# JuliaMolSim/DFTK.jl

Measured on AMD Instinct MI355X. Metric: SCF iterations/sec (Hψ applies/sec) at fixed Ecut·atoms, higher is better.
Workload: dtype f64

## Files before the change

### dftk.jl_amd/_lib.py

```python
from __future__ import annotations

import ctypes as C
import os

from . import _build

c_cplx_p = C.c_void_p
_i64 = C.c_int64


class dftk_mi_cplx(C.Structure):
    _fields_ = [("re", C.c_double), ("im", C.c_double)]


class dftk_mi_batch_op(C.Structure):
    _fields_ = ([(name, C.c_int32) for name in ("type", "fiber", "trans", "m", "k", "i0", "mode", "flags", "join_next",
                                                 "sync_after", "status", "reserved")] +
                [(name, _i64) for name in ("n", "gm", "gn", "gk", "lda", "ldb", "ldc")] +
                [("alpha", dftk_mi_cplx), ("beta", dftk_mi_cplx), ("s0", C.c_double)] +
                [(name, C.c_void_p) for name in ("A", "B", "W", "W2", "W3", "C", "D", "E", "F", "kb", "host")] +
                [("bytes", C.c_uint64)])


class DftkMiError(RuntimeError):
    def __init__(self, status, msg):
        super().__init__(f"dftk_mi355x status {status}: {msg}")
        self.status = status


_SIGNATURES = {
    "dftk_mi_last_error": (C.c_char_p, []),
    "dftk_mi_version": (C.c_char_p, []),
    "dftk_mi_basis_create": (C.c_int, [C.c_int, C.c_int, C.c_int, C.c_double, C.c_int, C.POINTER(C.c_void_p)]),
    "dftk_mi_basis_destroy": (C.c_int, [C.c_void_p]),
    "dftk_mi_basis_sync": (C.c_int, [C.c_void_p]),
    "dftk_mi_basis_set_fft_batch": (C.c_int, [C.c_void_p, C.c_int]),
    "dftk_mi_basis_stream": (C.c_void_p, [C.c_void_p]),
    "dftk_mi_kblock_create": (C.c_int, [C.c_void_p, _i64, C.c_void_p, C.c_void_p, C.POINTER(C.c_void_p)]),
    "dftk_mi_kblock_destroy": (C.c_int, [C.c_void_p]),
    "dftk_mi_kblock_set_projectors": (C.c_int, [C.c_void_p, C.c_int, C.c_void_p, _i64, C.c_void_p]),
    "dftk_mi_kblock_set_potential": (C.c_int, [C.c_void_p, C.c_void_p]),
    "dftk_mi_apply_H": (C.c_int, [C.c_void_p, C.c_int, C.c_void_p, _i64, C.c_void_p, _i64]),
    "dftk_mi_apply_H_parts": (C.c_int, [C.c_void_p, C.c_int, C.c_int, C.c_void_p, _i64, C.c_void_p, _i64]),
    "dftk_mi_local_potential": (C.c_int, [C.c_void_p, C.c_void_p, C.c_void_p, C.c_void_p, C.c_int, C.c_void_p,
                                          C.c_void_p]),
    "dftk_mi_local_potential_collinear": (C.c_int, [C.c_void_p, C.c_void_p, C.c_void_p, C.c_void_p, C.c_int, C.c_void_p,
                                                    C.c_void_p]),
    "dftk_mi_density_accumulate_spin": (C.c_int, [C.c_void_p, C.c_int, C.c_void_p, _i64, C.c_void_p, C.c_void_p, C.c_int,
                                                  C.c_int]),
    "dftk_mi_kpoint_sphere_host": (C.c_int, [C.c_int, C.c_int, C.c_int, C.c_void_p, C.c_void_p, C.c_double, _i64,
                                             C.POINTER(_i64), C.c_void_p, C.c_void_p, C.c_void_p]),
    "dftk_mi_build_projectors_hgh": (C.c_int, [C.c_void_p, _i64, C.c_void_p, C.c_void_p, C.c_void_p, C.c_double, C.c_int,
                                               C.c_void_p, C.c_void_p, C.c_int, C.c_void_p, C.c_void_p, C.c_void_p, _i64,
                                               C.POINTER(C.c_int)]),
    "dftk_mi_atomic_superposition": (C.c_int, [C.c_void_p, C.c_int, C.c_void_p, C.c_int, C.c_void_p, C.c_int, C.c_void_p,
                                               C.c_void_p, C.c_void_p]),
    "dftk_mi_forces_local": (C.c_int, [C.c_void_p, C.c_void_p, C.c_int, C.c_void_p, C.c_int, C.c_void_p, C.c_void_p,
                                       C.c_void_p, C.c_void_p]),
    "dftk_mi_radial_transform": (C.c_int, [C.c_void_p, C.c_int, C.c_int, C.c_int, C.c_void_p, C.c_void_p, C.c_double, _i64,
                                           C.c_void_p, C.c_void_p]),
    "dftk_mi_radial_tile": (C.c_int, []),
    "dftk_mi_build_projectors_radial": (C.c_int, [C.c_void_p, _i64, C.c_void_p, C.c_void_p, C.c_void_p, C.c_double,
                                                  C.c_int, C.c_void_p, _i64, C.c_void_p, C.c_void_p, C.c_int, C.c_void_p,
                                                  C.c_void_p, C.c_void_p, _i64, C.POINTER(C.c_int)]),
    "dftk_mi_atomic_superposition_table": (C.c_int, [C.c_void_p, C.c_void_p, C.c_int, C.c_void_p, C.c_int, C.c_void_p,
                                                     C.c_void_p, C.c_void_p, C.c_void_p]),
    "dftk_mi_forces_local_table": (C.c_int, [C.c_void_p, C.c_void_p, C.c_int, C.c_void_p, C.c_int, C.c_void_p, C.c_void_p,
                                             C.c_void_p, C.c_void_p]),
    "dftk_mi_forces_nonlocal": (C.c_int, [C.c_void_p, C.c_void_p, C.c_int, C.c_void_p, _i64, C.c_void_p, C.c_int,
                                          C.c_void_p, C.c_void_p]),
    "dftk_mi_local_potential_displacement": (C.c_int, [C.c_void_p, C.c_void_p, C.c_int, C.c_void_p, C.c_int, C.c_void_p,
                                                       C.c_void_p]),
    "dftk_mi_dynmat_local": (C.c_int, [C.c_void_p, C.c_void_p, C.c_int, C.c_void_p, C.c_int, C.c_void_p, C.c_void_p,
                                       C.c_void_p, C.c_void_p]),
    "dftk_mi_nonlocal_displacement_apply": (C.c_int, [C.c_void_p, C.c_void_p, C.c_int, C.c_int, C.c_void_p, C.c_int,
                                                      C.c_void_p, _i64, C.c_void_p, _i64]),
    "dftk_mi_dynmat_nonlocal": (C.c_int, [C.c_void_p, C.c_void_p, C.c_int, C.c_void_p, _i64, C.c_void_p, _i64, C.c_void_p,
                                          C.c_void_p, C.c_int, C.c_void_p, C.c_void_p, C.c_void_p]),
    "dftk_mi_stress_kinetic_nonlocal": (C.c_int, [C.c_void_p, C.c_void_p, C.c_void_p, C.c_int, C.c_void_p, _i64, C.c_void_p,
                                                  C.c_int, C.c_void_p, C.c_void_p, C.c_int, C.c_void_p, C.c_void_p,
                                                  C.c_void_p, C.c_void_p]),
    "dftk_mi_stress_cube": (C.c_int, [C.c_void_p, C.c_void_p, C.c_int, C.c_void_p, C.c_int, C.c_void_p, C.c_void_p,
                                      C.c_void_p, C.c_void_p]),
    "dftk_mi_stress_xc": (C.c_int, [C.c_void_p, _i64, C.c_int, C.c_void_p, C.c_void_p, C.c_void_p, C.c_void_p, C.c_void_p,
                                    C.c_void_p]),
    "dftk_mi_xc_gga": (C.c_int, [C.c_void_p, _i64, C.c_void_p, C.c_void_p, C.c_int, C.c_double, C.c_void_p, C.c_void_p,
                                 C.c_void_p]),
    "dftk_mi_ifft_sphere": (C.c_int, [C.c_void_p, C.c_void_p, C.c_void_p]),
    "dftk_mi_fft_sphere": (C.c_int, [C.c_void_p, C.c_void_p, C.c_void_p]),
    "dftk_mi_density_accumulate": (C.c_int, [C.c_void_p, C.c_int, C.c_void_p, _i64, C.c_void_p, C.c_void_p]),
    "dftk_mi_sternheimer": (C.c_int, [C.c_void_p, C.c_int, C.c_void_p, _i64, C.c_void_p, C.c_int, C.c_void_p, _i64, C.c_void_p,
                                      _i64, C.c_void_p, C.c_int, C.c_int, C.c_void_p, _i64, C.c_void_p, _i64,
                                      C.POINTER(C.c_int), C.c_void_p, C.POINTER(C.c_int)]),
    "dftk_mi_density_response_accumulate": (C.c_int, [C.c_void_p, C.c_int, C.c_void_p, _i64, C.c_void_p, _i64, C.c_void_p,
                                                      C.c_void_p, C.c_void_p]),
    "dftk_mi_apply_kernel": (C.c_int, [C.c_void_p, C.c_void_p, C.c_void_p, C.c_void_p, C.c_int, C.c_void_p]),
    "dftk_mi_transfer_blochwave": (C.c_int, [C.c_void_p, C.c_void_p, C.c_void_p, C.c_int, C.c_void_p, _i64, C.c_void_p, _i64]),
    "dftk_mi_transfer_density": (C.c_int, [C.c_void_p, C.c_void_p, C.c_int, C.c_void_p, C.c_void_p]),
    "dftk_mi_refinement_metric_solve": (C.c_int, [C.c_void_p, C.c_int, C.c_void_p, _i64, C.c_void_p, _i64, C.c_double, C.c_int,
                                                  C.c_void_p, _i64, C.c_void_p, C.c_void_p]),
    "dftk_mi_exx_apply": (C.c_int, [C.c_void_p, C.c_int, C.c_void_p, _i64, C.c_void_p, C.c_void_p, C.c_int, C.c_void_p, _i64,
                                    C.c_void_p, _i64, C.c_int]),
    "dftk_mi_lobpcg": (C.c_int, [C.c_void_p, C.c_int, C.c_void_p, _i64, C.c_double, C.c_int, C.c_int, C.c_int,
                                 C.c_int, C.c_uint64, C.c_void_p, C.c_void_p, C.POINTER(C.c_int),
                                 C.POINTER(C.c_int), C.POINTER(_i64)]),
    "dftk_mi_local_potential_gga": (C.c_int, [C.c_void_p, C.c_void_p, C.c_void_p, C.c_void_p, C.c_void_p, C.c_int,
                                              C.c_double, C.c_void_p, C.c_void_p]),
    "dftk_mi_local_potential_collinear_gga": (C.c_int, [C.c_void_p, C.c_void_p, C.c_void_p, C.c_void_p, C.c_void_p, C.c_int,
                                                        C.c_double, C.c_void_p, C.c_void_p]),
    "dftk_mi_local_potential_core": (C.c_int, [C.c_void_p, C.c_void_p, C.c_int, C.c_void_p, C.c_void_p, C.c_void_p,
                                               C.c_void_p, C.c_void_p, C.c_int, C.c_double, C.c_void_p, C.c_void_p]),
    "dftk_mi_cube_gradient": (C.c_int, [C.c_void_p, C.c_void_p, C.c_void_p, C.c_void_p]),
    "dftk_mi_xc_gga_spin": (C.c_int, [C.c_void_p, _i64, C.c_void_p, C.c_void_p, C.c_int, C.c_double, C.c_void_p, C.c_void_p,
                                      C.c_void_p]),
    "dftk_mi_kblock_set_kpoint": (C.c_int, [C.c_void_p, C.c_void_p, C.c_void_p]),
    "dftk_mi_kblock_set_tau_potential": (C.c_int, [C.c_void_p, C.c_void_p]),
    "dftk_mi_kblocks_set_tau_potential": (C.c_int, [C.c_int, C.c_void_p, C.c_void_p]),
    "dftk_mi_kinetic_energy_density_accumulate": (C.c_int, [C.c_void_p, C.c_int, C.c_void_p, _i64, C.c_void_p, C.c_void_p]),
    "dftk_mi_local_potential_mgga": (C.c_int, [C.c_void_p, C.c_void_p, C.c_void_p, C.c_void_p, C.c_void_p, C.c_void_p, C.c_int,
                                               C.c_double, C.c_void_p, C.c_void_p, C.c_void_p]),
    "dftk_mi_xc_mgga": (C.c_int, [C.c_void_p, _i64, C.c_void_p, C.c_void_p, C.c_void_p, C.c_int, C.c_double, C.c_void_p,
                                  C.c_void_p, C.c_void_p, C.c_void_p]),
    "dftk_mi_symmetrize_rho": (C.c_int, [C.c_void_p, C.c_int, C.c_void_p, C.c_void_p, C.c_int, C.c_void_p, C.c_void_p]),
    "dftk_mi_mix_kerker": (C.c_int, [C.c_void_p, C.c_void_p, C.c_double, C.c_void_p, C.c_void_p]),
    "dftk_mi_mix_dielectric": (C.c_int, [C.c_void_p, C.c_void_p, C.c_double, C.c_double, C.c_void_p, C.c_void_p]),
    "dftk_mi_chi0_dielectric_apply": (C.c_int, [C.c_void_p, C.c_void_p, C.c_double, C.c_double, C.c_void_p, C.c_void_p]),
    "dftk_mi_cube_fourier_filter": (C.c_int, [C.c_void_p, C.c_void_p, C.c_void_p, C.c_void_p]),
    "dftk_mi_kblocks_set_potential": (C.c_int, [C.c_int, C.c_void_p, C.c_void_p]),
    "dftk_mi_lobpcg_multi": (C.c_int, [C.c_int, C.c_void_p, C.c_int, C.c_void_p, C.c_void_p, C.c_double, C.c_int, C.c_int,
                                       C.c_int, C.c_int, C.c_void_p, C.c_void_p, C.c_void_p, C.c_void_p, C.c_void_p,
                                       C.c_void_p, C.c_void_p]),
    "dftk_mi_density_accumulate_multi": (C.c_int, [C.c_int, C.c_void_p, C.c_void_p, C.c_void_p, C.c_void_p, C.c_void_p,
                                                   C.c_void_p]),
    "dftk_mi_density_accumulate_multi2": (C.c_int, [C.c_int, C.c_void_p, C.c_void_p, C.c_void_p, C.c_void_p, C.c_void_p,
                                                    C.c_void_p, C.c_void_p, C.c_void_p]),
    "dftk_mi_band_kinetic_multi": (C.c_int, [C.c_int, C.c_void_p, C.c_void_p, C.c_void_p, C.c_void_p, C.c_void_p]),
    "dftk_mi_batch_stats": (C.c_int, [C.POINTER(_i64), C.POINTER(_i64), C.POINTER(_i64), C.POINTER(_i64)]),
    "dftk_mi_lobpcg_small_stats": (C.c_int, [C.POINTER(_i64), C.POINTER(_i64)]),
    "dftk_mi_ortho_small": (C.c_int, [C.c_void_p, _i64, C.c_int, C.c_void_p, _i64, C.c_int, C.c_void_p, _i64, C.c_void_p,
                                      C.c_double, C.c_void_p]),
    "dftk_mi_batch_replay": (C.c_int, [C.c_void_p, C.c_int, C.c_int, C.c_void_p]),
    "dftk_mi_lobpcg_last_AX": (C.c_void_p, [C.c_void_p]),
    "dftk_mi_lobpcg_history": (C.c_int, [C.c_void_p, C.POINTER(C.c_int), C.POINTER(C.c_int), C.c_void_p, C.c_size_t,
                                         C.POINTER(C.c_int)]),
    "dftk_mi_columnwise_norms": (C.c_int, [C.c_void_p, _i64, C.c_int, C.c_void_p, _i64, C.c_void_p]),
    "dftk_mi_columnwise_dots": (C.c_int, [C.c_void_p, _i64, C.c_int, C.c_void_p, _i64, C.c_void_p, _i64, C.c_void_p]),
    "dftk_mi_ortho_qr": (C.c_int, [C.c_void_p, _i64, C.c_int, C.c_void_p, _i64, C.c_int, C.POINTER(C.c_int),
                                   C.POINTER(C.c_int)]),
    "dftk_mi_tpa_precondprep": (C.c_int, [C.c_void_p, C.c_int, C.c_void_p, _i64, C.c_void_p]),
    "dftk_mi_tpa_ldiv": (C.c_int, [C.c_void_p, C.c_int, C.c_void_p, _i64, C.c_void_p, C.c_double, C.c_void_p, _i64]),
    "dftk_mi_block_residual": (C.c_int, [C.c_void_p, C.c_int, C.c_void_p, _i64, C.c_void_p, _i64, C.c_void_p,
                                         C.c_void_p, _i64, C.c_void_p, C.c_void_p, C.c_void_p]),
    "dftk_mi_kblock_set_gamma_real": (C.c_int, [C.c_void_p, C.c_int]),
    "dftk_mi_gamma_half_size": (C.c_int, [C.c_void_p, C.POINTER(_i64)]),
    "dftk_mi_gamma_tables_host": (C.c_int, [C.c_int, C.c_int, C.c_int, _i64, C.c_void_p, C.POINTER(_i64), C.c_void_p,
                                            C.c_void_p]),
    "dftk_mi_gamma_compress": (C.c_int, [C.c_void_p, C.c_int, C.c_void_p, _i64, C.c_void_p, _i64]),
    "dftk_mi_gamma_compress_aligned": (C.c_int, [C.c_void_p, C.c_int, C.c_void_p, _i64, C.c_void_p, _i64]),
    "dftk_mi_gamma_expand": (C.c_int, [C.c_void_p, C.c_int, C.c_void_p, _i64, C.c_void_p, _i64]),
    "dftk_mi_gamma_apply_H": (C.c_int, [C.c_void_p, C.c_int, C.c_int, C.c_void_p, _i64, C.c_void_p, _i64]),
    "dftk_mi_density_accumulate_real": (C.c_int, [C.c_void_p, C.c_int, C.c_void_p, _i64, C.c_void_p, C.c_void_p]),
    "dftk_mi_shard_plan_host": (C.c_int, [C.c_int, C.c_int, C.c_int, C.c_void_p, C.c_void_p, C.c_void_p, C.c_void_p,
                                          C.c_void_p, C.c_void_p]),
    "dftk_mi_kblock_set_shard": (C.c_int, [C.c_void_p, C.c_void_p, C.c_void_p]),
    "dftk_mi_zgemm": (C.c_int, [C.c_void_p, C.c_char, _i64, _i64, _i64, dftk_mi_cplx, C.c_void_p, _i64,
                                C.c_void_p, _i64, dftk_mi_cplx, C.c_void_p, _i64]),
    "dftk_mi_zgemm_ex": (C.c_int, [C.c_void_p, C.c_char, _i64, _i64, _i64, dftk_mi_cplx, C.c_void_p, _i64,
                                   C.c_void_p, _i64, dftk_mi_cplx, C.c_void_p, _i64, C.c_int]),
    "dftk_mi_zgemm_to": (C.c_int, [C.c_void_p, C.c_char, _i64, _i64, _i64, dftk_mi_cplx, C.c_void_p, _i64,
                                   C.c_void_p, _i64, dftk_mi_cplx, C.c_void_p, _i64, C.c_void_p, C.c_int]),
    "dftk_mi_zgemm_plan_host": (C.c_int, [C.c_char, _i64, _i64, _i64, C.c_int, C.POINTER(C.c_int)]),
    "dftk_mi_zgemm_fold_host": (C.c_int, [C.c_char, _i64, _i64, _i64, C.c_int, C.c_int, C.POINTER(C.c_int), C.POINTER(C.c_int)]),
    "dftk_mi_zgemm_compact_host": (C.c_int, [C.c_int, C.c_int, C.c_int, C.c_int, C.c_int, C.POINTER(C.c_int), C.POINTER(C.c_int)]),
    "dftk_mi_heev": (C.c_int, [C.c_void_p, C.c_int, C.c_void_p, _i64, C.c_void_p, C.c_void_p, _i64]),
    "dftk_mi_prof_zgemm_shapes": (C.c_int, [C.c_void_p, C.c_int, C.c_void_p, C.c_void_p, C.POINTER(C.c_int)]),
    "dftk_mi_eig_mirror_tall": (C.c_int, [C.c_void_p, C.c_int, C.c_int, C.c_void_p, _i64]),
    "dftk_mi_heev_lowest": (C.c_int, [C.c_void_p, C.c_int, C.c_int, C.c_void_p, _i64, C.c_void_p, C.c_void_p, _i64]),
    "dftk_mi_heev_sigma_host": (C.c_int, [C.c_int, C.c_void_p, C.c_int, C.POINTER(C.c_double), C.POINTER(C.c_double),
                                          C.POINTER(C.c_int), C.c_double]),
    "dftk_mi_potrf_trtri": (C.c_int, [C.c_void_p, C.c_int, C.c_void_p, _i64, C.c_void_p, _i64]),
    "dftk_mi_potrf_trtri_real": (C.c_int, [C.c_void_p, C.c_int, C.c_void_p, _i64, C.c_void_p, _i64]),
    "dftk_mi_lowdin_ortho": (C.c_int, [C.c_void_p, _i64, C.c_int, C.c_void_p, _i64, C.c_void_p]),
    "dftk_mi_pdos_accumulate": (C.c_int, [C.c_void_p, _i64, C.c_int, C.c_void_p, _i64, C.c_int, C.c_void_p, _i64, C.c_void_p,
                                          C.c_double, C.c_int, C.c_double, C.c_int, C.c_void_p, C.c_void_p, C.c_void_p]),
    "dftk_mi_hubbard_occupation": (C.c_int, [C.c_void_p, _i64, C.c_int, C.c_void_p, _i64, C.c_int, C.c_void_p, _i64, C.c_void_p,
                                             C.c_int, C.c_void_p, C.c_void_p, C.c_void_p]),
    "dftk_mi_hubbard_rotate": (C.c_int, [C.c_void_p, _i64, C.c_int, C.c_void_p, C.c_void_p, C.c_void_p, _i64, C.c_void_p,
                                         C.c_void_p, _i64]),
    "dftk_mi_comm_get_unique_id": (C.c_int, [C.c_char_p]),
    "dftk_mi_comm_init_rank": (C.c_int, [C.c_char_p, C.c_int, C.c_int, C.c_int, C.POINTER(C.c_void_p)]),
    "dftk_mi_comm_create_host": (C.c_int, [C.c_int, C.c_int, C.c_int, C.c_void_p, C.c_void_p, C.c_void_p,
                                           C.POINTER(C.c_void_p)]),
    "dftk_mi_comm_destroy": (C.c_int, [C.c_void_p]),
    "dftk_mi_comm_describe": (C.c_int, [C.c_void_p, C.POINTER(C.c_int), C.POINTER(C.c_int), C.POINTER(C.c_int)]),
    "dftk_mi_comm_rank": (C.c_int, [C.c_void_p]),
    "dftk_mi_comm_size": (C.c_int, [C.c_void_p]),
    "dftk_mi_allreduce_sum_f64": (C.c_int, [C.c_void_p, C.c_void_p, C.c_size_t, C.c_void_p]),
    "dftk_mi_prof_enable": (C.c_int, [C.c_void_p, C.c_int]),
    "dftk_mi_prof_get": (C.c_int, [C.c_void_p, C.c_int, C.POINTER(C.c_double), C.POINTER(C.c_double),
                                   C.POINTER(_i64)]),
    "dftk_mi_anderson_create": (C.c_int, [C.c_void_p, _i64, C.c_int, C.c_double, C.c_double, C.POINTER(C.c_void_p)]),
    "dftk_mi_anderson_destroy": (C.c_int, [C.c_void_p]),
    "dftk_mi_anderson_reset": (C.c_int, [C.c_void_p]),
    "dftk_mi_anderson_history": (C.c_int, [C.c_void_p]),
    "dftk_mi_stiefel_project_tangent": (C.c_int, [C.c_void_p, _i64, C.c_int, C.c_void_p, _i64, C.c_void_p, _i64]),
    "dftk_mi_lbfgs_create": (C.c_int, [C.c_void_p, C.c_int, C.c_void_p, C.c_void_p, C.c_int, C.POINTER(C.c_void_p)]),
    "dftk_mi_lbfgs_destroy": (C.c_int, [C.c_void_p]),
    "dftk_mi_lbfgs_reset": (C.c_int, [C.c_void_p]),
    "dftk_mi_lbfgs_history": (C.c_int, [C.c_void_p]),
    "dftk_mi_lbfgs_update": (C.c_int, [C.c_void_p, C.c_void_p, C.c_void_p, C.c_void_p, C.c_void_p, C.POINTER(C.c_double),
                                       C.POINTER(C.c_int)]),
    "dftk_mi_lbfgs_direction": (C.c_int, [C.c_void_p, C.c_void_p, C.c_void_p, C.c_void_p, C.c_void_p, C.c_void_p, C.c_void_p,
                                          C.c_void_p]),
    "dftk_mi_anderson_step": (C.c_int, [C.c_void_p, C.c_void_p, C.c_double, C.c_void_p, C.c_void_p, C.POINTER(C.c_int)]),
    "dftk_mi_chi0_mix": (C.c_int, [C.c_void_p, C.c_int, C.c_void_p, C.c_void_p, C.c_void_p, C.c_double, C.c_int, C.c_double,
                                   C.c_double, C.c_void_p, C.c_double, C.c_int, C.c_int, C.c_void_p, C.POINTER(C.c_int),
                                   C.POINTER(C.c_int)]),
    "dftk_mi_launch_count": (C.c_int, [C.POINTER(_i64), C.POINTER(_i64)]),
    "dftk_mi_device_buffers_live": (C.c_int, [C.POINTER(_i64), C.POINTER(_i64)]),
    "dftk_mi_kblock_reuse_AX": (C.c_int, [C.c_void_p, C.c_int]),
    "dftk_mi_ax_reuse_count": (C.c_int, [C.POINTER(_i64)]),
    "dftk_mi_planes_reuse_count": (C.c_int, [C.POINTER(_i64)]),
    "dftk_mi_step_sums": (C.c_int, [C.c_void_p, _i64, C.c_void_p, C.c_void_p, C.c_void_p, C.c_void_p]),
    "dftk_mi_fermi_bisection": (C.c_int, [C.c_int, C.c_void_p, C.c_void_p, C.c_void_p, C.c_int, C.c_double, C.c_double,
                                          C.c_double, C.c_double, C.c_double, C.POINTER(C.c_double)]),
    "dftk_mi_diag_mfma_peak": (C.c_int, [C.c_void_p, C.c_int, C.c_int, C.POINTER(C.c_double)]),
    "dftk_mi_jacobi_schedule_host": (C.c_int, [C.c_int, C.c_int, C.POINTER(C.c_int), C.POINTER(C.c_int),
                                               C.POINTER(C.c_int)]),
    "dftk_mi_fft_plan_host": (C.c_int, [C.c_int, C.POINTER(C.c_int), C.POINTER(C.c_int), C.POINTER(C.c_int)]),
    "dftk_mi_sphere_tables_host": (C.c_int, [C.c_int, C.c_int, C.c_int, _i64, C.c_void_p, C.POINTER(_i64),
                                             C.POINTER(C.c_int), C.c_void_p, C.c_void_p]),
}

ALLREDUCE_FN = C.CFUNCTYPE(C.c_int, C.c_void_p, C.POINTER(C.c_double), C.c_size_t)
ALLTOALLV_FN = C.CFUNCTYPE(C.c_int, C.c_void_p, C.POINTER(C.c_double), C.POINTER(C.c_size_t), C.POINTER(C.c_size_t),
                           C.POINTER(C.c_double), C.POINTER(C.c_size_t), C.POINTER(C.c_size_t))

EXPORTED_SYMBOLS = tuple(_SIGNATURES)
_lib = None


def load(build_if_missing: bool = True):
    global _lib
    if _lib is not None:
        return _lib
    path = _build.LIBPATH
    if build_if_missing and _build.needs_build():
        _build.build()
    if not os.path.exists(path):
        raise RuntimeError(f"{path} is missing and could not be built; the MI355X hot path has no fallback")
    lib = C.CDLL(path, mode=C.RTLD_GLOBAL)
    for name, (res, args) in _SIGNATURES.items():
        fn = getattr(lib, name)
        fn.restype = res
        fn.argtypes = args
    version = lib.dftk_mi_version().decode()
    if not version.endswith("src=" + _build.source_hash()):
        raise RuntimeError(f"{path} was built from other sources ({version!r}, expected src={_build.source_hash()}): "
                           "stale binary, rebuild with python -m dftk_jl_amd._build")
    _lib = lib
    return lib


def check(status: int):
    if status != 0:
        msg = load().dftk_mi_last_error().decode(errors="replace")
        raise DftkMiError(status, msg)


def cplx(z) -> dftk_mi_cplx:
    z = complex(z)
    return dftk_mi_cplx(z.real, z.imag)
```

### dftk.jl_amd/csrc/api.cpp

```cpp
#include "common.h"
#include <chrono>
#include "batch.h"
#include <algorithm>
#include <cmath>
#include <cstdarg>
#include <cstdio>
#include <cstdlib>
#include <cstring>
#include <vector>

static thread_local char g_err[1024] = "";

void dftk_set_error(const char* fmt, ...) {
    va_list ap;
    va_start(ap, fmt);
    vsnprintf(g_err, sizeof(g_err), fmt, ap);
    va_end(ap);
}

extern "C" const char* dftk_mi_last_error(void) { return g_err; }

hipError_t dftk_scratch_malloc(void** p, size_t bytes) {
    static const bool poison = getenv("DFTK_MI_POISON") != nullptr;
    hipError_t e = hipMalloc(p, bytes);
// ... 147 lines not shown
int plan_radices(int n, int* nrad, int* rad) {
    int m = n, a2 = 0, a3 = 0, a5 = 0;
    while (m % 2 == 0 && m > 1) { m /= 2; ++a2; }
    while (m % 3 == 0 && m > 1) { m /= 3; ++a3; }
    while (m % 5 == 0 && m > 1) { m /= 5; ++a5; }
    int best8 = 0, best6 = 0, best = 1 << 30;
    for (int n8 = 0; n8 <= a2 / 3; ++n8)
        for (int n6 = 0; n6 <= (a2 - 3 * n8 < a3 ? a2 - 3 * n8 : a3); ++n6) {
            const int rem2 = a2 - 3 * n8 - n6;
            const int stages = n8 + n6 + rem2 / 2 + rem2 % 2 + (a3 - n6) + a5;
            if (stages < best) {
                best = stages;
                best8 = n8;
                best6 = n6;
            }
        }
    const int rem2 = a2 - 3 * best8 - best6;
    int counts[6][2] = {{8, best8}, {6, best6}, {5, a5}, {4, rem2 / 2}, {3, a3 - best6}, {2, rem2 % 2}};
    int k = 0;
    for (int oi : {2, 4})
        if (counts[oi][1] > 0) {
            rad[k++] = counts[oi][0];
            counts[oi][1] -= 1;
            break;
        }
    for (auto& c : counts)
        for (int i = 0; i < c[1]; ++i) {
            if (k >= DFTK_MAX_RADICES) return -1;
            rad[k++] = c[0];
        }
    for (int p = 7; m > 1; p += 2)
        while (m % p == 0) {
            if (k >= DFTK_MAX_RADICES || p > 64) return -1;
            rad[k++] = p;
            m /= p;
        }
    *nrad = k;
    return 0;
}

void plan_positions(int n, int nrad, const int* rad, int* pos) {
    if (nrad == 0) {
        for (int i = 0; i < n; ++i) pos[i] = i;
        return;
    }
    std::vector<int> m(nrad + 1, 1);
    for (int s = 0; s < nrad; ++s) m[s + 1] = m[s] * rad[s];
    for (int p = 0; p < n; ++p) {
        int e = (p / m[0]) % rad[0];
        for (int s = 1; s < nrad; ++s) e = (p / m[s]) % rad[s] + rad[s] * e;
        pos[e] = p;
    }
}

extern "C" int dftk_mi_jacobi_schedule_host(int n, int round, int* n_blocks, int* pairs, int* where) {
    return jacobi_schedule_host(n, round, n_blocks, pairs, where);
}

extern "C" int dftk_mi_fft_plan_host(int n, int* n_radices, int* radices, int* pos) {
    if (n < 1 || !n_radices || !radices || !pos) return DFTK_MI_EINVAL;
    if (plan_radices(n, n_radices, radices) != 0) {
        dftk_set_error("cannot plan FFT of length %d (prime factor > 64)", n);
        return DFTK_MI_EINVAL;
    }
    plan_positions(n, *n_radices, radices, pos);
    return 0;
}

struct SphereTables {
    std::vector<int64_t> line_id;
    std::vector<int64_t> line_start;
    std::vector<int> zval;
    std::vector<int> zls;
};

static int build_sphere_tables(int nx, int ny, int nz, int64_t n_G, const int64_t* mapping, SphereTables& t) {
    const int64_t N = (int64_t)nx * ny * nz;
    int64_t prev = -1, prev_line = -1;
    int prev_z = -1;
    for (int64_t c = 0; c < n_G; ++c) {
        const int64_t g = mapping[c];
        if (g < 0 || g >= N || g <= prev) {
            dftk_set_error("mapping must be strictly ascending and within the cube (entry %lld = %lld)", (long long)c,
                           (long long)g);
            return DFTK_MI_EINVAL;
        }
        prev = g;
        const int64_t line = g / nx;
        if (line != prev_line) {
            t.line_id.push_back(line);
            t.line_start.push_back(c);
            prev_line = line;
            const int iz = (int)(line / ny);
            if (iz != prev_z) {
                t.zval.push_back(iz);
                t.zls.push_back((int)t.line_id.size() - 1);
                prev_z = iz;
            }
        }
    }
    t.line_start.push_back(n_G);
    t.zls.push_back((int)t.line_id.size());
    return 0;
}

extern "C" int dftk_mi_sphere_tables_host(int nx, int ny, int nz, int64_t n_G, const int64_t* mapping0_h,
                                          int64_t* n_lines, int* n_zplanes, int64_t* line_id, int64_t* line_start) {
    if (nx < 1 || ny < 1 || nz < 1 || n_G < 0 || (n_G > 0 && !mapping0_h)) return DFTK_MI_EINVAL;
    SphereTables t;
    CHK(build_sphere_tables(nx, ny, nz, n_G, mapping0_h, t));
    if (n_lines) *n_lines = (int64_t)t.line_id.size();
    if (n_zplanes) *n_zplanes = (int)t.zval.size();
    if (line_id) std::copy(t.line_id.begin(), t.line_id.end(), line_id);
    if (line_start) std::copy(t.line_start.begin(), t.line_start.end(), line_start);
    return 0;
}

template <typename T, typename U>
static int upload(const std::vector<T>& v, DevTable<U>& d) {
    HIPCHK(d.alloc(v.size() * sizeof(T)));
    if (v.empty()) return 0;
    HIPCHK(hipMemcpy(d.get(), v.data(), v.size() * sizeof(T), hipMemcpyHostToDevice));
    return 0;
}

static int check_device(int device) {
    int count = 0;
    hipError_t e = hipGetDeviceCount(&count);
    if (e != hipSuccess || count <= 0) {
        dftk_set_error("no HIP device visible (%s): this library has no CPU fallback",
                       e == hipSuccess ? "count = 0" : hipGetErrorString(e));
        return DFTK_MI_ENOGPU;
    }
    if (device < 0 || device >= count) {
        dftk_set_error("device %d out of range (%d visible)", device, count);
        return DFTK_MI_EINVAL;
    }
    return 0;
}

extern "C" int dftk_mi_basis_create(int nx, int ny, int nz, double unit_cell_volume, int device,
                                    dftk_mi_basis** out) {
    if (!out || nx < 1 || ny < 1 || nz < 1 || !(unit_cell_volume > 0)) return DFTK_MI_EINVAL;
    CHK(check_device(device));
    HIPCHK(hipSetDevice(device));
    std::unique_ptr<dftk_mi_basis> b(new dftk_mi_basis());
    b->nx = nx;
    b->ny = ny;
    b->nz = nz;
    b->nxp = ((nx + 7) / 8) * 8;
    b->volume = unit_cell_volume;
    b->device = device;
    b->fft_batch = 32;
    b->prof.reset(new Prof());
    const char* g = getenv("DFTK_MI_GEMM");
    b->use_mfma = (g && strcmp(g, "naive") == 0) ? 0 : 1;
    HIPCHK(hipStreamCreate(&b->stream.s));
    const int dims[3] = {nx, ny, nz};
    for (int a = 0; a < 3; ++a) {
        const int n = dims[a];
        FftAxis& ax = b->ax[a];
        ax.n = n;
        if (plan_radices(n, &ax.nrad, ax.rad) != 0) {
            dftk_set_error("cannot plan FFT axis of length %d", n);
            return DFTK_MI_EINVAL;
        }
        std::vector<int> pos(n);
        plan_positions(n, ax.nrad, ax.rad, pos.data());
        std::vector<double> tw(2 * (size_t)n);
        for (int t = 0; t < n; ++t) {
            const long double ang = 2.0L * 3.14159265358979323846264338327950288L * (long double)t / (long double)n;
            tw[2 * t] = (double)cosl(ang);
            tw[2 * t + 1] = (double)sinl(ang);
        }
        CHK(upload(tw, b->d_tables[2 * a]));
        CHK(upload(pos, b->d_tables[2 * a + 1]));
        ax.tw = static_cast<const cd*>(b->d_tables[2 * a].get());
        ax.pos = static_cast<const int*>(b->d_tables[2 * a + 1].get());
    }
    HIPCHK(b->d_scalars.alloc(256 * sizeof(double)));
    HIPCHK(b->h_scalars.alloc(256 * sizeof(double)));
    HIPCHK(b->h_fetch.alloc(HOST_FETCH_BYTES));
    *out = b.release();
    return 0;
}

extern "C" int dftk_mi_basis_destroy(dftk_mi_basis* b) {
    if (!b) return 0;
    hipSetDevice(b->device);
    hipStreamSynchronize(b->stream);
    prof_resolve(b);
    delete b;
    return 0;
}

extern "C" int dftk_mi_basis_sync(dftk_mi_basis* b) {
    if (!b) return DFTK_MI_EINVAL;
    HIPCHK(hipStreamSynchronize(b->stream));
    return 0;
}

extern "C" int dftk_mi_basis_set_fft_batch(dftk_mi_basis* b, int n) {
    if (!b || n < 1 || n > 256) return DFTK_MI_EINVAL;
    b->fft_batch = n;
    return 0;
}

extern "C" void* dftk_mi_basis_stream(dftk_mi_basis* b) { return b ? (void*)b->stream : nullptr; }

extern "C" int dftk_mi_kblock_create(dftk_mi_basis* b, int64_t n_G, const int64_t* mapping0_h, const double* kinetic_h,
                                     dftk_mi_kblock** out) {
    if (!b || !out || n_G < 1 || !mapping0_h) return DFTK_MI_EINVAL;
    if (n_G > INT32_MAX) return DFTK_MI_EINVAL;
    HIPCHK(hipSetDevice(b->device));
    SphereTables t;
    CHK(build_sphere_tables(b->nx, b->ny, b->nz, n_G, mapping0_h, t));
    std::vector<int> pos[3];
    const int dims[3] = {b->nx, b->ny, b->nz};
    for (int a = 0; a < 3; ++a) {
        pos[a].resize(dims[a]);
        plan_positions(dims[a], b->ax[a].nrad, b->ax[a].rad, pos[a].data());
    }
    const int64_t n_lines = (int64_t)t.line_id.size();
    std::vector<int> cpos(n_G), cx(n_G), line_start(n_lines + 1), line_ypos(n_lines), line_yval(n_lines);
    for (int64_t l = 0; l < n_lines; ++l) {
        const int iy = (int)(t.line_id[l] % b->ny);
        line_yval[l] = iy;
        line_ypos[l] = pos[1][iy];
        line_start[l] = (int)t.line_start[l];
        for (int64_t c = t.line_start[l]; c < t.line_start[l + 1]; ++c) {
            const int ix = (int)(mapping0_h[c] - t.line_id[l] * b->nx);
            cx[c] = ix;
            cpos[c] = pos[0][ix];
        }
    }
    line_start[n_lines] = (int)n_G;
    std::vector<int> zpos(t.zval.size());
    for (size_t i = 0; i < t.zval.size(); ++i) zpos[i] = pos[2][t.zval[i]];

    std::unique_ptr<dftk_mi_kblock> kb(new dftk_mi_kblock());
    kb->basis = b;
    kb->device = b->device;
    kb->n_G = n_G;
    kb->n_lines = n_lines;
    kb->nzx = (int)t.zval.size();
    {
        int lo = 0;
        while (lo < kb->nzx && t.zval[lo] == lo) ++lo;
        bool ok = true;
        for (int i = lo; i < kb->nzx; ++i) ok = ok && t.zval[i] == b->nz - (kb->nzx - i);
        kb->z_lo = ok ? lo : -1;
    }
    CHK(upload(cpos, kb->d_cpos));
    CHK(upload(cx, kb->d_cx));
    CHK(upload(line_start, kb->d_line_start));
    CHK(upload(line_ypos, kb->d_line_ypos));
    CHK(upload(line_yval, kb->d_line_yval));
    CHK(upload(t.zls, kb->d_zls));
    CHK(upload(zpos, kb->d_zpos));
    CHK(upload(t.zval, kb->d_zval));
    std::vector<double> kin(n_G, 0.0);
    if (kinetic_h) std::copy(kinetic_h, kinetic_h + n_G, kin.begin());
    CHK(upload(kin, kb->d_kin));
    kb->h_mapping.assign(mapping0_h, mapping0_h + n_G);
    kb->h_kin = std::move(kin);
    kb->kin_given = kinetic_h != nullptr;
    *out = kb.release();
    return 0;
}

static void release_Vs(dftk_mi_kblock* kb) {
    kb->Vs_buf.reset();
    kb->Vs_shared = false;
    kb->d_Vs = nullptr;
}

extern "C" int dftk_mi_kblock_destroy(dftk_mi_kblock* kb) {
    if (!kb) return 0;
    hipSetDevice(kb->device);
    hipDeviceSynchronize();
    delete kb;
    return 0;
}

static int64_t local_rows(const dftk_mi_kblock* kb) {
    if (!kb->sh_comm) return kb->n_G;
    const int r = comm_rank(kb->sh_comm);
    return kb->sh_rows[r + 1] - kb->sh_rows[r];
}

extern "C" int dftk_mi_kblock_set_shard(dftk_mi_kblock* kb, dftk_mi_comm* comm, const int64_t* row_starts_h) {
    if (!kb) return DFTK_MI_EINVAL;
    HIPCHK(hipSetDevice(kb->basis->device));
    HIPCHK(hipStreamSynchronize(kb->basis->stream));
    kb->ho.forget_planes();
    if (!comm || comm_size(comm) == 1) {
        kb->sh_comm = nullptr;
        return 0;
    }
    if (kb->gr && kb->gr->on) {
        dftk_set_error("set_shard: call before dftk_mi_kblock_set_gamma_real (the half-format rows are split when it is switched on)");
        return DFTK_MI_EINVAL;
    }
    const int p = comm_size(comm);
    if (!row_starts_h || row_starts_h[0] != 0 || row_starts_h[p] != kb->n_G) {
        dftk_set_error("set_shard: row_starts must run from 0 to n_G over n_ranks + 1 entries");
        return DFTK_MI_EINVAL;
    }
    for (int r = 0; r < p; ++r)
        if (row_starts_h[r + 1] <= row_starts_h[r]) {
            dftk_set_error("set_shard: every rank needs a non-empty row slab");
            return DFTK_MI_EINVAL;
        }
    if (kb->n_p != 0) {
        dftk_set_error("set_shard: call before dftk_mi_kblock_set_projectors (P becomes the row slab of this rank)");
        return DFTK_MI_EINVAL;
    }
    kb->sh_rows.assign(row_starts_h, row_starts_h + p + 1);
    kb->sh_comm = comm;
    return 0;
}

static void band_split(int nb, int p, std::vector<int>& c0) {
    c0.assign(p + 1, 0);
    const int base = nb / p, rem = nb % p;
    for (int s = 0; s < p; ++s) c0[s + 1] = c0[s] + base + (s < rem ? 1 : 0);
}

static int shard_buffers(dftk_mi_kblock* kb, int nb, cd** R1, cd** F, cd** G) {
    const int p = comm_size(kb->sh_comm);
    const size_t maxc = (size_t)(nb + p - 1) / p;
    const size_t each = (size_t)kb->n_G * (maxc ? maxc : 1);
    const size_t need = 3 * each * sizeof(cd);
    CHK(scratch_grow(kb->basis, kb->sh_buf, need));
    *R1 = kb->sh_buf;
    *F = kb->sh_buf + each;
    *G = kb->sh_buf + 2 * each;
    return 0;
}

static void shard_plan(const std::vector<int64_t>& rows, int p, int me, int nb, std::vector<int>& c0,
                       std::vector<size_t>& slab_off, std::vector<size_t>& slab_cnt, std::vector<size_t>& band_off,
                       std::vector<size_t>& band_cnt) {
    band_split(nb, p, c0);
    const int64_t nloc = rows[me + 1] - rows[me];
    const int mine = c0[me + 1] - c0[me];
    slab_off.resize(p), slab_cnt.resize(p), band_off.resize(p), band_cnt.resize(p);
    for (int s = 0; s < p; ++s) {
        slab_off[s] = (size_t)c0[s] * nloc;
        slab_cnt[s] = (size_t)(c0[s + 1] - c0[s]) * nloc;
        band_off[s] = (size_t)rows[s] * mine;
        band_cnt[s] = (size_t)(rows[s + 1] - rows[s]) * mine;
    }
}

extern "C" int dftk_mi_shard_plan_host(int n_ranks, int rank, int n_bands, const int64_t* row_starts_h,
                                       int* band_starts , int64_t* slab_off, int64_t* slab_cnt,
// ... 1177 lines not shown
```

### dftk.jl_amd/csrc/common.h

```cpp
#pragma once
#include <hip/hip_runtime.h>
#include <stdint.h>
#include <stddef.h>
#include <string>
#include <map>
#include <vector>
#include <memory>
#include "devbuf.h"
#include "handover.h"
#include "../../include/dftk_mi355x.h"

typedef double2 cd;

#include <atomic>
extern std::atomic<int64_t> g_dftk_launches, g_dftk_host_syncs;
inline hipError_t dftk_counted_stream_sync(hipStream_t s) {
    g_dftk_host_syncs.fetch_add(1, std::memory_order_relaxed);
    return (hipStreamSynchronize)(s);
}
#define hipStreamSynchronize(s) dftk_counted_stream_sync(s)
#undef hipLaunchKernelGGL
#define hipLaunchKernelGGL(kernelName, ...)                               \
    do {                                                                  \
        g_dftk_launches.fetch_add(1, std::memory_order_relaxed);          \
        hipLaunchKernelGGLInternal((kernelName), __VA_ARGS__);            \
    } while (0)

void dftk_set_error(const char* fmt, ...);
bool land_in_place();
hipError_t dftk_scratch_malloc(void** p, size_t bytes);

#define HIPCHK(expr)                                                                      \
    do {                                                                                  \
        hipError_t _e = (expr);                                                           \
        if (_e != hipSuccess) {                                                           \
            dftk_set_error("%s failed: %s (%s:%d)", #expr, hipGetErrorString(_e), __FILE__, __LINE__); \
            return DFTK_MI_EHIP;                                                          \
        }                                                                                 \
    } while (0)

#define CHK(expr)                                 \
    do {                                          \
        int _s = (expr);                          \
        if (_s != 0) return _s;                   \
    } while (0)

struct WsCarver {
    void** slot[16];
    size_t at[16];
    int n = 0;
    size_t off = 0;
    template <class T>
    void take(T** p, size_t count) {
        slot[n] = reinterpret_cast<void**>(p);
        at[n++] = off;
        off += (count * sizeof(T) + 255) & ~(size_t)255;
    }
    size_t bytes() const { return off; }
    void bind(void* base) const {
        for (int i = 0; i < n; ++i) *slot[i] = static_cast<char*>(base) + at[i];
    }
};

template <int K>
__device__ inline void block_reduce(double* v) {
    __shared__ double sh[K][256];
#pragma unroll
    for (int k = 0; k < K; ++k) sh[k][threadIdx.x] = v[k];
    __syncthreads();
    for (int h = 128; h > 0; h >>= 1) {
        if ((int)threadIdx.x < h)
#pragma unroll
            for (int k = 0; k < K; ++k) sh[k][threadIdx.x] += sh[k][threadIdx.x + h];
        __syncthreads();
    }
    if (threadIdx.x == 0)
#pragma unroll
        for (int k = 0; k < K; ++k) v[k] = sh[k][0];
}

__device__ __forceinline__ double wave_sum(double v) {
#pragma unroll
    for (int off = 32; off > 0; off >>= 1) v += __shfl_down(v, off, 64);
    return v;
}
template <int NT>
__device__ __forceinline__ double block_sum(double v, double* sh) {
    v = wave_sum(v);
    const int lane = threadIdx.x & 63, w = threadIdx.x >> 6;
    if (lane == 0) sh[w] = v;
    __syncthreads();
    double r = 0.0;
    if (threadIdx.x == 0) {
#pragma unroll
        for (int i = 0; i < NT / 64; ++i) r += sh[i];
    }
    __syncthreads();
    return r;
}

#define DFTK_MAX_RADICES 32
struct FftAxis {
    int n;
    int nrad;
    int rad[DFTK_MAX_RADICES];
    const cd* tw;
    const int* pos;
};

int  plan_radices(int n, int* nrad, int* rad);
void plan_positions(int n, int nrad, const int* rad, int* pos);

struct StreamOwner {
    hipStream_t s = nullptr;
    StreamOwner() = default;
    StreamOwner(const StreamOwner&) = delete;
    StreamOwner& operator=(const StreamOwner&) = delete;
    ~StreamOwner() { if (s) hipStreamDestroy(s); }
    operator hipStream_t() const { return s; }
};
struct EventOwner {
    hipEvent_t e = nullptr;
    EventOwner() = default;
    EventOwner(const EventOwner&) = delete;
    EventOwner& operator=(const EventOwner&) = delete;
    ~EventOwner() { if (e) hipEventDestroy(e); }
};
struct dftk_mi_basis {
    int nx = 0, ny = 0, nz = 0, nxp = 0;
    double volume = 0.0;
    int device = 0;
    StreamOwner stream;
    EventOwner order_ev;
    FftAxis ax[3] = {};
    DevTable<void> d_tables[6];
    int fft_batch = 0;
    DevBuf<cd> T1;
    DevBuf<cd> T2;
    DevBuf<void> ws;
    DevTable<double> d_scalars;
    PinnedBuf<double> h_scalars;
    Buf<char, Mem::PinnedMapped> h_fetch;
    int use_mfma = 0;
    std::unique_ptr<struct Prof> prof;
    DevBuf<void> dense_ws;
    DevBuf<void> eig_ws;
    struct dftk_mi_comm* comm = nullptr;
    DevTable<void> symm_tab; uint64_t symm_key = 0; int symm_n = 0;
    DevBuf<void> resp_ws;
    DevBuf<void> exx_ws;
};

enum ProfFamily {
    PROF_ZGEMM = 0,
    PROF_FFT_A = 1,
    PROF_FFT_B = 2,
    PROF_FFT_C = 3,
    PROF_FFT_D = 4,
    PROF_FFT_E = 5,
    PROF_DENS_Z = 6,
    PROF_HEEV = 7,
    PROF_CHOL = 8,
    PROF_APPLY_H = 9,
    PROF_ZGEMM_BYTES = 10,
    PROF_ZGEMM_STRUCT = 11,
    PROF_ZGEMM_EXEC = 12,
    PROF_COMM = 13,
    PROF_ZGEMM_CPLX = 14,
    PROF_EW = 15,
    PROF_HOST_WAIT = 16,
    PROF_AR_MODEL = 17,
    PROF_A2A_MODEL = 18,
    PROF_NFAM = 24
};
struct Prof {
    bool on = false;
    struct Pair { hipEvent_t a, b; int fam; uint64_t tag; double work; };
    struct Shape { double ms = 0, work = 0; int64_t n = 0; };
    std::map<uint64_t, Shape> shapes;
    std::vector<Pair> pending;
    std::vector<Pair> pool;
    int open = 0;
    int mute = 0;
    bool shape_tags = false;
    double ms[PROF_NFAM] = {0};
    double work[PROF_NFAM] = {0};
    int64_t launches[PROF_NFAM] = {0};
    Prof() = default;
    Prof(const Prof&) = delete;
    Prof& operator=(const Prof&) = delete;
    ~Prof() {
        for (auto* v : {&pending, &pool})
            for (auto& pr : *v) {
                hipEventDestroy(pr.a);
                hipEventDestroy(pr.b);
            }
    }
};
int prof_begin(dftk_mi_basis* b, int fam, double work, uint64_t tag = 0);
void prof_end(dftk_mi_basis* b, int slot);
int prof_resolve(dftk_mi_basis* b);
struct ProfScope {
    dftk_mi_basis* b;
    int slot;
    ProfScope(dftk_mi_basis* basis, int fam, double work) : b(basis), slot(prof_begin(basis, fam, work)) {}
    ~ProfScope() { prof_end(b, slot); }
    ProfScope(const ProfScope&) = delete;
    ProfScope& operator=(const ProfScope&) = delete;
};
void prof_count(dftk_mi_basis* b, int fam, double work);
const size_t HOST_FETCH_BYTES = 256 * 1024;
int host_wait(dftk_mi_basis* b);
int host_fetch(dftk_mi_basis* b, void* dst_h, const void* src_d, size_t bytes);

struct GammaReal {
    bool on = false;
    int64_t n_half = 0;
    DevTable<int> d_g, d_mg;
    DevTable<double> d_kin_half;
    DevTable<cd> P_half;
    const cd* P_src = nullptr;
    int P_n_p = 0;
    DevBuf<cd> buf;
    std::vector<int64_t> half_rows;
};

inline std::atomic<uint64_t> g_kblock_serial{0};
struct dftk_mi_kblock {
    dftk_mi_basis* basis = nullptr;
    int device = 0;
    int64_t n_G = 0;
    int64_t n_lines = 0;
    int nzx = 0;
    int z_lo = 0;
    DevTable<int> d_cpos;
    DevTable<int> d_line_start;
    DevTable<int> d_line_ypos;
    DevTable<int> d_zls;
    DevTable<int> d_zpos;
    DevTable<int> d_zval;
    DevTable<int> d_line_yval;
    DevTable<int> d_cx;
    DevTable<double> d_kin;
    std::shared_ptr<DevTable<double>> Vs_buf;
    bool Vs_shared = false;
    double* d_Vs = nullptr;
    std::shared_ptr<DevTable<double>> Vtau_buf;
    bool Vtau_shared = false;
    double* d_Vtau = nullptr;
    bool frame_set = false;
    double frame_B[9] = {0};
    double frame_k[3] = {0};
    DevBuf<cd> mgga_buf;
    int n_p = 0;
    const cd* P = nullptr;
    int64_t ldP = 0;
    DevTable<double> d_D;
    int D_bw = 0;
    DevBuf<cd> lob_buf;
    LobHandover ho;
    dftk_mi_comm* sh_comm = nullptr;
    std::vector<int64_t> sh_rows;
    DevBuf<cd> sh_buf;
    std::vector<double> lob_hist; int lob_hist_M = 0, lob_hist_iters = 0, lob_n_svd = 0;
    std::vector<int64_t> h_mapping;
    std::vector<double> h_kin;
    std::unique_ptr<GammaReal> gr;
    DevTable<int32_t> d_G3;
    DevTable<int32_t> d_inv;
    uint64_t serial = g_kblock_serial.fetch_add(1, std::memory_order_relaxed) + 1;
    uint64_t transfer_in_serial = 0;
    int transfer_dG[3] = {0, 0, 0};
    bool kin_given = false;
};

int fft_ensure_scratch(dftk_mi_basis* b, dftk_mi_kblock* kb, int nb);
int launch_local_apply(dftk_mi_kblock* kb, int nb, const cd* psi, int64_t ldpsi, cd* out,
                       int64_t ldout, bool add_kinetic, bool have_local, const double* shift_d = nullptr);
int launch_ifft_to_cube(dftk_mi_kblock* kb, const cd* c, cd* cube, int nb = 1);
int launch_fft_from_cube(dftk_mi_kblock* kb, const cd* cube, cd* c, int nb = 1);
int launch_density(dftk_mi_kblock* kb, int nb, const cd* psi, int64_t ldpsi, const double* w_h, double* rho,
                   const double* w_im_h = nullptr, const double* w2_h = nullptr, double* rho2 = nullptr,
                   bool keep_planes = false, int pair_nb = 0);
int fft_group_size(const dftk_mi_basis* b);
int launch_planes_fill(dftk_mi_kblock* kb, int b0, int nbb, const cd* psi, int64_t ldpsi, cd* planes, int pair_nb = 0);
int launch_local_apply_from_planes(dftk_mi_kblock* kb, int nb, cd* planes, cd* out, int64_t ldout);
int launch_density_response(dftk_mi_kblock* kb, int nb, const cd* psi, int64_t ldpsi, const cd* dpsi, int64_t lddpsi,
                            const double* wo_h, const double* wd_h, double* drho);
int launch_pad_potential(dftk_mi_kblock* kb, const double* V, double* dst = nullptr);
// ... 207 lines not shown
```

### dftk.jl_amd/csrc/fft_kernels.hip

```cpp
#include "common.h"
#include "batch.h"
#include <algorithm>
#include <cstring>
#include <type_traits>

#define FFT_L 8
#ifndef ZPASS_MIN_BLOCKS
#define ZPASS_MIN_BLOCKS 6
#endif
#ifndef DENS_MIN_BLOCKS
#define DENS_MIN_BLOCKS 1
#endif
#ifndef YFWD_MIN_BLOCKS
#define YFWD_MIN_BLOCKS 1
#endif
#define FFT_LS_X 9
#define FFT_LS_YZ 8
#define FFT_THREADS 256
#define FFT_TPL (FFT_THREADS / FFT_L)
#define DENS_MAXACC 12

__device__ __forceinline__ cd cmul(cd a, cd w) {
    return make_double2(fma(a.x, w.x, -a.y * w.y), fma(a.x, w.y, a.y * w.x));
}
// ... 122 lines not shown
                a[p] = cmul(a[p], w);
            }
        }
        if (VMUL) {
#pragma unroll
            for (int p = 0; p < R; ++p) {
                a[p].x *= vv[p];
                a[p].y *= vv[p];
            }
            dft_small<R>(a, -sgn, tw, nOverR);
            if (m > 1) {
#pragma unroll
                for (int p = 1; p < R; ++p) {
                    cd w = tw[p * jj * twstep];
                    w.y *= -sgn;
                    a[p] = cmul(a[p], w);
                }
            }
        }
#pragma unroll
        for (int p = 0; p < R; ++p) buf[(base + p * m) * FFT_LS + l] = a[p];
    }
}

template <int FFT_LS, bool DIF>
__device__ void fft_stage_generic(cd* buf, const cd* __restrict__ tw, int n, int m, int R, double sgn,
                                  int l, int j) {
    const int nb = n / R;
    const int twstep = n / (R * m);
    const int nOverR = n / R;
    for (int b = j; b < nb; b += FFT_TPL) {
        const int g = b / m;
        const int jj = b - g * m;
        const int base = g * R * m + jj;
        cd a[64], o[64];
        for (int q = 0; q < R; ++q) {
            cd v = buf[(base + q * m) * FFT_LS + l];
            if (!DIF && m > 1 && q > 0) {
                cd w = tw[q * jj * twstep];
                w.y *= sgn;
                v = cmul(v, w);
            }
            a[q] = v;
        }
        for (int p = 0; p < R; ++p) {
            cd acc = a[0];
            for (int q = 1; q < R; ++q) {
                cd w = tw[((p * q) % R) * nOverR];
                w.y *= sgn;
                cd t = cmul(a[q], w);
                acc.x += t.x;
                acc.y += t.y;
            }
            if (DIF && m > 1 && p > 0) {
                cd w = tw[p * jj * twstep];
                w.y *= sgn;
                acc = cmul(acc, w);
            }
            o[p] = acc;
        }
        for (int p = 0; p < R; ++p) buf[(base + p * m) * FFT_LS + l] = o[p];
    }
}

template <int FFT_LS>
__device__ __forceinline__ bool fft_stage_vmul(int R, cd* buf, const cd* tw, int n, int m, double sgn, int l, int j,
                                               const double* vcol, int64_t vstride) {
    switch (R) {
        case 2: fft_stage<FFT_LS, 2, false, true>(buf, tw, n, m, sgn, l, j, vcol, vstride); return true;
        case 3: fft_stage<FFT_LS, 3, false, true>(buf, tw, n, m, sgn, l, j, vcol, vstride); return true;
        case 4: fft_stage<FFT_LS, 4, false, true>(buf, tw, n, m, sgn, l, j, vcol, vstride); return true;
        case 5: fft_stage<FFT_LS, 5, false, true>(buf, tw, n, m, sgn, l, j, vcol, vstride); return true;
        case 6: fft_stage<FFT_LS, 6, false, true>(buf, tw, n, m, sgn, l, j, vcol, vstride); return true;
        case 8: fft_stage<FFT_LS, 8, false, true>(buf, tw, n, m, sgn, l, j, vcol, vstride); return true;
        default: return false;
    }
}

template <int FFT_LS, bool DIF, bool GEN>
__device__ __forceinline__ void fft_stage_dispatch(int R, cd* buf, const cd* tw, int n, int m, double sgn,
                                                   int l, int j) {
    switch (R) {
        case 2: fft_stage<FFT_LS, 2, DIF>(buf, tw, n, m, sgn, l, j); break;
        case 3: fft_stage<FFT_LS, 3, DIF>(buf, tw, n, m, sgn, l, j); break;
        case 4: fft_stage<FFT_LS, 4, DIF>(buf, tw, n, m, sgn, l, j); break;
        case 5: fft_stage<FFT_LS, 5, DIF>(buf, tw, n, m, sgn, l, j); break;
        case 6: fft_stage<FFT_LS, 6, DIF>(buf, tw, n, m, sgn, l, j); break;
        case 8: fft_stage<FFT_LS, 8, DIF>(buf, tw, n, m, sgn, l, j); break;
        default:
            if constexpr (GEN) {
                if (R == 7)
                    fft_stage<FFT_LS, 7, DIF>(buf, tw, n, m, sgn, l, j);
                else
                    fft_stage_generic<FFT_LS, DIF>(buf, tw, n, m, R, sgn, l, j);
            }
            break;
    }
}

template <int FFT_LS, bool DIF, bool GEN>
__device__ __forceinline__ bool fft_tile(cd* buf, const cd* tw, const FftAxis& ax, double sgn, int l, int j,
                                         const double* vcol = nullptr, int64_t vstride = 0,
                                         bool skip_first = false) {
    const int n = ax.n;
    bool fused = false;
    if (!DIF) {
        int m = 1;
        for (int s = 0; s < ax.nrad; ++s) {
            const int R = ax.rad[s];
            if (vcol != nullptr && s == ax.nrad - 1)
                fused = fft_stage_vmul<FFT_LS>(R, buf, tw, n, m, sgn, l, j, vcol, vstride);
            if (!fused) fft_stage_dispatch<FFT_LS, false, GEN>(R, buf, tw, n, m, sgn, l, j);
            __syncthreads();
            m *= R;
        }
    } else {
        int m = n;
        for (int s = ax.nrad - 1; s >= 0; --s) {
            const int R = ax.rad[s];
            m /= R;
            if (skip_first && s == ax.nrad - 1) continue;
            fft_stage_dispatch<FFT_LS, true, GEN>(R, buf, tw, n, m, sgn, l, j);
            __syncthreads();
        }
    }
    return fused;
}

template <int FFT_LS>
__device__ __forceinline__ void tile_prologue(cd* buf, cd* tw, const FftAxis& ax, bool zero, bool copy_tw = true) {
    const int n = ax.n;
    if (copy_tw)
        for (int t = threadIdx.x; t < n; t += FFT_THREADS) tw[t] = ax.tw[t];
    if (zero) {
        const cd z = make_double2(0.0, 0.0);
        for (int t = threadIdx.x; t < n * FFT_LS; t += FFT_THREADS) buf[t] = z;
    }
}

extern __shared__ __attribute__((aligned(16))) char dftk_smem[];

struct FftJob {
    const int *line_start, *cpos, *line_ypos, *zls, *zpos;
    int z_lo;
    const double* kin;
    const double* Vs;
    const cd* psi;
    cd* out;
    int n_lines, nzx;
    double w, wim;
    double w2;
};

template <bool GEN, bool PAIR = false>
__global__ __launch_bounds__(FFT_THREADS) void k_xbwd_scatter(FftAxis ax, int nxp, int n_lines,
                                                              const int* __restrict__ line_start,
                                                              const int* __restrict__ cpos,
                                                              const cd* __restrict__ psi, int64_t ldpsi,
                                                              cd* __restrict__ T1, int64_t T1_stride,
                                                              const FftJob* __restrict__ jobs, int pair_nb) {
    constexpr int FFT_LS = FFT_LS_X;
    cd* buf = reinterpret_cast<cd*>(dftk_smem);
    cd* tw = buf + ax.n * FFT_LS;
    const int tid = threadIdx.x, l = tid & (FFT_L - 1), j = tid >> 3;
    const int band = blockIdx.y;
    const int l0 = blockIdx.x * FFT_L;
    const cd* p = psi + (int64_t)(PAIR ? 2 * band : band) * ldpsi;
    if (!PAIR && jobs) {
        const FftJob jb = jobs[band];
        n_lines = jb.n_lines;
        line_start = jb.line_start;
        cpos = jb.cpos;
        p = jb.psi;
        if (l0 >= n_lines) return;
    }
    tile_prologue<FFT_LS>(buf, tw, ax, true);
    __syncthreads();
    const int line = l0 + l;
    if (line < n_lines) {
        const int c0 = line_start[line], c1 = line_start[line + 1];
        if (PAIR) {
            const bool has_b = 2 * band + 1 < pair_nb;
            const cd* pb = p + ldpsi;
            for (int c = c0 + j; c < c1; c += FFT_TPL) {
                const cd a = p[c];
                const cd bb = has_b ? pb[c] : make_double2(0.0, 0.0);
                buf[cpos[c] * FFT_LS + l] = make_double2(a.x - bb.y, a.y + bb.x);
            }
        } else {
            for (int c = c0 + j; c < c1; c += FFT_TPL) buf[cpos[c] * FFT_LS + l] = p[c];
        }
    }
    __syncthreads();
    fft_tile<FFT_LS, false, GEN>(buf, tw, ax, +1.0, l, j);
    cd* out = T1 + (int64_t)band * T1_stride + (int64_t)l0 * nxp;
    const int nlv = min(FFT_L, n_lines - l0);
    const int n = ax.n;
    for (int idx = tid; idx < nlv * nxp; idx += FFT_THREADS) {
        const int ll = idx / nxp;
        const int x = idx - ll * nxp;
        out[idx] = (x < n) ? buf[x * FFT_LS + ll] : make_double2(0.0, 0.0);
    }
}

template <bool GEN>
__global__ __launch_bounds__(FFT_THREADS) void k_ybwd(FftAxis ay, int nxp, int ny,
                                                      const int* __restrict__ zls,
                                                      const int* __restrict__ line_ypos,
                                                      const cd* __restrict__ T1, int64_t T1_stride,
                                                      cd* __restrict__ T2, int64_t T2_stride,
                                                      const FftJob* __restrict__ jobs) {
    constexpr int FFT_LS = FFT_LS_YZ;
    cd* buf = reinterpret_cast<cd*>(dftk_smem);
    cd* tw = buf + ay.n * FFT_LS;
    const int tid = threadIdx.x, l = tid & (FFT_L - 1), j = tid >> 3;
    const int x = blockIdx.x * FFT_L + l;
    const int zi = blockIdx.y, band = blockIdx.z;
    if (jobs) {
        const FftJob jb = jobs[band];
        if (zi >= jb.nzx) return;
        zls = jb.zls;
        line_ypos = jb.line_ypos;
    }
    const cd* t1 = T1 + (int64_t)band * T1_stride;
    const int ln0 = zls[zi] + j, ln1 = zls[zi + 1];
    const bool early = ln1 - zls[zi] <= 3 * FFT_TPL;
    cd e0, e1, e2;
    if (early) {
        if (ln0 < ln1) e0 = t1[(int64_t)ln0 * nxp + x];
        if (ln0 + FFT_TPL < ln1) e1 = t1[(int64_t)(ln0 + FFT_TPL) * nxp + x];
        if (ln0 + 2 * FFT_TPL < ln1) e2 = t1[(int64_t)(ln0 + 2 * FFT_TPL) * nxp + x];
    }
    tile_prologue<FFT_LS>(buf, tw, ay, true);
    __syncthreads();
    if (early) {
        if (ln0 < ln1) buf[line_ypos[ln0] * FFT_LS + l] = e0;
        if (ln0 + FFT_TPL < ln1) buf[line_ypos[ln0 + FFT_TPL] * FFT_LS + l] = e1;
        if (ln0 + 2 * FFT_TPL < ln1) buf[line_ypos[ln0 + 2 * FFT_TPL] * FFT_LS + l] = e2;
    } else {
        for (int ln = ln0; ln < ln1; ln += FFT_TPL) buf[line_ypos[ln] * FFT_LS + l] = t1[(int64_t)ln * nxp + x];
    }
    __syncthreads();
    fft_tile<FFT_LS, false, GEN>(buf, tw, ay, +1.0, l, j);
    cd* t2 = T2 + (int64_t)band * T2_stride + (int64_t)zi * ny * nxp + x;
    for (int y = j; y < ny; y += FFT_TPL) t2[(int64_t)y * nxp] = buf[y * FFT_LS + l];
}

template <int MODE, bool GEN>
__global__ __launch_bounds__(FFT_THREADS, ZPASS_MIN_BLOCKS) void k_zpass(FftAxis az, int nx, int nxp, int ny, int nzx,
                                                       int nbands, const int* __restrict__ zpos,
                                                       const double* __restrict__ Vs,
                                                       cd* __restrict__ T2, int64_t T2_stride,
                                                       cd* __restrict__ cube, const FftJob* __restrict__ jobs = nullptr) {
    constexpr int FFT_LS = FFT_LS_YZ;
    cd* buf = reinterpret_cast<cd*>(dftk_smem);
    cd* tw = buf + az.n * FFT_LS;
    const int tid = threadIdx.x, l = tid & (FFT_L - 1), j = tid >> 3;
    const int xcd = blockIdx.x & 7, slot = blockIdx.x >> 3;
    const int band = slot % nbands;
    const int grp = (slot / nbands) * 8 + xcd;
    const int nxt = nxp / FFT_L;
    if (grp >= nxt * ny) return;
    if (jobs) {
        const FftJob jb = jobs[band];
        zpos = jb.zpos;
        nzx = jb.nzx;
        Vs = jb.Vs;
    }
    const int y = grp / nxt;
    const int x = (grp - y * nxt) * FFT_L + l;
    const int nz = az.n;
    const int64_t plane = (int64_t)ny * nxp;
    cd* t2 = T2 + (int64_t)band * T2_stride + (int64_t)y * nxp + x;
    const bool early = MODE != 2 && nzx <= 3 * FFT_TPL;
    cd e0, e1, e2;
    if (early) {
        if (j < nzx) e0 = t2[(int64_t)j * plane];
        if (j + FFT_TPL < nzx) e1 = t2[(int64_t)(j + FFT_TPL) * plane];
        if (j + 2 * FFT_TPL < nzx) e2 = t2[(int64_t)(j + 2 * FFT_TPL) * plane];
    }
    tile_prologue<FFT_LS>(buf, tw, az, MODE != 2, true);
    __syncthreads();
    bool fused_v = false;
    if (MODE != 2) {
        if (early) {
            if (j < nzx) buf[zpos[j] * FFT_LS + l] = e0;
            if (j + FFT_TPL < nzx) buf[zpos[j + FFT_TPL] * FFT_LS + l] = e1;
            if (j + 2 * FFT_TPL < nzx) buf[zpos[j + 2 * FFT_TPL] * FFT_LS + l] = e2;
        } else {
            for (int zi = j; zi < nzx; zi += FFT_TPL) buf[zpos[zi] * FFT_LS + l] = t2[(int64_t)zi * plane];
        }
        __syncthreads();
        fused_v = fft_tile<FFT_LS, false, GEN>(buf, tw, az, +1.0, l, j,
                                       (MODE == 0 && !GEN) ? Vs + (int64_t)y * nxp + x : nullptr, plane);
    }
    if (MODE == 0 && !fused_v) {
        const double* v = Vs + (int64_t)y * nxp + x;
        for (int z = j; z < nz; z += FFT_TPL) {
            const double s = v[(int64_t)z * plane];
            cd a = buf[z * FFT_LS + l];
            a.x *= s;
            a.y *= s;
            buf[z * FFT_LS + l] = a;
        }
        __syncthreads();
    }
    if (MODE == 1 || MODE == 2) cube += (int64_t)band * nz * ny * nx;
    if (MODE == 1) {
        if (x < nx)
            for (int z = j; z < nz; z += FFT_TPL) cube[((int64_t)z * ny + y) * nx + x] = buf[z * FFT_LS + l];
        return;
    }
    if (MODE == 2) {
        for (int z = j; z < nz; z += FFT_TPL)
            buf[z * FFT_LS + l] = (x < nx) ? cube[((int64_t)z * ny + y) * nx + x] : make_double2(0.0, 0.0);
        __syncthreads();
    }
    fft_tile<FFT_LS, true, GEN>(buf, tw, az, -1.0, l, j, nullptr, 0, MODE == 0 && fused_v);
    for (int zi = j; zi < nzx; zi += FFT_TPL) t2[(int64_t)zi * plane] = buf[zpos[zi] * FFT_LS + l];
}

namespace ctw {
constexpr double PI = 3.14159265358979323846264338327950288;
constexpr double sin_small(double x) {
    const double x2 = x * x;
    double term = x, sum = x;
    for (int k = 1; k <= 12; ++k) {
        term *= -x2 / (double)((2 * k) * (2 * k + 1));
        sum += term;
    }
    return sum;
}
constexpr double cos_small(double x) {
    const double x2 = x * x;
    double term = 1.0, sum = 1.0;
    for (int k = 1; k <= 12; ++k) {
        term *= -x2 / (double)((2 * k - 1) * (2 * k));
        sum += term;
    }
    return sum;
}
struct CS {
    double c, s;
};
constexpr CS cs(int m, int N) {
    m %= N;
    if (m < 0) m += N;
    const int k = (8 * m + N) / (2 * N);
    const double delta = 2.0 * PI * (double)(4 * m - k * N) / (4.0 * (double)N);
    const double c = cos_small(delta), s = sin_small(delta);
    switch (k & 3) {
        case 0: return CS{c, s};
        case 1: return CS{-s, c};
        case 2: return CS{-c, -s};
        default: return CS{s, -c};
    }
}
}

template <int B, int E, class F>
__device__ __forceinline__ void static_for(F&& f) {
    if constexpr (B < E) {
        f(std::integral_constant<int, B>{});
        static_for<B + 1, E>(f);
    }
}
template <int N, int SGN, int M>
__device__ __forceinline__ cd tw_mul_c(cd a) {
    constexpr int m = ((M % N) + N) % N;
    if constexpr (m == 0) {
        return a;
    } else if constexpr (2 * m == N) {
        return make_double2(-a.x, -a.y);
    } else if constexpr (4 * m == N) {
        return SGN > 0 ? make_double2(-a.y, a.x) : make_double2(a.y, -a.x);
    } else if constexpr (4 * m == 3 * N) {
        return SGN > 0 ? make_double2(a.y, -a.x) : make_double2(-a.y, a.x);
    } else {
        constexpr ctw::CS w = ctw::cs(m, N);
        constexpr double c = w.c, s = (SGN > 0 ? w.s : -w.s);
        return make_double2(fma(a.x, c, -a.y * s), fma(a.x, s, a.y * c));
    }
}
template <int RA, int RB, int SGN>
__device__ __forceinline__ void dft_ct(cd (&x)[RA * RB]) {
    static_for<0, RB>([&](auto bi) {
        constexpr int b = decltype(bi)::value;
        cd t[RA];
#pragma unroll
        for (int a = 0; a < RA; ++a) t[a] = x[RB * a + b];
        dft_small<RA>(t, (double)SGN, nullptr, 0);
        static_for<0, RA>([&](auto ci) {
            constexpr int c = decltype(ci)::value;
            x[RB * c + b] = tw_mul_c<RA * RB, SGN, b * c>(t[c]);
        });
    });
    static_for<0, RA>([&](auto ci) {
        constexpr int c = decltype(ci)::value;
        cd u[RB];
#pragma unroll
        for (int b = 0; b < RB; ++b) u[b] = x[RB * c + b];
        dft_small<RB>(u, (double)SGN, nullptr, 0);
#pragma unroll
        for (int d = 0; d < RB; ++d) x[RB * c + d] = u[d];
    });
}

#ifndef ZREG_MIN_BLOCKS
#define ZREG_MIN_BLOCKS 3
#endif
template <int R1A, int R1B, int R2A, int R2B>
struct FourStep {
    static constexpr int R1 = R1A * R1B, R2 = R2A * R2B, N = R1 * R2, L = FFT_L;
    static constexpr int TPL = R1 > R2 ? R1 : R2, THREADS = L * TPL;
    static constexpr int P1 = R2 * L + ((R2 % 2 == 0) ? 8 : 0), P2 = R1 * L + ((R1 % 2 == 0) ? 8 : 0);
    static constexpr int LDS_ELEMS = R1 * P1 > R2 * P2 ? R1 * P1 : R2 * P2;
    static constexpr int k2_of(int p) { return p / R2B + R2A * (p % R2B); }
    static constexpr int k2p_of(int p) { return p / R1B + R1A * (p % R1B); }

    template <class IN>
    static __device__ __forceinline__ void backward(cd* buf, const cd* __restrict__ twg, int l, int j, IN in, cd (&out)[R2]) {
        if (j < R2) {
            cd a[R1];
            static_for<0, R1>([&](auto ni) { a[decltype(ni)::value] = in(ni); });
            const cd w1 = twg[j], wA = twg[j * R1A];
            dft_ct<R1A, R1B, +1>(a);
            cd wd = make_double2(1.0, 0.0);
            static_for<0, R1B>([&](auto di) {
                constexpr int d = decltype(di)::value;
                if constexpr (d > 0) wd = (d == 1) ? wA : cmul(wd, wA);
                cd w = wd;
                static_for<0, R1A>([&](auto ci) {
                    constexpr int c = decltype(ci)::value;
                    if constexpr (c > 0) w = cmul(w, w1);
                    constexpr int k1 = c + R1A * d;
                    buf[k1 * P1 + j * L + l] = (k1 == 0) ? a[R1B * c + d] : cmul(a[R1B * c + d], w);
                });
            });
        }
        __syncthreads();
        if (j < R1) {
#pragma unroll
            for (int n2 = 0; n2 < R2; ++n2) out[n2] = buf[j * P1 + n2 * L + l];
            dft_ct<R2A, R2B, +1>(out);
        }
    }
    static __device__ __forceinline__ void forward(cd* buf, const cd* __restrict__ twg, int l, int j, cd (&f)[R2],
                                                   cd (&out)[R1]) {
        if (j < R1) {
            const cd w1 = twg[j], wA = twg[j * R2A];
            dft_ct<R2A, R2B, -1>(f);
            cd wd = make_double2(1.0, 0.0);
            static_for<0, R2B>([&](auto di) {
                constexpr int d = decltype(di)::value;
                if constexpr (d > 0) wd = (d == 1) ? wA : cmul(wd, wA);
                cd w = wd;
                static_for<0, R2A>([&](auto ci) {
                    constexpr int c = decltype(ci)::value;
                    if constexpr (c > 0) w = cmul(w, w1);
                    constexpr int k1p = c + R2A * d;
                    buf[k1p * P2 + j * L + l] = (k1p == 0) ? f[R2B * c + d] : cmul(f[R2B * c + d], make_double2(w.x, -w.y));
                });
            });
        }
        __syncthreads();
        if (j < R2) {
#pragma unroll
            for (int k1 = 0; k1 < R1; ++k1) out[k1] = buf[j * P2 + k1 * L + l];
            dft_ct<R1A, R1B, -1>(out);
        }
    }
};
template <class T>
__device__ __forceinline__ T ld_off(const T* base, unsigned byte_off) {
    return *reinterpret_cast<const T*>(reinterpret_cast<const char*>(base) + byte_off);
}
template <class T>
__device__ __forceinline__ void st_off(T* base, unsigned byte_off, T v) {
    *reinterpret_cast<T*>(reinterpret_cast<char*>(base) + byte_off) = v;
}

template <int R1A, int R1B, int R2A, int R2B>
__global__ __launch_bounds__(FFT_L * ((R1A * R1B > R2A * R2B) ? R1A * R1B : R2A * R2B), ZREG_MIN_BLOCKS)
void k_zpass_reg(FftAxis az, int nx, int nxp, int ny, int nzx, int z_lo, int nbands, const double* __restrict__ Vs,
                 cd* __restrict__ T2, int64_t T2_stride, const FftJob* __restrict__ jobs) {
    typedef FourStep<R1A, R1B, R2A, R2B> FS;
    cd* buf = reinterpret_cast<cd*>(dftk_smem);
    const int tid = threadIdx.x, l = tid & (FFT_L - 1), j = tid >> 3;
    const int xcd = blockIdx.x & 7, slot = blockIdx.x >> 3;
    const int band = slot % nbands;
    const int grp = (slot / nbands) * 8 + xcd;
    const int nxt = nxp / FFT_L;
    if (grp >= nxt * ny) return;
    if (jobs) {
        const FftJob jb = jobs[band];
        nzx = jb.nzx;
        z_lo = jb.z_lo;
        Vs = jb.Vs;
    }
    const int y = grp / nxt;
    const int x = (grp - y * nxt) * FFT_L + l;
    const unsigned plane = (unsigned)ny * (unsigned)nxp;
    const int64_t col0 = (int64_t)y * nxp + (x - l);
    cd* __restrict__ t2 = T2 + (int64_t)band * T2_stride + col0;
    const unsigned planeB = plane * (unsigned)sizeof(cd), stepB = (unsigned)FS::R2 * planeB;
    const unsigned off_lo = (unsigned)j * planeB + (unsigned)l * (unsigned)sizeof(cd);
    const unsigned off_hi = off_lo - (unsigned)(FS::N - nzx) * planeB;
    const int zneg0 = FS::N - (nzx - z_lo);
    auto in = [&](auto ni) -> cd {
        constexpr int n1 = decltype(ni)::value;
        const int e = FS::R2 * n1 + j;
        const bool lo = e < z_lo, hi = e >= zneg0;
        cd v = make_double2(0.0, 0.0);
        if (lo || hi) v = ld_off(t2, (lo ? off_lo : off_hi) + (unsigned)n1 * stepB);
        return v;
    };
    cd psi[FS::R2];
    double vv[FS::R2];
    if (j < FS::R1) {
        const double* __restrict__ vcol = Vs + col0;
        const unsigned vb = ((unsigned)j * plane + (unsigned)l) * 8u;
#pragma unroll
        for (int k2 = 0; k2 < FS::R2; ++k2) vv[k2] = ld_off(vcol, vb + (unsigned)(FS::R1 * k2) * plane * 8u);
    }
    FS::backward(buf, az.tw, l, j, in, psi);
    cd f[FS::R2];
    if (j < FS::R1) {
        static_for<0, FS::R2>([&](auto pi) {
            constexpr int p = decltype(pi)::value;
            constexpr int k2 = FS::k2_of(p);
            f[k2] = make_double2(psi[p].x * vv[k2], psi[p].y * vv[k2]);
        });
    }
    __syncthreads();
    cd out[FS::R1];
    FS::forward(buf, az.tw, l, j, f, out);
    if (j < FS::R2) {
        static_for<0, FS::R1>([&](auto pi) {
            constexpr int p = decltype(pi)::value;
            constexpr int k2p = FS::k2p_of(p);
            const int e = j + FS::R2 * k2p;
            const bool lo = e < z_lo, hi = e >= zneg0;
            if (lo || hi) st_off(t2, (lo ? off_lo : off_hi) + (unsigned)k2p * stepB, out[p]);
        });
    }
}

template <int R1A, int R1B, int R2A, int R2B>
__global__ __launch_bounds__(FFT_L * ((R1A * R1B > R2A * R2B) ? R1A * R1B : R2A * R2B), ZREG_MIN_BLOCKS)
void k_zdensity_reg(FftAxis az, int nx, int nxp, int ny, int nzx, int z_lo, int nb, const double* __restrict__ w,
                    const double* __restrict__ wim, const cd* __restrict__ T2, int64_t T2_stride,
                    double* __restrict__ rho, const FftJob* __restrict__ jobs, double* __restrict__ part,
                    double* __restrict__ rho2 = nullptr) {
    typedef FourStep<R1A, R1B, R2A, R2B> FS;
    cd* buf = reinterpret_cast<cd*>(dftk_smem);
    const int tid = threadIdx.x, l = tid & (FFT_L - 1), j = tid >> 3;
    const int x = blockIdx.x * FFT_L + l;
    const int y = blockIdx.y;
    const unsigned plane = (unsigned)ny * (unsigned)nxp;
    double acc[FS::R2], acc2[FS::R2];
#pragma unroll
    for (int p = 0; p < FS::R2; ++p) acc[p] = acc2[p] = 0.0;
    for (int ib = blockIdx.z; ib < nb; ib += gridDim.z) {
        double wb, wi, wb2 = 0.0;
        if (jobs) {
            const FftJob jb = jobs[ib];
            wb = jb.w;
            wi = jb.wim;
            wb2 = jb.w2;
            nzx = jb.nzx;
            z_lo = jb.z_lo;
        } else {
            wb = w[ib];
            wi = wim ? wim[ib] : wb;
        }
        if (wb == 0.0 && wi == 0.0 && wb2 == 0.0) continue;
        const cd* __restrict__ t2 = T2 + (int64_t)ib * T2_stride + (int64_t)y * nxp + (x - l);
        const unsigned planeB = plane * (unsigned)sizeof(cd), stepB = (unsigned)FS::R2 * planeB;
        const unsigned off_lo = (unsigned)j * planeB + (unsigned)l * (unsigned)sizeof(cd);
        const unsigned off_hi = off_lo - (unsigned)(FS::N - nzx) * planeB;
        const int zneg0 = FS::N - (nzx - z_lo);
        auto in = [&](auto ni) -> cd {
            constexpr int n1 = decltype(ni)::value;
            const int e = FS::R2 * n1 + j;
            const bool lo = e < z_lo, hi = e >= zneg0;
            cd v = make_double2(0.0, 0.0);
            if (lo || hi) v = ld_off(t2, (lo ? off_lo : off_hi) + (unsigned)n1 * stepB);
            return v;
        };
        cd psi[FS::R2];
        FS::backward(buf, az.tw, l, j, in, psi);
        if (j < FS::R1) {
#pragma unroll
            for (int p = 0; p < FS::R2; ++p) {
                acc[p] = fma(wb, psi[p].x * psi[p].x, fma(wi, psi[p].y * psi[p].y, acc[p]));
                if (rho2) acc2[p] = fma(wb2, psi[p].x * psi[p].x + psi[p].y * psi[p].y, acc2[p]);
            }
        }
        __syncthreads();
    }
    if (j < FS::R1 && x < nx) {
        double* __restrict__ r0 = (part ? part + (int64_t)blockIdx.z * az.n * ny * nx : rho) + (int64_t)y * nx + (x - l);
        const unsigned zB = (unsigned)ny * (unsigned)nx * 8u;
        const unsigned ob = (unsigned)j * zB + (unsigned)l * 8u;
        static_for<0, FS::R2>([&](auto pi) {
            constexpr int p = decltype(pi)::value;
            const unsigned off = ob + (unsigned)(FS::R1 * FS::k2_of(p)) * zB;
            st_off(r0, off, part ? acc[p] : ld_off((const double*)r0, off) + acc[p]);
        });
        if (rho2) {
            double* __restrict__ q0 = (part ? part + ((int64_t)gridDim.z + blockIdx.z) * az.n * ny * nx : rho2) + (int64_t)y * nx + (x - l);
            static_for<0, FS::R2>([&](auto pi) {
                constexpr int p = decltype(pi)::value;
                const unsigned off = ob + (unsigned)(FS::R1 * FS::k2_of(p)) * zB;
                st_off(q0, off, part ? acc2[p] : ld_off((const double*)q0, off) + acc2[p]);
            });
        }
    }
}

template <bool GEN>
__global__ __launch_bounds__(FFT_THREADS, YFWD_MIN_BLOCKS) void k_yfwd(FftAxis ay, int nxp, int ny,
                                                      const int* __restrict__ zls,
                                                      const int* __restrict__ line_ypos,
                                                      const cd* __restrict__ T2, int64_t T2_stride,
                                                      cd* __restrict__ T1, int64_t T1_stride,
                                                      const FftJob* __restrict__ jobs) {
    constexpr int FFT_LS = FFT_LS_YZ;
    cd* buf = reinterpret_cast<cd*>(dftk_smem);
    cd* tw = buf + ay.n * FFT_LS;
    const int tid = threadIdx.x, l = tid & (FFT_L - 1), j = tid >> 3;
    const int x = blockIdx.x * FFT_L + l;
    const int zi = blockIdx.y, band = blockIdx.z;
    if (jobs) {
        const FftJob jb = jobs[band];
        if (zi >= jb.nzx) return;
        zls = jb.zls;
        line_ypos = jb.line_ypos;
    }
    tile_prologue<FFT_LS>(buf, tw, ay, false);
    const cd* t2 = T2 + (int64_t)band * T2_stride + (int64_t)zi * ny * nxp + x;
    for (int y = j; y < ny; y += FFT_TPL) buf[y * FFT_LS + l] = t2[(int64_t)y * nxp];
    __syncthreads();
    fft_tile<FFT_LS, true, GEN>(buf, tw, ay, -1.0, l, j);
    cd* t1 = T1 + (int64_t)band * T1_stride;
    const int ln1 = zls[zi + 1];
    for (int ln = zls[zi] + j; ln < ln1; ln += FFT_TPL)
        t1[(int64_t)ln * nxp + x] = buf[line_ypos[ln] * FFT_LS + l];
}

template <bool GEN>
__global__ __launch_bounds__(FFT_THREADS, YFWD_MIN_BLOCKS) void k_xfwd_gather(FftAxis ax, int nxp, int n_lines,
                                                             const int* __restrict__ line_start,
                                                             const int* __restrict__ cpos,
                                                             const cd* __restrict__ T1, int64_t T1_stride,
                                                             const double* __restrict__ kin,
                                                             const cd* __restrict__ psi, int64_t ldpsi,
                                                             cd* __restrict__ out, int64_t ldout,
                                                             const FftJob* __restrict__ jobs,
                                                             const double* __restrict__ shift) {
    constexpr int FFT_LS = FFT_LS_X;
    cd* buf = reinterpret_cast<cd*>(dftk_smem);
    cd* tw = buf + ax.n * FFT_LS;
    const int tid = threadIdx.x, l = tid & (FFT_L - 1), j = tid >> 3;
    const int band = blockIdx.y;
    const int l0 = blockIdx.x * FFT_L;
    const int n = ax.n;
    cd* o = out + (int64_t)band * ldout;
    const cd* p = psi + (int64_t)band * ldpsi;
    if (jobs) {
        const FftJob jb = jobs[band];
        n_lines = jb.n_lines;
        line_start = jb.line_start;
        cpos = jb.cpos;
        kin = jb.kin;
        p = jb.psi;
        o = jb.out;
        if (l0 >= n_lines) return;
    }
    tile_prologue<FFT_LS>(buf, tw, ax, false);
    const cd* in = T1 + (int64_t)band * T1_stride + (int64_t)l0 * nxp;
    const int nlv = min(FFT_L, n_lines - l0);
    for (int idx = tid; idx < FFT_L * nxp; idx += FFT_THREADS) {
        const int ll = idx / nxp;
        const int x = idx - ll * nxp;
        if (x < n) buf[x * FFT_LS + ll] = (ll < nlv) ? in[idx] : make_double2(0.0, 0.0);
    }
    __syncthreads();
    fft_tile<FFT_LS, true, GEN>(buf, tw, ax, -1.0, l, j);
    const int line = l0 + l;
    const double sh = shift ? shift[band] : 0.0;
    if (line < n_lines) {
        const int c0 = line_start[line], c1 = line_start[line + 1];
        for (int c = c0 + j; c < c1; c += FFT_TPL) {
            cd v = buf[cpos[c] * FFT_LS + l];
            if (kin != nullptr) {
                const double k = kin[c] - sh;
                const cd q = p[c];
                v.x = fma(k, q.x, v.x);
                v.y = fma(k, q.y, v.y);
            }
            o[c] = v;
        }
    }
}

template <bool GEN>
__global__ __launch_bounds__(FFT_THREADS, DENS_MIN_BLOCKS) void k_zdensity(FftAxis az, int nx, int nxp, int ny, int nzx,
                                                          const int* __restrict__ zpos, int nb,
                                                          const double* __restrict__ w,
                                                          const double* __restrict__ wim,
                                                          const cd* __restrict__ T2, int64_t T2_stride,
                                                          double* __restrict__ rho, const FftJob* __restrict__ jobs,
                                                          double* __restrict__ part, double* __restrict__ rho2 = nullptr) {
    constexpr int FFT_LS = FFT_LS_YZ;
    cd* buf = reinterpret_cast<cd*>(dftk_smem);
    cd* tw = buf + az.n * FFT_LS;
    const int tid = threadIdx.x, l = tid & (FFT_L - 1), j = tid >> 3;
    const int x = blockIdx.x * FFT_L + l;
    const int y = blockIdx.y;
    const int nz = az.n;
    const int64_t plane = (int64_t)ny * nxp;
    double acc[DENS_MAXACC], acc2[DENS_MAXACC];
#pragma unroll
    for (int k = 0; k < DENS_MAXACC; ++k) acc[k] = acc2[k] = 0.0;
    for (int t = tid; t < nz; t += FFT_THREADS) tw[t] = az.tw[t];
    for (int ib = blockIdx.z; ib < nb; ib += gridDim.z) {
        double wb, wi, wb2 = 0.0;
        if (jobs) {
            const FftJob jb = jobs[ib];
            wb = jb.w;
            wi = jb.wim;
            wb2 = jb.w2;
            zpos = jb.zpos;
            nzx = jb.nzx;
        } else {
            wb = w[ib];
            wi = wim ? wim[ib] : wb;
        }
        if (wb == 0.0 && wi == 0.0 && wb2 == 0.0) continue;
        const cd z0 = make_double2(0.0, 0.0);
        for (int t = tid; t < nz * FFT_LS; t += FFT_THREADS) buf[t] = z0;
        __syncthreads();
        const cd* t2 = T2 + (int64_t)ib * T2_stride + (int64_t)y * nxp + x;
        for (int zi = j; zi < nzx; zi += FFT_TPL) buf[zpos[zi] * FFT_LS + l] = t2[(int64_t)zi * plane];
        __syncthreads();
        fft_tile<FFT_LS, false, GEN>(buf, tw, az, +1.0, l, j);
#pragma unroll
        for (int k = 0; k < DENS_MAXACC; ++k) {
            const int z = j + k * FFT_TPL;
            if (z < nz) {
                const cd v = buf[z * FFT_LS + l];
                acc[k] = fma(wb, v.x * v.x, fma(wi, v.y * v.y, acc[k]));
                if (rho2) acc2[k] = fma(wb2, v.x * v.x + v.y * v.y, acc2[k]);
            }
        }
        __syncthreads();
    }
    if (x < nx) {
        double* __restrict__ dst = part ? part + (int64_t)blockIdx.z * nz * ny * nx : rho;
#pragma unroll
        for (int k = 0; k < DENS_MAXACC; ++k) {
            const int z = j + k * FFT_TPL;
            if (z < nz) {
                const int64_t at = ((int64_t)z * ny + y) * nx + x;
                dst[at] = part ? acc[k] : dst[at] + acc[k];
            }
        }
        if (rho2) {
            double* __restrict__ dst2 = part ? part + ((int64_t)gridDim.z + blockIdx.z) * nz * ny * nx : rho2;
#pragma unroll
            for (int k = 0; k < DENS_MAXACC; ++k) {
                const int z = j + k * FFT_TPL;
                if (z < nz) {
                    const int64_t at = ((int64_t)z * ny + y) * nx + x;
                    dst2[at] = part ? acc2[k] : dst2[at] + acc2[k];
                }
            }
        }
    }
}

template <bool GEN>
__global__ __launch_bounds__(FFT_THREADS, DENS_MIN_BLOCKS) void k_zdensity_response(FftAxis az, int nx, int nxp, int ny,
                                                                   int nzx, const int* __restrict__ zpos, int nb,
                                                                   const double* __restrict__ wo,
                                                                   const double* __restrict__ wd,
                                                                   const cd* __restrict__ T2, int64_t T2_stride,
                                                                   double* __restrict__ drho) {
    constexpr int FFT_LS = FFT_LS_YZ;
    cd* buf = reinterpret_cast<cd*>(dftk_smem);
    cd* tw = buf + az.n * FFT_LS;
    const int tid = threadIdx.x, l = tid & (FFT_L - 1), j = tid >> 3;
    const int x = blockIdx.x * FFT_L + l;
    const int y = blockIdx.y;
    const int nz = az.n;
    const int64_t plane = (int64_t)ny * nxp;
    double acc[DENS_MAXACC];
    cd pv[DENS_MAXACC];
#pragma unroll
    for (int k = 0; k < DENS_MAXACC; ++k) acc[k] = 0.0;
    for (int t = tid; t < nz; t += FFT_THREADS) tw[t] = az.tw[t];
    const cd z0 = make_double2(0.0, 0.0);
    for (int ib = 0; ib < nb; ++ib) {
        const double w2 = 2.0 * wo[ib], w1 = wd[ib];
        if (w2 == 0.0 && w1 == 0.0) continue;
        for (int t = tid; t < nz * FFT_LS; t += FFT_THREADS) buf[t] = z0;
        __syncthreads();
        const cd* t2 = T2 + (int64_t)ib * T2_stride + (int64_t)y * nxp + x;
        for (int zi = j; zi < nzx; zi += FFT_TPL) buf[zpos[zi] * FFT_LS + l] = t2[(int64_t)zi * plane];
        __syncthreads();
        fft_tile<FFT_LS, false, GEN>(buf, tw, az, +1.0, l, j);
#pragma unroll
        for (int k = 0; k < DENS_MAXACC; ++k) {
            const int z = j + k * FFT_TPL;
            pv[k] = z < nz ? buf[z * FFT_LS + l] : z0;
            acc[k] = fma(w1, pv[k].x * pv[k].x + pv[k].y * pv[k].y, acc[k]);
        }
        __syncthreads();
        if (w2 == 0.0) continue;
        for (int t = tid; t < nz * FFT_LS; t += FFT_THREADS) buf[t] = z0;
        __syncthreads();
        const cd* d2 = T2 + (int64_t)(nb + ib) * T2_stride + (int64_t)y * nxp + x;
        for (int zi = j; zi < nzx; zi += FFT_TPL) buf[zpos[zi] * FFT_LS + l] = d2[(int64_t)zi * plane];
        __syncthreads();
        fft_tile<FFT_LS, false, GEN>(buf, tw, az, +1.0, l, j);
#pragma unroll
        for (int k = 0; k < DENS_MAXACC; ++k) {
            const int z = j + k * FFT_TPL;
            if (z < nz) {
                const cd v = buf[z * FFT_LS + l];
                acc[k] = fma(w2, pv[k].x * v.x + pv[k].y * v.y, acc[k]);
            }
        }
        __syncthreads();
    }
    if (x < nx) {
#pragma unroll
        for (int k = 0; k < DENS_MAXACC; ++k) {
            const int z = j + k * FFT_TPL;
            if (z < nz) drho[((int64_t)z * ny + y) * nx + x] += acc[k];
        }
    }
}

__global__ void k_dens_reduce(int64_t n, int ngroups, const double* __restrict__ part, double* __restrict__ rho) {
    const int64_t i = (int64_t)blockIdx.x * blockDim.x + threadIdx.x;
    if (i >= n) return;
    double s = 0.0;
    for (int g = 0; g < ngroups; ++g) s += part[(int64_t)g * n + i];
    rho[i] += s;
}

__global__ void k_pad_potential(int nx, int nxp, int64_t rows, double scale, const double* __restrict__ V,
                                double* __restrict__ Vs) {
    const int64_t i = (int64_t)blockIdx.x * blockDim.x + threadIdx.x;
    if (i >= rows * nxp) return;
    const int64_t r = i / nxp;
    const int x = (int)(i - r * nxp);
    Vs[i] = (x < nx) ? V[r * nx + x] * scale : 0.0;
}

__global__ void k_kinetic(int64_t n, int nb, const double* __restrict__ kin, const cd* __restrict__ psi,
                          int64_t ldpsi, cd* __restrict__ out, int64_t ldout, int accumulate) {
    const int64_t i = (int64_t)blockIdx.x * blockDim.x + threadIdx.x;
    if (i >= n) return;
    const double k = kin ? kin[i] : 0.0;
    for (int b = 0; b < nb; ++b) {
        cd q = psi[(int64_t)b * ldpsi + i];
        cd v = make_double2(k * q.x, k * q.y);
        if (accumulate) {
            cd o = out[(int64_t)b * ldout + i];
            v.x += o.x;
            v.y += o.y;
        }
        out[(int64_t)b * ldout + i] = v;
    }
}

static size_t lds_bytes(int n, int ls = FFT_LS_YZ) { return (size_t)n * (ls + 1) * sizeof(cd); }

int fft_ensure_scratch(dftk_mi_basis* b, dftk_mi_kblock* kb, int nb) {
    const size_t t1 = (size_t)nb * kb->n_lines * b->nxp * sizeof(cd);
    const size_t t2 = (size_t)nb * kb->nzx * b->ny * b->nxp * sizeof(cd);
    HIPCHK(b->T1.reserve(t1));
    HIPCHK(b->T2.reserve(t2));
    return 0;
}

static int check_lds(dftk_mi_basis* b) {
    const int nmax = b->nx > b->ny ? (b->nx > b->nz ? b->nx : b->nz) : (b->ny > b->nz ? b->ny : b->nz);
    if (lds_bytes(nmax, FFT_LS_X) > 160 * 1024) {
        dftk_set_error("FFT axis length %d needs %zu B of LDS (> 160 KiB)", nmax, lds_bytes(nmax, FFT_LS_X));
        return DFTK_MI_EINVAL;
    }
    return 0;
}

template <typename K>
static int set_lds_attr(K kernel, size_t bytes) {
    if (bytes > 64 * 1024) {
        HIPCHK(hipFuncSetAttribute(reinterpret_cast<const void*>(kernel),
                                   hipFuncAttributeMaxDynamicSharedMemorySize, (int)bytes));
    }
    return 0;
}

static bool axis_generic(const FftAxis& ax) {
    for (int s = 0; s < ax.nrad; ++s)
        if (ax.rad[s] > 5 && ax.rad[s] != 6 && ax.rad[s] != 8) return true;
    return false;
}

#define LAUNCH_FFT(KERNEL, AX, GRID, LDS, STREAM, ...)                                       \
    do {                                                                                     \
        if (axis_generic(AX)) {                                                              \
            constexpr bool GEN = true;                                                       \
            CHK(set_lds_attr(KERNEL, LDS));                                                  \
            hipLaunchKernelGGL(KERNEL, GRID, dim3(FFT_THREADS), LDS, STREAM, __VA_ARGS__);   \
        } else {                                                                             \
            constexpr bool GEN = false;                                                      \
            CHK(set_lds_attr(KERNEL, LDS));                                                  \
            hipLaunchKernelGGL(KERNEL, GRID, dim3(FFT_THREADS), LDS, STREAM, __VA_ARGS__);   \
        }                                                                                    \
    } while (0)

static FftJob kblock_tables(const dftk_mi_kblock* kb) {
    FftJob j{};
    j.line_start = kb->d_line_start;
    j.cpos = kb->d_cpos;
    j.line_ypos = kb->d_line_ypos;
    j.zls = kb->d_zls;
    j.zpos = kb->d_zpos;
    j.z_lo = kb->z_lo;
    j.Vs = kb->d_Vs;
    j.n_lines = (int)kb->n_lines;
    j.nzx = kb->nzx;
    return j;
}

struct FftPipe {
    dftk_mi_basis* b;
    hipStream_t stream;
    int nb;
    cd *T1, *T2;
    int64_t s1, s2;
    int n_lines, nzx;
    FftJob tab;
    const FftJob* jobs;
    bool reg_z;
    bool book;
    int64_t n_G;
};
static FftPipe kblock_pipe(dftk_mi_kblock* kb, int nb, int t_off = 0, cd* planes = nullptr) {
    dftk_mi_basis* b = kb->basis;
    const int64_t s1 = (int64_t)kb->n_lines * b->nxp, s2 = (int64_t)kb->nzx * b->ny * b->nxp;
    return FftPipe{b, b->stream, nb, b->T1 + t_off * s1, planes ? planes : b->T2 + t_off * s2, s1, s2, (int)kb->n_lines,
                   kb->nzx, kblock_tables(kb), nullptr, kb->z_lo >= 0, true, kb->n_G};
}
static FftPipe jobs_pipe(dftk_mi_basis* b, hipStream_t stream, int nb, const FftJob* jobs, cd* T1, cd* T2, int64_t s1,
                         int64_t s2, int max_lines, int max_nzx, bool reg_z) {
    return FftPipe{b, stream, nb, T1, T2, s1, s2, max_lines, max_nzx, FftJob{}, jobs, reg_z, false, 0};
}

#define REG_SIZES(X)                                                                                                      \
    X(24, 2, 2, 3, 2) X(27, 3, 3, 3, 1) X(30, 5, 1, 3, 2) X(32, 2, 2, 4, 2) X(36, 3, 2, 3, 2) X(40, 2, 2, 5, 2) X(48, 3, 2, 4, 2) X(54, 3, 2, 3, 3)           \
    X(45, 3, 3, 5, 1) X(50, 5, 2, 5, 1) X(60, 3, 2, 5, 2)                                                                 \
    X(64, 4, 2, 4, 2) X(72, 3, 3, 4, 2) X(80, 5, 2, 4, 2) X(90, 5, 2, 3, 3) X(96, 4, 3, 4, 2) X(100, 5, 2, 5, 2)          \
    X(108, 4, 3, 3, 3) X(120, 4, 3, 5, 2) X(128, 4, 4, 4, 2) X(144, 4, 3, 4, 3) X(150, 5, 3, 5, 2) X(160, 4, 4, 5, 2)     \
    X(180, 5, 3, 4, 3) X(192, 4, 4, 4, 3) X(200, 5, 4, 5, 2) X(216, 6, 3, 4, 3) X(240, 4, 4, 5, 3) X(256, 4, 4, 4, 4)
static bool fft_reg_on(int n) {
    static const bool off = getenv("DFTK_MI_FFT_REG") != nullptr && atoi(getenv("DFTK_MI_FFT_REG")) == 0;
    static const int nmin = getenv("DFTK_MI_FFT_REG_MIN") ? atoi(getenv("DFTK_MI_FFT_REG_MIN")) : 24;
    return !off && n >= nmin;
}
static bool fft_reg_fits(const dftk_mi_basis* b) {
    return (uint64_t)b->nz * (uint64_t)b->ny * (uint64_t)b->nxp * sizeof(cd) < (1ull << 32);
}
template <bool DENS, int A, int B, int C, int D>
static int reg_launch_t(const FftPipe& p, dim3 grid, const double* w, const double* wim, double* rho, double* part,
                        double* rho2) {
    typedef FourStep<A, B, C, D> FS;
    const dftk_mi_basis* b = p.b;
    const size_t lds = (size_t)FS::LDS_ELEMS * sizeof(cd);
    if constexpr (DENS) {
        CHK(set_lds_attr(k_zdensity_reg<A, B, C, D>, lds));
        hipLaunchKernelGGL((k_zdensity_reg<A, B, C, D>), grid, dim3(FS::THREADS), lds, p.stream, b->ax[2], b->nx, b->nxp, b->ny,
                           p.tab.nzx, p.tab.z_lo, p.nb, w, wim, (const cd*)p.T2, p.s2, rho, p.jobs, part, rho2);
    } else {
        CHK(set_lds_attr(k_zpass_reg<A, B, C, D>, lds));
        hipLaunchKernelGGL((k_zpass_reg<A, B, C, D>), grid, dim3(FS::THREADS), lds, p.stream, b->ax[2], b->nx, b->nxp, b->ny,
                           p.tab.nzx, p.tab.z_lo, p.nb, p.tab.Vs, p.T2, p.s2, p.jobs);
    }
    return 0;
}
template <bool DENS>
static int reg_launch(const FftPipe& p, dim3 grid, const double* w = nullptr, const double* wim = nullptr, double* rho = nullptr,
                      double* part = nullptr, double* rho2 = nullptr) {
    if (!p.reg_z || !fft_reg_on(p.b->nz) || !fft_reg_fits(p.b)) return 1;
    switch (p.b->nz) {
#define X(NN, A, B, C, D) case NN: return reg_launch_t<DENS, A, B, C, D>(p, grid, w, wim, rho, part, rho2);
        REG_SIZES(X)
#undef X
        default: return 1;
    }
}
template int reg_launch<false>(const FftPipe&, dim3, const double*, const double*, double*, double*, double*);
template int reg_launch<true>(const FftPipe&, dim3, const double*, const double*, double*, double*, double*);

static double t1_bytes(const FftPipe& p) { return 16.0 * (double)p.s1; }
static double t2_bytes(const FftPipe& p) { return 16.0 * (double)p.s2; }
static int book(const FftPipe& p, int fam, double bytes) { return p.book ? prof_begin(p.b, fam, bytes) : -1; }

static int stage_A(const FftPipe& p, const cd* psi, int64_t ldpsi, int pair_nb = 0) {
    const dftk_mi_basis* b = p.b;
    if (pair_nb > 0) {
        if (p.jobs || (pair_nb + 1) / 2 != p.nb) {
            dftk_set_error("stage A: a band pair per transform needs the single-block pipeline and nb = ceil(pair_nb / 2)");
            return DFTK_MI_EINVAL;
        }
        const int ps = book(p, PROF_FFT_A, 16.0 * p.n_G * pair_nb + t1_bytes(p) * p.nb);
        LAUNCH_FFT((k_xbwd_scatter<GEN, true>), b->ax[0], dim3((p.n_lines + FFT_L - 1) / FFT_L, p.nb), lds_bytes(b->nx, FFT_LS_X),
                   p.stream, b->ax[0], b->nxp, p.tab.n_lines, p.tab.line_start, p.tab.cpos, psi, ldpsi, p.T1, p.s1, p.jobs, pair_nb);
        prof_end(p.b, ps);
        return 0;
    }
    const int ps = book(p, PROF_FFT_A, (16.0 * p.n_G + t1_bytes(p)) * p.nb);
    LAUNCH_FFT((k_xbwd_scatter<GEN>), b->ax[0], dim3((p.n_lines + FFT_L - 1) / FFT_L, p.nb), lds_bytes(b->nx, FFT_LS_X),
               p.stream, b->ax[0], b->nxp, p.tab.n_lines, p.tab.line_start, p.tab.cpos, psi, ldpsi, p.T1, p.s1, p.jobs, 0);
    prof_end(p.b, ps);
    return 0;
}
static int stage_B(const FftPipe& p) {
    const dftk_mi_basis* b = p.b;
    const int ps = book(p, PROF_FFT_B, (t1_bytes(p) + t2_bytes(p)) * p.nb);
    LAUNCH_FFT((k_ybwd<GEN>), b->ax[1], dim3(b->nxp / FFT_L, p.nzx, p.nb), lds_bytes(b->ny), p.stream, b->ax[1], b->nxp,
               b->ny, p.tab.zls, p.tab.line_ypos, (const cd*)p.T1, p.s1, p.T2, p.s2, p.jobs);
    prof_end(p.b, ps);
    return 0;
}
static int stage_D(const FftPipe& p) {
    const dftk_mi_basis* b = p.b;
    const int ps = book(p, PROF_FFT_D, (t1_bytes(p) + t2_bytes(p)) * p.nb);
    LAUNCH_FFT((k_yfwd<GEN>), b->ax[1], dim3(b->nxp / FFT_L, p.nzx, p.nb), lds_bytes(b->ny), p.stream, b->ax[1], b->nxp,
               b->ny, p.tab.zls, p.tab.line_ypos, (const cd*)p.T2, p.s2, p.T1, p.s1, p.jobs);
    prof_end(p.b, ps);
    return 0;
}
static int stage_E(const FftPipe& p, const double* kin, const cd* psi, int64_t ldpsi, cd* out, int64_t ldout,
                   const double* shift_d) {
    const dftk_mi_basis* b = p.b;
    const int ps = book(p, PROF_FFT_E, (t1_bytes(p) + (kin ? 40.0 : 16.0) * p.n_G) * p.nb);
    LAUNCH_FFT((k_xfwd_gather<GEN>), b->ax[0], dim3((p.n_lines + FFT_L - 1) / FFT_L, p.nb), lds_bytes(b->nx, FFT_LS_X),
               p.stream, b->ax[0], b->nxp, p.tab.n_lines, p.tab.line_start, p.tab.cpos, (const cd*)p.T1, p.s1, kin, psi,
               ldpsi, out, ldout, p.jobs, shift_d);
    prof_end(p.b, ps);
    return 0;
}

static dim3 zpass_grid(const dftk_mi_basis* b, int nbands) {
    const int64_t groups = (int64_t)(b->nxp / FFT_L) * b->ny;
    return dim3((unsigned)(((groups + 7) / 8) * 8 * nbands));
}

static int stage_C(const FftPipe& p) {
    const dftk_mi_basis* b = p.b;
    const dim3 grid = zpass_grid(b, p.nb);
    const int ps = book(p, PROF_FFT_C, 2.0 * t2_bytes(p) * p.nb + 8.0 * (double)b->nz * b->ny * b->nxp);
    const int rs = reg_launch<false>(p, grid);
    if (rs < 0) return rs;
    if (rs == 1)
        LAUNCH_FFT((k_zpass<0, GEN>), b->ax[2], grid, lds_bytes(b->nz), p.stream, b->ax[2], b->nx, b->nxp, b->ny, p.tab.nzx,
                   p.nb, p.tab.zpos, p.tab.Vs, p.T2, p.s2, (cd*)nullptr, p.jobs);
    prof_end(p.b, ps);
    return 0;
}
template <int MODE>
static int stage_z_cube(const FftPipe& p, cd* cube) {
    const dftk_mi_basis* b = p.b;
    LAUNCH_FFT((k_zpass<MODE, GEN>), b->ax[2], zpass_grid(b, p.nb), lds_bytes(b->nz), p.stream, b->ax[2], b->nx, b->nxp,
               b->ny, p.tab.nzx, p.nb, p.tab.zpos, (const double*)nullptr, p.T2, p.s2, cube, p.jobs);
    return 0;
}
int launch_ifft_to_cube(dftk_mi_kblock* kb, const cd* c, cd* cube, int nb) {
    dftk_mi_basis* b = kb->basis;
    CHK(check_lds(b));
    CHK(fft_ensure_scratch(b, kb, nb));
    const FftPipe p = kblock_pipe(kb, nb);
    CHK(stage_A(p, c, kb->n_G));
    CHK(stage_B(p));
    CHK(stage_z_cube<1>(p, cube));
    HIPCHK(hipGetLastError());
    return 0;
}

int launch_fft_from_cube(dftk_mi_kblock* kb, const cd* cube, cd* c, int nb) {
    dftk_mi_basis* b = kb->basis;
    CHK(check_lds(b));
    CHK(fft_ensure_scratch(b, kb, nb));
    const FftPipe p = kblock_pipe(kb, nb);
    CHK(stage_z_cube<2>(p, const_cast<cd*>(cube)));
    CHK(stage_D(p));
    CHK(stage_E(p, nullptr, c, kb->n_G, c, kb->n_G, nullptr));
    HIPCHK(hipGetLastError());
    return 0;
}

static int stage_density(const FftPipe& p, const double* w, const double* wim, double* rho, int groups = 1,
                         double* part = nullptr, double* rho2 = nullptr) {
    const dftk_mi_basis* b = p.b;
    const dim3 grid(b->nxp / FFT_L, b->ny, groups);
    const int ps = book(p, PROF_DENS_Z, t2_bytes(p) * p.nb + 16.0 * (double)b->nx * b->ny * b->nz);
    const int rs = reg_launch<true>(p, grid, w, wim, rho, part, rho2);
    if (rs < 0) return rs;
    if (rs == 1)
        LAUNCH_FFT((k_zdensity<GEN>), b->ax[2], grid, lds_bytes(b->nz), p.stream, b->ax[2], b->nx, b->nxp, b->ny, p.tab.nzx,
                   p.tab.zpos, p.nb, w, wim, (const cd*)p.T2, p.s2, rho, p.jobs, part, rho2);
    prof_end(p.b, ps);
    return 0;
}
static int stage_density_response(const FftPipe& p, const double* wo, const double* wd, double* drho) {
    const dftk_mi_basis* b = p.b;
    const int ps = book(p, PROF_DENS_Z, 2.0 * t2_bytes(p) * p.nb + 16.0 * (double)b->nx * b->ny * b->nz);
    LAUNCH_FFT((k_zdensity_response<GEN>), b->ax[2], dim3(b->nxp / FFT_L, b->ny), lds_bytes(b->nz), p.stream, b->ax[2], b->nx,
               b->nxp, b->ny, p.tab.nzx, p.tab.zpos, p.nb, wo, wd, (const cd*)p.T2, p.s2, drho);
    prof_end(p.b, ps);
    return 0;
}

int fft_group_size(const dftk_mi_basis* b) { return std::max(1, b->fft_batch); }

template <class F>
static int band_groups(dftk_mi_kblock* kb, int nb, int slots, const double* wa_h, const double* wb_h, F&& body) {
    dftk_mi_basis* b = kb->basis;
    const int group = std::max(1, b->fft_batch / slots);
    CHK(fft_ensure_scratch(b, kb, slots * std::min(nb, group)));
    double* d = nullptr;
    if (wa_h) {
        CHK(ensure_ws(b, 2 * (size_t)nb * sizeof(double)));
        d = reinterpret_cast<double*>(b->ws.get());
        HIPCHK(hipMemcpyAsync(d, wa_h, (size_t)nb * sizeof(double), hipMemcpyHostToDevice, b->stream));
        if (wb_h) HIPCHK(hipMemcpyAsync(d + nb, wb_h, (size_t)nb * sizeof(double), hipMemcpyHostToDevice, b->stream));
    }
    for (int b0 = 0; b0 < nb; b0 += group) {
        const int nbb = std::min(group, nb - b0);
        bool any = !wa_h;
        for (int i = 0; i < nbb && !any; ++i) any = wa_h[b0 + i] != 0.0 || (wb_h && wb_h[b0 + i] != 0.0);
        if (!any) continue;
        CHK(body(b0, nbb, d ? d + b0 : nullptr, wb_h ? d + nb + b0 : nullptr));
    }
    HIPCHK(hipGetLastError());
    return 0;
}

int launch_local_apply(dftk_mi_kblock* kb, int nb, const cd* psi, int64_t ldpsi, cd* out, int64_t ldout,
                       bool add_kinetic, bool have_local, const double* shift_d) {
    dftk_mi_basis* b = kb->basis;
    if (shift_d && (!add_kinetic || !have_local || kb->d_Vs == nullptr)) {
        dftk_set_error("launch_local_apply: the per-band shift rides on the kinetic term of the gather pass");
        return DFTK_MI_EINVAL;
    }
    if (!have_local || kb->d_Vs == nullptr) {
        return launch_kinetic_only(kb, nb, psi, ldpsi, out, ldout, false, add_kinetic);
    }
    CHK(check_lds(b));
    return band_groups(kb, nb, 1, nullptr, nullptr, [&](int b0, int nbb, const double*, const double*) -> int {
        const FftPipe p = kblock_pipe(kb, nbb);
        const cd* in = psi + (int64_t)b0 * ldpsi;
        CHK(stage_A(p, in, ldpsi));
        CHK(stage_B(p));
        CHK(stage_C(p));
        CHK(stage_D(p));
        return stage_E(p, add_kinetic ? kb->d_kin : nullptr, in, ldpsi, out + (int64_t)b0 * ldout, ldout,
                       shift_d ? shift_d + b0 : nullptr);
    });
}

int launch_planes_fill(dftk_mi_kblock* kb, int b0, int nbb, const cd* psi, int64_t ldpsi, cd* planes, int pair_nb) {
    dftk_mi_basis* b = kb->basis;
    CHK(check_lds(b));
    CHK(fft_ensure_scratch(b, kb, nbb));
    const int64_t s2 = (int64_t)kb->nzx * b->ny * b->nxp;
    const FftPipe p = kblock_pipe(kb, nbb, 0, planes + (int64_t)b0 * s2);
    CHK(stage_A(p, psi, ldpsi, pair_nb));
    CHK(stage_B(p));
    HIPCHK(hipGetLastError());
    return 0;
}

int launch_local_apply_from_planes(dftk_mi_kblock* kb, int nb, cd* planes, cd* out, int64_t ldout) {
    dftk_mi_basis* b = kb->basis;
    if (kb->d_Vs == nullptr) {
        dftk_set_error("launch_local_apply_from_planes: no local potential is bound");
        return DFTK_MI_EINVAL;
    }
    CHK(check_lds(b));
    const int64_t s2 = (int64_t)kb->nzx * b->ny * b->nxp;
    return band_groups(kb, nb, 1, nullptr, nullptr, [&](int b0, int nbb, const double*, const double*) -> int {
        const FftPipe p = kblock_pipe(kb, nbb, 0, planes + (int64_t)b0 * s2);
        cd* o = out + (int64_t)b0 * ldout;
        CHK(stage_C(p));
        CHK(stage_D(p));
        return stage_E(p, nullptr, o, ldout, o, ldout, nullptr);
    });
}

int launch_kinetic_only(dftk_mi_kblock* kb, int nb, const cd* psi, int64_t ldpsi, cd* out, int64_t ldout,
                        bool accumulate, bool use_kin) {
    dftk_mi_basis* b = kb->basis;
    const int threads = 256;
    const int blocks = (int)((kb->n_G + threads - 1) / threads);
    hipLaunchKernelGGL(k_kinetic, dim3(blocks), dim3(threads), 0, b->stream, kb->n_G, nb,
                       use_kin ? kb->d_kin : (const double*)nullptr, psi, ldpsi, out, ldout, accumulate ? 1 : 0);
    HIPCHK(hipGetLastError());
    return 0;
}

static int check_density_nz(const dftk_mi_basis* b) {
    if (b->nz > DENS_MAXACC * FFT_TPL) {
        dftk_set_error("density kernel supports nz <= %d", DENS_MAXACC * FFT_TPL);
        return DFTK_MI_EINVAL;
    }
    return 0;
}

int launch_density(dftk_mi_kblock* kb, int nb, const cd* psi, int64_t ldpsi, const double* w_h, double* rho,
                   const double* w_im_h, const double* w2_h, double* rho2, bool keep_planes, int pair_nb) {
    dftk_mi_basis* b = kb->basis;
    if (pair_nb > 0 && (batching() || w2_h || (pair_nb + 1) / 2 != nb)) {
        dftk_set_error("launch_density: a band pair per transform is a one-weight pass of nb = ceil(pair_nb / 2) transforms "
                       "outside a batched call");
        return DFTK_MI_EINVAL;
    }
    if (!keep_planes) kb->ho.planes_off();
    if (batching() && nb > 0) {
        BOp o;
        o.b = b;
        o.kb = kb;
        o.type = BOP_DENSITY; o.m = nb; o.A = psi; o.lda = ldpsi; o.C = rho; o.D = w2_h ? rho2 : nullptr;
        o.flags = (w_im_h ? 1 : 0) | (w2_h ? 2 : 0);
        o.payload.resize((size_t)(1 + (w_im_h ? 1 : 0) + (w2_h ? 1 : 0)) * nb * sizeof(double));
        memcpy(o.payload.data(), w_h, (size_t)nb * sizeof(double));
        size_t at = (size_t)nb * sizeof(double);
        if (w_im_h) {
            memcpy(o.payload.data() + at, w_im_h, (size_t)nb * sizeof(double));
            at += (size_t)nb * sizeof(double);
        }
        if (w2_h) memcpy(o.payload.data() + at, w2_h, (size_t)nb * sizeof(double));
        return batch_record(std::move(o));
    }
    if (w2_h) {
        CHK(launch_density(kb, nb, psi, ldpsi, w_h, rho, w_im_h, nullptr, nullptr));
        return launch_density(kb, nb, psi, ldpsi, w2_h, rho2, nullptr, nullptr, nullptr);
    }
    CHK(check_lds(b));
    CHK(check_density_nz(b));
    const int64_t s2 = (int64_t)kb->nzx * b->ny * b->nxp;
    return band_groups(kb, nb, 1, w_h, w_im_h, [&](int b0, int nbb, const double* w_d, const double* wim_d) -> int {
        const FftPipe p = kblock_pipe(kb, nbb, 0, keep_planes ? kb->ho.planes + (int64_t)b0 * s2 : nullptr);
        if (pair_nb > 0)
            CHK(stage_A(p, psi + (int64_t)(2 * b0) * ldpsi, ldpsi, std::min(2 * nbb, pair_nb - 2 * b0)));
        else
            CHK(stage_A(p, psi + (int64_t)b0 * ldpsi, ldpsi));
        CHK(stage_B(p));
        if (keep_planes) kb->ho.planes_mark(b0, nbb);
        return stage_density(p, w_d, wim_d, rho);
    });
}

int launch_density_response(dftk_mi_kblock* kb, int nb, const cd* psi, int64_t ldpsi, const cd* dpsi, int64_t lddpsi,
                            const double* wo_h, const double* wd_h, double* drho) {
    dftk_mi_basis* b = kb->basis;
    CHK(check_lds(b));
    CHK(check_density_nz(b));
    return band_groups(kb, nb, 2, wo_h, wd_h, [&](int b0, int nbb, const double* wo_d, const double* wd_d) -> int {
        const FftPipe p = kblock_pipe(kb, nbb), pd = kblock_pipe(kb, nbb, nbb);
        CHK(stage_A(p, psi + (int64_t)b0 * ldpsi, ldpsi));
        CHK(stage_B(p));
// ... 170 lines not shown
```

### dftk.jl_amd/csrc/gamma_kernels.hip

```cpp
#include "common.h"
#include "batch.h"
#include <algorithm>
#include <cmath>
#include <cstdio>
#include <cstdlib>
#include <unordered_map>
#include <vector>

int gamma_tables_host(int nx, int ny, int nz, int64_t n_G, const int64_t* mapping, int64_t* n_half_out, int32_t* g,
                      int32_t* mg) {
    if (n_G < 1 || mapping[0] != 0) {
        dftk_set_error("gamma_real: the sphere must contain G = 0 as its first entry");
        return DFTK_MI_EINVAL;
    }
    std::unordered_map<int64_t, int32_t> row;
    row.reserve((size_t)n_G * 2);
    for (int64_t c = 0; c < n_G; ++c) row[mapping[c]] = (int32_t)c;
    int64_t nh = 0;
    for (int64_t c = 0; c < n_G; ++c) {
        const int64_t lin = mapping[c];
        const int ix = (int)(lin % nx), iy = (int)((lin / nx) % ny), iz = (int)(lin / ((int64_t)nx * ny));
        const int64_t mlin = (int64_t)((nx - ix) % nx) + (int64_t)nx * (((ny - iy) % ny) + (int64_t)ny * ((nz - iz) % nz));
        auto it = row.find(mlin);
        if (it == row.end()) {
// ... 406 lines not shown
int gamma_projectors_renew(dftk_mi_kblock* kb, size_t elems) {
    HIPCHK(hipStreamSynchronize(kb->basis->stream));
    HIPCHK(kb->gr->P_half.alloc(elems * sizeof(cd)));
    return 0;
}

static int gr_projectors(dftk_mi_kblock* kb) {
    GammaReal* gr = kb->gr.get();
    if (gr->P_src == kb->P && gr->P_n_p == kb->n_p && gr->P_half) return 0;
    if (kb->sh_comm) return gamma_projectors_sharded(kb);
    CHK(gamma_projectors_renew(kb, (size_t)gr->n_half * kb->n_p));
    double h[2];
    CHK(gamma_gather_P(kb, kb->n_p, kb->P, kb->ldP, gr->P_half, gr->n_half, h));
    if (!(std::isfinite(h[1]) && h[0] <= 1e-10 * (h[1] > 0 ? h[1] : 1.0))) {
        dftk_set_error("gamma_real: the projectors are not real-symmetric (max |P(-G) - conj P(G)| = %.3e, max |P| = %.3e)",
                       h[0], h[1]);
        gr->P_half.reset();
        return DFTK_MI_EINVAL;
    }
    gr->P_src = kb->P;
    gr->P_n_p = kb->n_p;
    return 0;
}

int gamma_projectors(dftk_mi_kblock* kb) { return gr_projectors(kb); }

int gamma_pack_pairs(dftk_mi_kblock* kb, int nb, const cd* H, int64_t ldh, cd* Z, int64_t ldz) {
    if (nb <= 0) return 0;
    GammaReal* gr = kb->gr.get();
    ProfScope prof_scope(kb->basis, PROF_EW, 32.0 * (double)gr->n_half * nb);
    hipLaunchKernelGGL(k_gr_pack, gr_grid_unr(gr->n_half, (nb + 1) / 2), dim3(256), 0, kb->basis->stream, gr->n_half, nb,
                       gr->d_g, gr->d_mg, H, ldh, Z, ldz);
    HIPCHK(hipGetLastError());
    return 0;
}
int gamma_unpack_pairs(dftk_mi_kblock* kb, int nb, const cd* W, int64_t ldw, cd* H, int64_t ldh, const cd* add, int64_t ldadd) {
    if (nb <= 0) return 0;
    GammaReal* gr = kb->gr.get();
    ProfScope prof_scope(kb->basis, PROF_EW, (add ? 48.0 : 32.0) * (double)gr->n_half * nb);
    if (add)
        hipLaunchKernelGGL(k_gr_unpack<true>, gr_grid_unr(gr->n_half, (nb + 1) / 2), dim3(256), 0, kb->basis->stream, gr->n_half,
                           nb, gr->d_g, gr->d_mg, W, ldw, H, ldh, add, ldadd);
    else
        hipLaunchKernelGGL(k_gr_unpack<false>, gr_grid_unr(gr->n_half, (nb + 1) / 2), dim3(256), 0, kb->basis->stream, gr->n_half,
                           nb, gr->d_g, gr->d_mg, W, ldw, H, ldh, add, ldadd);
    HIPCHK(hipGetLastError());
    return 0;
}
int gamma_pack_full(dftk_mi_kblock* kb, int nb, const cd* X, int64_t ldx, cd* Z, int64_t ldz) {
    if (nb <= 0) return 0;
    ProfScope prof_scope(kb->basis, PROF_EW, 32.0 * (double)kb->n_G * nb);
    hipLaunchKernelGGL(k_gr_pack_full, gr_grid_unr(kb->n_G, (nb + 1) / 2), dim3(256), 0, kb->basis->stream, kb->n_G, nb, X,
                       ldx, Z, ldz);
    HIPCHK(hipGetLastError());
    return 0;
}

int gamma_apply_H(dftk_mi_kblock* kb, int which, int nb, const cd* psi, int64_t ldpsi, cd* Hpsi, int64_t ldH, const cd* add,
                  int64_t ldadd) {
    if (nb <= 0) return 0;
    if (kb->d_Vtau) {
        dftk_set_error("gamma_apply_H: the block has a tau potential bound (meta-GGA): the Gamma-real format does not know the "
                       "div-A-grad term");
        return DFTK_MI_EINVAL;
    }
    if (add && (kb->sh_comm || (which & 4))) {
        dftk_set_error("gamma_apply_H: an addend goes with the local and kinetic parts of an un-sharded block only");
        return DFTK_MI_EINVAL;
    }
    if (kb->sh_comm) return gamma_apply_H_sharded(kb, which, nb, psi, ldpsi, Hpsi, ldH);
    GammaReal* gr = kb->gr.get();
    dftk_mi_basis* b = kb->basis;
    const int nb2 = (nb + 1) / 2;
    const bool local = (which & 1) && kb->d_Vs != nullptr;
    const bool kinetic = which & 2;
    const int slot = prof_begin(b, PROF_APPLY_H, (double)nb);
    struct G {
        dftk_mi_basis* b;
        int s;
        ~G() { prof_end(b, s); }
    } guard{b, slot};
    CHK(gamma_ensure_buf(kb, 2 * (size_t)kb->n_G * nb2));
    cd* Z = gr->buf;
    cd* W = gr->buf + (size_t)kb->n_G * nb2;
    prof_count(b, PROF_A2A_MODEL, 16.0 * (double)gr->n_half * nb);
    prof_count(b, PROF_A2A_MODEL, 16.0 * (double)gr->n_half * nb);
    if ((which & 4) && kb->n_p > 0) prof_count(b, PROF_AR_MODEL, 16.0 * (double)kb->n_p * nb);
    CHK(gamma_pack_pairs(kb, nb, psi, ldpsi, Z, kb->n_G));
    CHK(launch_local_apply(kb, nb2, Z, kb->n_G, W, kb->n_G, kinetic, local));
    CHK(gamma_unpack_pairs(kb, nb, W, kb->n_G, Hpsi, ldH, add, ldadd));
    if ((which & 4) && kb->n_p > 0) {
        CHK(gr_projectors(kb));
        CHK(apply_nonlocal_rows(kb, nb, gr->P_half, gr->n_half, gr->n_half, psi, ldpsi, Hpsi, ldH, true,
                                DFTK_MI_GEMM_REAL, nullptr));
    }
    return 0;
}

int gamma_density(dftk_mi_kblock* kb, int nb, const cd* psi, int64_t ldpsi, const double* w_h, double* rho) {
    if (nb <= 0) return 0;
    if (!kb->gr) {
        kb->gr.reset(new GammaReal());
    }
    if (kb->sh_comm) return gamma_density_sharded(kb, nb, psi, ldpsi, w_h, rho);
    return gamma_density_bands(kb, nb, psi, ldpsi, w_h, rho);
}

static bool planes_wanted() {
    const char* e = getenv("DFTK_MI_PLANES_REUSE");
    return !(e && atoi(e) == 0);
}

bool planes_eligible(const dftk_mi_kblock* kb) {
    return planes_wanted() && kb->gr && kb->gr->on && !kb->sh_comm && !batching();
}

static int planes_prepare(dftk_mi_kblock* kb, int nb, const cd* psi, int64_t ldpsi, bool* keep) {
    *keep = false;
    dftk_mi_basis* b = kb->basis;
    LobHandover& ho = kb->ho;
    if (!planes_eligible(kb) || !ho.pass_keeps_planes(psi, ldpsi, nb)) return 0;
    const size_t nb2 = (size_t)(nb + 1) / 2;
    const size_t need = nb2 * (size_t)kb->nzx * b->ny * b->nxp * sizeof(cd);
    if (need > ho.planes.bytes()) {
        HIPCHK(hipStreamSynchronize(b->stream));
        HIPCHK(ho.planes.reset());
        size_t free_b = 0, total_b = 0;
        HIPCHK(hipMemGetInfo(&free_b, &total_b));
        if (free_b < 2 * need + ((size_t)1 << 30) || ho.planes.reserve(need) != hipSuccess) {
            (void)hipGetLastError();
            ho.planes_decline();
            return 0;
        }
    }
    *keep = true;
    return 0;
}

int gamma_density_bands(dftk_mi_kblock* kb, int nb, const cd* psi, int64_t ldpsi, const double* w_h, double* rho) {
    if (nb <= 0) return 0;
    const int nb2 = (nb + 1) / 2;
    bool keep = false;
    CHK(planes_prepare(kb, nb, psi, ldpsi, &keep));
    const bool pairs_in_A = land_in_place() && !batching();
    if (!pairs_in_A) {
        CHK(gamma_ensure_buf(kb, (size_t)kb->n_G * nb2));
        CHK(gamma_pack_full(kb, nb, psi, ldpsi, kb->gr->buf, kb->n_G));
    }
    std::vector<double> wre(nb2), wim(nb2);
    for (int p = 0; p < nb2; ++p) {
        wre[p] = w_h[2 * p];
        wim[p] = (2 * p + 1 < nb) ? w_h[2 * p + 1] : 0.0;
    }
    if (keep) kb->ho.planes_begin(nb, kb->basis->fft_batch);
    if (pairs_in_A) return launch_density(kb, nb2, psi, ldpsi, wre.data(), rho, wim.data(), nullptr, nullptr, keep, nb);
    return launch_density(kb, nb2, kb->gr->buf, kb->n_G, wre.data(), rho, wim.data(), nullptr, nullptr, keep);
}

int gamma_apply_local_from_planes(dftk_mi_kblock* kb, int nb, const cd* X, int64_t ldx, cd* Hpsi, int64_t ldH, const cd* add,
                                  int64_t ldadd) {
    if (nb <= 0) return 0;
    GammaReal* gr = kb->gr.get();
    dftk_mi_basis* b = kb->basis;
    const int nb2 = (nb + 1) / 2;
    const std::vector<char>& valid = kb->ho.planes_consume();
    const int slot = prof_begin(b, PROF_APPLY_H, (double)nb);
    struct G {
        dftk_mi_basis* b;
        int s;
        ~G() { prof_end(b, s); }
    } guard{b, slot};
    const bool pairs_in_A = land_in_place();
    CHK(gamma_ensure_buf(kb, (pairs_in_A ? 1 : 2) * (size_t)kb->n_G * nb2));
    cd* Z = gr->buf;
    cd* W = pairs_in_A ? gr->buf.get() : gr->buf + (size_t)kb->n_G * nb2;
    prof_count(b, PROF_A2A_MODEL, 16.0 * (double)gr->n_half * nb);
    prof_count(b, PROF_A2A_MODEL, 16.0 * (double)gr->n_half * nb);
    const int group = fft_group_size(b);
    for (int b0 = 0; b0 < nb2; b0 += group) {
        const int nbb = std::min(group, nb2 - b0);
        if (std::all_of(valid.begin() + b0, valid.begin() + b0 + nbb, [](char v) { return v != 0; })) continue;
        const int ncol = std::min(2 * nbb, nb - 2 * b0);
        if (pairs_in_A) {
            CHK(launch_planes_fill(kb, b0, nbb, X + (int64_t)(2 * b0) * ldx, ldx, kb->ho.planes, ncol));
            continue;
        }
        CHK(gamma_pack_full(kb, ncol, X + (int64_t)(2 * b0) * ldx, ldx, Z, kb->n_G));
        CHK(launch_planes_fill(kb, b0, nbb, Z, kb->n_G, kb->ho.planes));
    }
    CHK(launch_local_apply_from_planes(kb, nb2, kb->ho.planes, W, kb->n_G));
    return gamma_unpack_pairs(kb, nb, W, kb->n_G, Hpsi, ldH, add, ldadd);
}
```

### dftk.jl_amd/csrc/handover.h

```cpp
#pragma once
#include <algorithm>
#include <vector>
#include "devbuf.h"

typedef double2 cd;

struct LobHandover {
    DevTable<double> V_kept;
    DevTable<double> dV;
    DevTable<cd> planes;

    struct Taken {
        cd* AX = nullptr;
        int64_t ld = 0;
        bool planes = false;
    };

    void promise(bool on) { promised_ = on && kept_ != nullptr; }

    Taken take(int M, int64_t N, bool workspace_moves, bool planes_eligible, int fft_batch) {
        Taken t;
        if (promised_ && kept_M_ == M && kept_N_ == N && !workspace_moves) {
            t.AX = kept_;
            t.ld = kept_ld_;
            t.planes = planes_eligible && on_ && planes != nullptr && back_M_ == M && batch_ == fft_batch &&
                       valid_.size() == (size_t)(M + 1) / 2;
        }
        promised_ = false;
        kept_ = nullptr;
        forget_planes();
        return t;
    }

    void keep(cd* AX, int64_t ld, int M, int64_t N) {
        kept_ = AX;
        kept_ld_ = ld;
        kept_M_ = M;
        kept_N_ = N;
    }
    void returned(const cd* X, int64_t ld, int M) {
        back_X_ = X;
        back_ld_ = ld;
        back_M_ = M;
    }

    void forget() {
        kept_ = nullptr;
        promised_ = false;
        forget_planes();
    }
    void forget_planes() {
        on_ = false;
        back_X_ = nullptr;
    }

    bool pass_keeps_planes(const cd* psi, int64_t ld, int nb) const {
        return !declined_ && back_X_ != nullptr && back_X_ == psi && back_ld_ == ld && back_M_ == nb;
    }
    void planes_begin(int nb, int fft_batch) {
        valid_.assign((size_t)(nb + 1) / 2, 0);
        batch_ = fft_batch;
        on_ = true;
    }
    void planes_mark(int p0, int n) { std::fill_n(valid_.begin() + p0, n, (char)1); }
    void planes_off() { on_ = false; }
    const std::vector<char>& planes_consume() {
        on_ = false;
        return valid_;
    }
    void planes_decline() { declined_ = true; }

    void set_last_AX(cd* AX) { last_AX_ = AX; }
    cd* last_AX() const { return last_AX_; }

private:
    cd* last_AX_ = nullptr;
    cd* kept_ = nullptr;
    int kept_M_ = 0;
    int64_t kept_N_ = 0, kept_ld_ = 0;
    bool promised_ = false;
    const cd* back_X_ = nullptr;
    int64_t back_ld_ = 0;
    int back_M_ = 0;
    bool on_ = false;
    bool declined_ = false;
    int batch_ = 0;
    std::vector<char> valid_;
};
```

### dftk.jl_amd/csrc/lobpcg.cpp

```cpp
#include "common.h"
#include "batch.h"
#include <cstdio>
#include <cstdlib>
#include <algorithm>
#include <atomic>
#include <cmath>
#include <complex>
#include <cstring>
#include <functional>
#include <numeric>
#include <random>
#include <utility>
#include <vector>

std::atomic<int64_t> g_ax_reuse_count{0};
std::atomic<int64_t> g_planes_reuse_count{0};

namespace {

const double EPS = 2.220446049250313e-16;
const double ORTHO_TOL = 2 * EPS;
const int64_t DEFER_FETCH_MAX_ELEMS = 1 << 16;
const cd ONE = {1.0, 0.0}, ZERO = {0.0, 0.0}, MONE = {-1.0, 0.0};

// ... 397 lines not shown
                    const double re = nd(*gen), im = nd(*gen);
                    X[i + (size_t)j * n] = zd(re, real ? 0.0 : im);
                }
                for (int a = 0; a < ny; ++a) {
                    zd s = 0.0;
                    for (int i = 0; i < n; ++i) s += std::conj(Y[i + (size_t)a * n]) * X[i + (size_t)j * n];
                    BYX[a + (size_t)j * ny] = s;
                }
                for (int a = 0; a < ny; ++a) {
                    const zd s = BYX[a + (size_t)j * ny];
                    for (int i = 0; i < n; ++i) X[i + (size_t)j * n] -= Y[i + (size_t)a * n] * s;
                }
            }
        }
        if (std::sqrt(byx2) < tol && niter > 1) break;
        double growth = 1.0;
        for (int pass = 0;; ++pass) {
            if (pass >= 30) {
                *why = 2;
                return 0;
            }
            for (int j = 0; j < m; ++j)
                for (int i = 0; i <= j; ++i) {
                    zd s = 0.0;
                    for (int r = 0; r < n; ++r) s += std::conj(X[r + (size_t)i * n]) * X[r + (size_t)j * n];
                    O[i + (size_t)j * m] = (i == j) ? zd(s.real(), 0.0) : s;
                }
            std::fill(R.begin(), R.end(), zd(0.0));
            for (int j = 0; j < m; ++j) {
                for (int i = 0; i < j; ++i) {
                    zd s = O[i + (size_t)j * m];
                    for (int k = 0; k < i; ++k) s -= std::conj(R[k + (size_t)i * m]) * R[k + (size_t)j * m];
                    R[i + (size_t)j * m] = s / R[i + (size_t)i * m].real();
                }
                double d = O[j + (size_t)j * m].real();
                for (int k = 0; k < j; ++k) d -= std::norm(R[k + (size_t)j * m]);
                if (!(d > 0.0) || !std::isfinite(d)) {
                    *why = 3;
                    return 0;
                }
                R[j + (size_t)j * m] = std::sqrt(d);
            }
            std::fill(Ri.begin(), Ri.end(), zd(0.0));
            for (int j = 0; j < m; ++j) {
                Ri[j + (size_t)j * m] = 1.0 / R[j + (size_t)j * m].real();
                for (int i = j - 1; i >= 0; --i) {
                    zd s = 0.0;
                    for (int k = i + 1; k <= j; ++k) s += R[i + (size_t)k * m] * Ri[k + (size_t)j * m];
                    Ri[i + (size_t)j * m] = -s / R[i + (size_t)i * m].real();
                }
            }
            const double nR = normest(R), nI = normest(Ri);
            if (!std::isfinite(nR) || !std::isfinite(nI)) {
                *why = 4;
                return 0;
            }
            for (int j = 0; j < m; ++j)
                for (int i = 0; i < n; ++i) {
                    zd s = 0.0;
                    for (int k = 0; k <= j; ++k) s += X[i + (size_t)k * n] * Ri[k + (size_t)j * m];
                    T[i + (size_t)j * n] = s;
                }
            X.swap(T);
            growth *= nI;
            const double condR = nR * nI;
            if (EPS * condR * condR < tol) break;
        }
        if (growth * EPS < tol) break;
        if (niter > 10) {
            *why = 5;
            return 0;
        }
    }
    Xio.swap(X);
    return 1;
}
const size_t HOST_CP_MAX_ELEMS = 2048;

int hcat_mul(Ctx& c, const Mat& Y, const cd* coef, int64_t ldcoef, int ncols, Mat C) {
    return c.mm('N', Y.rows, ncols, Y.cols, ONE, Y.p, Y.ld, coef, ldcoef, ZERO, C.p, C.ld);
}

struct NoComm {
    Ctx& c;
    dftk_mi_comm* saved;
    int saved_rf;
    explicit NoComm(Ctx& ctx) : c(ctx), saved(ctx.comm), saved_rf(ctx.rf) {
        c.comm = nullptr;
        c.replicated = saved != nullptr;
        c.small = true;
        c.rf = 0;
    }
    ~NoComm() {
        c.comm = saved;
        c.replicated = false;
        c.small = false;
        c.rf = saved_rf;
    }
};

struct Lob {
    Ctx c;
    dftk_mi_kblock* kb = nullptr;
    dftk_mi_basis* b = nullptr;
    int M = 0;
    int64_t N = 0;
    const double* kin = nullptr;
    Mat Yb[2], AYb[2], newR;
    cd *tmp = nullptr, *G = nullptr, *V = nullptr, *cP = nullptr;
    int DS = 0;
    double *dd = nullptr, *d_norms = nullptr, *d_mk = nullptr, *d_xx = nullptr, *d_lam = nullptr, *d_rn = nullptr;
    int* d_perm = nullptr;
    std::vector<double> hf;
    cd* kept_AX = nullptr;
    int64_t kept_ld = 0;
    bool kept_planes = false;
    std::vector<double> resid_history, full_lam;
    double& RH(int i, int it) { return resid_history[(size_t)i + (size_t)M * it]; }
    int cur = 0;
    int nlocked = 0, niter = 0, lo = 0, final_iter = 0;
    bool finished = false;
    int64_t n_matvec = 0;
    int nact = 0, nY = 0;
    Mat X, AX, Xa, AXa, Ra, ARa, nX, nAX, nR;
    Mat Y, AY;
    std::vector<zd> h_cX;
    bool host_cp = false;
    int ncx = 0;
    int newly_locked = 0, lenXn = 0, tgt = 0;
    Mat nP, nAP, Rn;
    std::vector<int> perm;

    Mat Pblk(const Mat& buf, int na) const { return buf.cols_from(M, na); }
    Mat Rblk(const Mat& buf, int na, bool has_p) const { return buf.cols_from(M + (has_p ? na : 0), na); }

    int bind(dftk_mi_kblock* kb_, int M_, int64_t N_, int dstride, dftk_mi_comm* comm, bool real_mode, const double* kin_,
             uint64_t seed, int maxiter) {
        kb = kb_;
        b = kb->basis;
        M = M_;
        N = N_;
        kin = kin_;
        DS = dstride;
        const size_t blk = (size_t)N * M;
        const size_t nbig = 14;
        const size_t m3 = 3 * (size_t)M;
        const size_t small_elems = m3 * m3 * 2
                                   + m3 * M * 2
                                   + (size_t)M * M * 4
                                   + (2 * (size_t)M + m3) * (M + 1);
        const size_t dbl = 9 * (size_t)DS;
        const size_t need = (nbig * blk + small_elems) * sizeof(cd) + dbl * sizeof(double) + m3 * sizeof(int) + 1024;
        const bool grows = need > kb->lob_buf.bytes();
        const LobHandover::Taken kept = kb->ho.take(M, N, grows, planes_eligible(kb), b->fft_batch);
        kept_AX = kept.AX;
        kept_ld = kept.ld;
        kept_planes = kept.planes;
        if (grows) {
            CHK(host_wait(b));
            HIPCHK(kb->lob_buf.reserve(need));
        }
        cd* w = kb->lob_buf;
        auto take = [&](size_t n) {
            cd* r = w;
            w += n;
            return r;
        };
        for (Mat& m : Yb) m = Mat{take(3 * blk), N, N, 3 * M};
        for (Mat& m : AYb) m = Mat{take(3 * blk), N, N, 3 * M};
        newR = Mat{take(blk), N, N, M};
        tmp = take(blk);
        G = take(m3 * m3);
        V = take(m3 * m3);
        cP = take(m3 * M);
        c.kb = kb;
        c.b = b;
        c.comm = comm;
        c.real_mode = real_mode;
        c.holds_g0 = real_mode && gamma_row0(kb) == 0;
        c.rf = real_mode ? DFTK_MI_GEMM_REAL : 0;
        c.tmpS = take(m3 * M);
        c.O = take((size_t)M * M);
        c.Rw = take((size_t)M * M);
        c.invR = take((size_t)M * M);
        c.Vh = take((size_t)M * M);
        c.BYX = take((2 * (size_t)M + m3) * (M + 1));
        dd = reinterpret_cast<double*>(w);
        c.d_a = dd;
        c.d_b = dd + DS;
        c.dstride = DS;
        d_norms = dd + 2 * DS;
        d_mk = dd + 3 * DS;
        d_xx = dd + 4 * DS;
        d_lam = dd + 5 * DS;
        d_rn = dd + 6 * DS;
        d_perm = reinterpret_cast<int*>(dd + 7 * DS);
        hf.assign(5 * (size_t)DS, 0.0);
        c.rng.seed((seed ? seed : 0x9E3779B97F4A7C15ull) + 0x632BE59BD9B4E019ull * (uint64_t)comm_rank(comm));
        c.rng_rep.seed((seed ? seed : 0x9E3779B97F4A7C15ull) ^ 0xD1B54A32D192ED03ull);
        X = Yb[0].cols_from(0, M);
        AX = AYb[0].cols_from(0, M);
        kb->ho.set_last_AX(real_mode ? nullptr : AX.p);
        resid_history.assign((size_t)M * (maxiter + 1), 0.0);
        full_lam.assign(M, 0.0);
        final_iter = maxiter;
        n_matvec = M;
        return 0;
    }

    int apply_H(int nb, const cd* in, int64_t ldin, cd* out, int64_t ldout) {
        if (c.real_mode) return gamma_apply_H(kb, 7, nb, in, ldin, out, ldout);
        return dftk_mi_apply_H(kb, nb, reinterpret_cast<const dftk_mi_cplx*>(in), ldin,
                               reinterpret_cast<dftk_mi_cplx*>(out), ldout);
    }

    int kept_times_invR() {
        if (kept_AX != AX.p) return c.mm('N', N, M, M, ONE, kept_AX, kept_ld, c.invR, M, ZERO, AX.p, AX.ld, 2);
        CHK(c.mm('N', N, M, M, ONE, kept_AX, kept_ld, c.invR, M, ZERO, newR.p, newR.ld, 2));
        return ew_copy(b, N, M, newR.p, newR.ld, AX.p, AX.ld);
    }

    int start_AX(const cd* Xp, int64_t ldX) {
        LobHandover& ho = kb->ho;
        bool reuse_ax = kept_AX != nullptr && kb->d_Vs != nullptr && ho.V_kept != nullptr && kb->d_Vtau == nullptr;
        const bool lip = land_in_place();
        cd* const X0 = lip ? tmp : X.p;
        if (c.real_mode)
            CHK(gamma_lobpcg_load(kb, M, Xp, ldX, X0, X.ld, true));
        else
            CHK(ew_copy(b, N, M, Xp, ldX, X0, X.ld));
        {
            int nch;
            double gr;
            CHK(ortho_X(c, X, tmp, ORTHO_TOL, &nch, &gr, true, 0, false, nullptr, nullptr, X0));
            if (reuse_ax && !(nch == 1)) reuse_ax = false;
        }
        if (!reuse_ax) return apply_H(M, X.p, X.ld, AX.p, AX.ld);
        g_ax_reuse_count.fetch_add(1);
        const size_t cube = (size_t)b->nz * b->ny * b->nxp;
        if (!ho.dV) HIPCHK(ho.dV.alloc(cube * sizeof(double)));
        CHK(ew_sub_real(b, (int64_t)cube, kb->d_Vs, ho.V_kept, ho.dV));
        double* const Vs_bound = kb->d_Vs;
        if (kept_planes) {
            g_planes_reuse_count.fetch_add(1);
            kb->d_Vs = ho.dV;
            if (lip) {
                const Mat S = kept_AX == AX.p ? newR : Mat{kept_AX, kept_ld, N, M};
                const int st_dv = gamma_apply_local_from_planes(kb, M, Xp, ldX, S.p, S.ld, kept_AX, kept_ld);
                kb->d_Vs = Vs_bound;
                CHK(st_dv);
                CHK(c.mm('N', N, M, M, ONE, S.p, S.ld, c.invR, M, ZERO, AX.p, AX.ld, 2));
            } else {
                const int st_dv = gamma_apply_local_from_planes(kb, M, Xp, ldX, newR.p, newR.ld);
                kb->d_Vs = Vs_bound;
                CHK(st_dv);
                CHK(ew_add(b, N, M, newR.p, newR.ld, kept_AX, kept_ld));
                CHK(kept_times_invR());
            }
        } else if (lip) {
            const Mat Pr = kept_AX == AX.p ? newR : AX;
            CHK(c.mm('N', N, M, M, ONE, kept_AX, kept_ld, c.invR, M, ZERO, Pr.p, Pr.ld, 2));
            kb->d_Vs = ho.dV;
            int st_dv;
            if (c.real_mode && !kb->sh_comm) {
                st_dv = gamma_apply_H(kb, 1, M, X.p, X.ld, AX.p, AX.ld, Pr.p, Pr.ld);
                kb->d_Vs = Vs_bound;
                CHK(st_dv);
            } else {
                const Mat Dl = kept_AX == AX.p ? AX : newR;
                st_dv = c.real_mode ? gamma_apply_H(kb, 1, M, X.p, X.ld, Dl.p, Dl.ld)
                                    : dftk_mi_apply_H_parts(kb, 1, M, reinterpret_cast<const dftk_mi_cplx*>(X.p), X.ld,
                                                            reinterpret_cast<dftk_mi_cplx*>(Dl.p), Dl.ld);
                kb->d_Vs = Vs_bound;
                CHK(st_dv);
                CHK(ew_add(b, N, M, newR.p, newR.ld, AX.p, AX.ld));
            }
        } else {
            CHK(kept_times_invR());
            kb->d_Vs = ho.dV;
            const int st_dv = c.real_mode ? gamma_apply_H(kb, 1, M, X.p, X.ld, newR.p, newR.ld)
                                          : dftk_mi_apply_H_parts(kb, 1, M, reinterpret_cast<const dftk_mi_cplx*>(X.p), X.ld,
                                                                  reinterpret_cast<dftk_mi_cplx*>(newR.p), newR.ld);
            kb->d_Vs = Vs_bound;
            CHK(st_dv);
            CHK(ew_add(b, N, M, newR.p, newR.ld, AX.p, AX.ld));
        }
        static const bool ax_check = getenv("DFTK_MI_AX_REUSE_CHECK") != nullptr;
        if (ax_check) {
            CHK(apply_H(M, X.p, X.ld, newR.p, newR.ld));
            std::vector<cd> h1((size_t)N * M), h2((size_t)N * M);
            CHK(stream_sync(b));
            HIPCHK(hipMemcpy(h1.data(), AX.p, h1.size() * sizeof(cd), hipMemcpyDeviceToHost));
            HIPCHK(hipMemcpy(h2.data(), newR.p, h2.size() * sizeof(cd), hipMemcpyDeviceToHost));
            double worst = 0.0, nrm = 0.0;
            int wc = -1;
            for (int j = 0; j < M; ++j) {
                double d = 0.0, r = 0.0;
                for (int64_t i = 0; i < N; ++i) {
                    const cd a = h1[(size_t)i + (size_t)j * N], f = h2[(size_t)i + (size_t)j * N];
                    d += (a.x - f.x) * (a.x - f.x) + (a.y - f.y) * (a.y - f.y);
                    r += f.x * f.x + f.y * f.y;
                }
                nrm = std::max(nrm, std::sqrt(r));
                if (std::sqrt(d) > worst) {
                    worst = std::sqrt(d);
                    wc = j;
                }
// ... 562 lines not shown
```

### include/dftk_mi355x.h

```cpp
#ifndef DFTK_MI355X_H
#define DFTK_MI355X_H

#include <stddef.h>
#include <stdint.h>

#ifdef __cplusplus
extern "C" {
#endif

typedef struct { double re, im; } dftk_mi_cplx;

typedef struct dftk_mi_basis  dftk_mi_basis;
typedef struct dftk_mi_kblock dftk_mi_kblock;
typedef struct dftk_mi_comm   dftk_mi_comm;

#define DFTK_MI_OK                 0
#define DFTK_MI_EINVAL            (-1)
#define DFTK_MI_EHIP              (-2)
#define DFTK_MI_ERCCL             (-3)
#define DFTK_MI_ENOGPU            (-100)
#define DFTK_MI_NUM_NONFINITE       1
#define DFTK_MI_NUM_CHOLESKY        2
#define DFTK_MI_NUM_NORMALIZATION   3
#define DFTK_MI_NUM_EIGEN           4
#define DFTK_MI_NUM_TOO_SMALL       5
#define DFTK_MI_NUM_RANK_DEFICIENT  6

const char* dftk_mi_last_error(void);
const char* dftk_mi_version(void);

int dftk_mi_basis_create(int nx, int ny, int nz, double unit_cell_volume, int device,
                         dftk_mi_basis** basis_out);
int dftk_mi_basis_destroy(dftk_mi_basis* basis);
int dftk_mi_basis_sync(dftk_mi_basis* basis);
int dftk_mi_basis_set_fft_batch(dftk_mi_basis* basis, int n_bands_per_batch);
void* dftk_mi_basis_stream(dftk_mi_basis* basis);

int dftk_mi_kblock_create(dftk_mi_basis* basis, int64_t n_G, const int64_t* mapping0_h,
                          const double* kinetic_h ,
                          dftk_mi_kblock** kb_out);
int dftk_mi_kblock_destroy(dftk_mi_kblock* kb);
int dftk_mi_kblock_set_projectors(dftk_mi_kblock* kb, int n_p, const dftk_mi_cplx* P_d, int64_t ldP,
                                  const double* D_h);
int dftk_mi_kblock_set_potential(dftk_mi_kblock* kb, const double* V_d);
int dftk_mi_kblocks_set_potential(int n_kblocks, dftk_mi_kblock* const* kbs, const double* V_d);
int dftk_mi_kblock_set_kpoint(dftk_mi_kblock* kb, const double* recip_lattice_h, const double* kcoord_h);
int dftk_mi_kblock_set_tau_potential(dftk_mi_kblock* kb, const double* Vtau_d);
int dftk_mi_kblocks_set_tau_potential(int n_kblocks, dftk_mi_kblock* const* kbs, const double* Vtau_d);

int dftk_mi_apply_H(dftk_mi_kblock* kb, int n_bands, const dftk_mi_cplx* psi_d, int64_t ld_psi,
                    dftk_mi_cplx* Hpsi_d, int64_t ld_Hpsi);
int dftk_mi_apply_H_parts(dftk_mi_kblock* kb, int which, int n_bands, const dftk_mi_cplx* psi_d,
                          int64_t ld_psi, dftk_mi_cplx* Hpsi_d, int64_t ld_Hpsi);

int dftk_mi_kpoint_sphere_host(int nx, int ny, int nz, const double* recip_lattice_h, const double* kcoord_h,
                               double Ecut, int64_t cap, int64_t* n_G, int64_t* mapping0_h, double* kinetic_h,
                               int32_t* G_h);
int dftk_mi_build_projectors_hgh(dftk_mi_basis* basis, int64_t n_rows, const int32_t* G_d,
                                 const double* recip_lattice_h, const double* kcoord_h, double unit_cell_volume,
                                 int n_species, const double* rp_h, const int* n_proj_h, int n_atoms,
                                 const int* species_of_atom_h, const double* positions_h, dftk_mi_cplx* P_d,
                                 int64_t ldP, int* n_p);

int dftk_mi_atomic_superposition(dftk_mi_kblock* cube_kb, int kind, const double* recip_lattice_h, int n_species,
                                 const double* params_h, int n_atoms, const int* species_of_atom_h,
                                 const double* positions_h, double* out_d);
int dftk_mi_forces_local(dftk_mi_kblock* cube_kb, const double* recip_lattice_h, int n_species, const double* params_h,
                         int n_atoms, const int* species_of_atom_h, const double* positions_h, const double* rho_d,
                         double* forces_h);
int dftk_mi_radial_transform(dftk_mi_basis* basis, int kind, int l, int n_r, const double* r_h, const double* wf_h,
                             double Zion, int64_t n_q, const double* q_d, double* out_d);
int dftk_mi_radial_tile(void);
int dftk_mi_build_projectors_radial(dftk_mi_basis* basis, int64_t n_rows, const int32_t* G_d,
                                    const double* recip_lattice_h, const double* kcoord_h, double unit_cell_volume,
                                    int n_species, const double* R_d, int64_t ldR, const int* first_chan_h,
                                    const int* n_chan_h, int n_atoms, const int* species_of_atom_h,
                                    const double* positions_h, dftk_mi_cplx* P_d, int64_t ldP, int* n_p);
int dftk_mi_atomic_superposition_table(dftk_mi_kblock* cube_kb, const double* recip_lattice_h, int n_species,
                                       const double* ff_d, int n_atoms, const int* species_of_atom_h,
                                       const double* positions_h, const double* coeff_h, double* out_d);
int dftk_mi_forces_local_table(dftk_mi_kblock* cube_kb, const double* recip_lattice_h, int n_species, const double* ff_d,
                               int n_atoms, const int* species_of_atom_h, const double* positions_h,
                               const double* rho_d, double* forces_h);
int dftk_mi_forces_nonlocal(dftk_mi_kblock* kb, const double* kcoord_h, int n_bands, const dftk_mi_cplx* psi_d,
                            int64_t ld_psi, const double* weight_h, int n_atoms, const int* col_start_h,
                            double* forces_h);

int dftk_mi_local_potential_displacement(dftk_mi_kblock* cube_kb, const double* recip_lattice_h, int n_species,
                                         const double* params_h, int species, const double* position_h, double* out_d);
int dftk_mi_dynmat_local(dftk_mi_kblock* cube_kb, const double* recip_lattice_h, int n_species, const double* params_h,
                         int n_atoms, const int* species_of_atom_h, const double* positions_h, const double* rho_d,
                         double* out_h);
int dftk_mi_nonlocal_displacement_apply(dftk_mi_kblock* kb, const double* kcoord_h, int atom, int n_atoms,
                                        const int* col_start_h, int n_bands, const dftk_mi_cplx* psi_d, int64_t ld_psi,
                                        dftk_mi_cplx* out_d, int64_t ld_out);
int dftk_mi_dynmat_nonlocal(dftk_mi_kblock* kb, const double* kcoord_h, int n_bands, const dftk_mi_cplx* psi_d,
                            int64_t ld_psi, const dftk_mi_cplx* dpsi_d, int64_t ld_dpsi, const double* w_h,
                            const double* wd_h, int n_atoms, const int* col_start_h, double* dforces_h, double* hess_h);

int dftk_mi_stress_kinetic_nonlocal(dftk_mi_kblock* kb, const double* recip_lattice_h, const double* kcoord_h,
                                    int n_bands, const dftk_mi_cplx* psi_d, int64_t ld_psi, const double* weight_h,
                                    int n_species, const double* rp_h, const int* n_proj_h, int n_atoms,
                                    const int* species_of_atom_h, const double* positions_h, const int* col_start_h,
                                    double* stress_h);
int dftk_mi_stress_cube(dftk_mi_kblock* cube_kb, const double* recip_lattice_h, int n_species, const double* params_h,
                        int n_atoms, const int* species_of_atom_h, const double* positions_h, const double* rho_d,
                        double* out_h);
int dftk_mi_stress_xc(dftk_mi_basis* basis, int64_t n, int n_spin, const double* rho_d, const double* vrho_d,
                      const double* e_d, const double* vsigma_d, const double* grad_d, double* out_h);

#define DFTK_MI_XC_LDA_X     1
#define DFTK_MI_XC_LDA_C_VWN 2
#define DFTK_MI_XC_LDA_C_PW  4
#define DFTK_MI_XC_LDA_XC_TETER93 32
int dftk_mi_local_potential(dftk_mi_kblock* cube_kb, const double* rho_d, const double* V_loc_d,
                            const double* poisson_green_d, int xc_functionals, double* V_out_d, double* energies_h);

int dftk_mi_local_potential_collinear(dftk_mi_kblock* cube_kb, const double* rho_d, const double* V_loc_d,
                                      const double* poisson_green_d, int xc_functionals, double* V_out_d,
                                      double* energies_h);

int dftk_mi_local_potential_gga(dftk_mi_kblock* cube_kb, const double* recip_lattice_h, const double* rho_d,
                                const double* V_loc_d, const double* poisson_green_d, int xc_functionals,
                                double density_threshold, double* V_out_d, double* energies_h);

int dftk_mi_local_potential_mgga(dftk_mi_kblock* cube_kb, const double* recip_lattice_h, const double* rho_d,
                                 const double* tau_d, const double* V_loc_d, const double* poisson_green_d, int xc_functionals,
                                 double density_threshold, double* V_out_d, double* Vtau_out_d, double* energies_h);

int dftk_mi_local_potential_collinear_gga(dftk_mi_kblock* cube_kb, const double* recip_lattice_h, const double* rho_d,
                                          const double* V_loc_d, const double* poisson_green_d, int xc_functionals,
                                          double density_threshold, double* V_out_d, double* energies_h);

int dftk_mi_local_potential_core(dftk_mi_kblock* cube_kb, const double* recip_lattice_h, int n_spin, const double* rho_d,
                                 const double* rho_core_d, const double* grad_core_d, const double* V_loc_d,
                                 const double* poisson_green_d, int xc_functionals, double density_threshold,
                                 double* V_out_d, double* energies_h);
int dftk_mi_cube_gradient(dftk_mi_kblock* cube_kb, const double* recip_lattice_h, const double* f_d, double* grad_d);

int dftk_mi_symmetrize_rho(dftk_mi_kblock* cube_kb, int n_sym, const int32_t* S_h, const double* tau_h, int do_lowpass,
                           const double* rho_in_d, double* rho_out_d);
int dftk_mi_mix_kerker(dftk_mi_kblock* cube_kb, const double* recip_lattice_h, double kTF, const double* dF_d,
                       double* drho_d);
int dftk_mi_mix_dielectric(dftk_mi_kblock* cube_kb, const double* recip_lattice_h, double kTF, double eps_r,
                           const double* dF_d, double* drho_d);
int dftk_mi_chi0_dielectric_apply(dftk_mi_kblock* cube_kb, const double* recip_lattice_h, double kTF, double eps_r,
                                  const double* dV_d, double* out_d);
int dftk_mi_cube_fourier_filter(dftk_mi_kblock* cube_kb, const double* multiplier_d, const double* f_d, double* out_d);

#define DFTK_MI_XC_GGA_X_PBE 8
#define DFTK_MI_XC_GGA_C_PBE 16
int dftk_mi_xc_gga(dftk_mi_basis* basis, int64_t n, const double* rho_d, const double* sigma_d, int xc_functionals,
                   double density_threshold, double* e_d, double* vrho_d, double* vsigma_d);

int dftk_mi_xc_gga_spin(dftk_mi_basis* basis, int64_t n, const double* rho_d, const double* sigma_d, int xc_functionals,
                        double density_threshold, double* e_d, double* vrho_d, double* vsigma_d);

#define DFTK_MI_XC_MGGA_X_SCAN 64
#define DFTK_MI_XC_MGGA_C_SCAN 128
int dftk_mi_xc_mgga(dftk_mi_basis* basis, int64_t n, const double* rho_d, const double* sigma_d, const double* tau_d,
                    int xc_functionals, double density_threshold, double* e_d, double* vrho_d, double* vsigma_d,
                    double* vtau_d);

int dftk_mi_ifft_sphere(dftk_mi_kblock* kb, const dftk_mi_cplx* c_d, dftk_mi_cplx* cube_d);
int dftk_mi_fft_sphere(dftk_mi_kblock* kb, const dftk_mi_cplx* cube_d, dftk_mi_cplx* c_d);

int dftk_mi_density_accumulate(dftk_mi_kblock* kb, int n_bands, const dftk_mi_cplx* psi_d,
                               int64_t ld_psi, const double* weight_h, double* rho_d);

int dftk_mi_kinetic_energy_density_accumulate(dftk_mi_kblock* kb, int n_bands, const dftk_mi_cplx* psi_d,
                                              int64_t ld_psi, const double* weight_h, double* tau_d);

int dftk_mi_density_accumulate_spin(dftk_mi_kblock* kb, int n_bands, const dftk_mi_cplx* psi_d, int64_t ld_psi,
                                    const double* weight_h, double* rho_d, int spin, int n_spin);

int dftk_mi_sternheimer(dftk_mi_kblock* kb, int n_occ, const dftk_mi_cplx* psi_occ_d, int64_t ld_occ, const double* eps_h,
                        int n_extra, const dftk_mi_cplx* psi_extra_d, int64_t ld_extra, const dftk_mi_cplx* rhs_d,
                        int64_t ld_rhs, const double* tol_h, int miniter, int maxiter, const dftk_mi_cplx* dpsi0_d,
                        int64_t ld_dpsi0, dftk_mi_cplx* dpsi_d, int64_t ld_dpsi, int* n_iter, double* resid_h,
                        int* converged);
int dftk_mi_density_response_accumulate(dftk_mi_kblock* kb, int n_bands, const dftk_mi_cplx* psi_d, int64_t ld_psi,
                                        const dftk_mi_cplx* dpsi_d, int64_t ld_dpsi, const double* w_occ_h,
                                        const double* w_docc_h, double* drho_d);
int dftk_mi_apply_kernel(dftk_mi_kblock* cube_kb, const double* rho_d, const double* drho_d, const double* poisson_green_d,
                         int xc_functionals, double* dV_d);

int dftk_mi_transfer_blochwave(dftk_mi_kblock* kb_in, dftk_mi_kblock* kb_out, const int* dG_h , int n_bands,
                               const dftk_mi_cplx* in_d, int64_t ld_in, dftk_mi_cplx* out_d, int64_t ld_out);
// ... 40 lines not shown
    int64_t n, gm, gn, gk, lda, ldb, ldc;
    dftk_mi_cplx alpha, beta;
    double s0;
    const void *A, *B, *W, *W2, *W3;
    void *C, *D, *E, *F;
    dftk_mi_kblock* kb;
    void* host;
    uint64_t bytes;
} dftk_mi_batch_op;
int dftk_mi_batch_replay(dftk_mi_basis* basis, int n_fibers, int n_ops, dftk_mi_batch_op* ops);
int dftk_mi_lobpcg_history(dftk_mi_kblock* kb, int* M, int* n_iter, double* hist_h, size_t cap, int* n_svd);
int dftk_mi_kblock_reuse_AX(dftk_mi_kblock* kb, int on);
int dftk_mi_ax_reuse_count(int64_t* calls);
int dftk_mi_planes_reuse_count(int64_t* calls);

const dftk_mi_cplx* dftk_mi_lobpcg_last_AX(dftk_mi_kblock* kb);

int dftk_mi_columnwise_norms(dftk_mi_basis* basis, int64_t n, int m, const dftk_mi_cplx* X_d, int64_t ldx,
                             double* norms_h );
int dftk_mi_columnwise_dots(dftk_mi_basis* basis, int64_t n, int m, const dftk_mi_cplx* A_d, int64_t lda,
                            const dftk_mi_cplx* B_d, int64_t ldb, dftk_mi_cplx* dots_h );
int dftk_mi_ortho_qr(dftk_mi_basis* basis, int64_t n, int m, dftk_mi_cplx* X_d, int64_t ldx, int force_svd,
                     int* n_chol, int* used_svd);
int dftk_mi_tpa_precondprep(dftk_mi_kblock* kb, int m, const dftk_mi_cplx* X_d, int64_t ldx, double* mean_kin_h);
int dftk_mi_tpa_ldiv(dftk_mi_kblock* kb, int m, const dftk_mi_cplx* R_d, int64_t ldr, const double* mean_kin_h,
                     double default_shift, dftk_mi_cplx* Y_d, int64_t ldy);
int dftk_mi_block_residual(dftk_mi_kblock* kb, int m, const dftk_mi_cplx* AX_d, int64_t lda,
                           const dftk_mi_cplx* X_d, int64_t ldx, const double* lambda_h, dftk_mi_cplx* R_d,
                           int64_t ldr, double* norms_h, double* mean_kin_h, double* xx_h);

int dftk_mi_zgemm(dftk_mi_basis* basis, char transA, int64_t m, int64_t n, int64_t k,
                  dftk_mi_cplx alpha, const dftk_mi_cplx* A_d, int64_t lda,
                  const dftk_mi_cplx* B_d, int64_t ldb, dftk_mi_cplx beta,
                  dftk_mi_cplx* C_d, int64_t ldc);
#define DFTK_MI_GEMM_UPPER 1
#define DFTK_MI_GEMM_B_UPPER 2
#define DFTK_MI_GEMM_REAL 8
#define DFTK_MI_GEMM_SYM_RESULT 32
int dftk_mi_zgemm_ex(dftk_mi_basis* basis, char transA, int64_t m, int64_t n, int64_t k,
                     dftk_mi_cplx alpha, const dftk_mi_cplx* A_d, int64_t lda,
                     const dftk_mi_cplx* B_d, int64_t ldb, dftk_mi_cplx beta,
                     dftk_mi_cplx* C_d, int64_t ldc, int flags);
int dftk_mi_zgemm_to(dftk_mi_basis* basis, char transA, int64_t m, int64_t n, int64_t k,
                     dftk_mi_cplx alpha, const dftk_mi_cplx* A_d, int64_t lda,
                     const dftk_mi_cplx* B_d, int64_t ldb, dftk_mi_cplx beta,
                     const dftk_mi_cplx* C_d, int64_t ldc, dftk_mi_cplx* D_d, int flags);
int dftk_mi_heev(dftk_mi_basis* basis, int n, dftk_mi_cplx* A_d, int64_t lda, double* W_h,
                 dftk_mi_cplx* V_d, int64_t ldv);
int dftk_mi_heev_lowest(dftk_mi_basis* basis, int n, int nev, dftk_mi_cplx* A_d, int64_t lda, double* W_h,
                        dftk_mi_cplx* V_d, int64_t ldv);
int dftk_mi_eig_mirror_tall(dftk_mi_basis* basis, int n, int real, dftk_mi_cplx* X_d, int64_t ldt);
int dftk_mi_heev_sigma_host(int n, const double* diag_h, int nev, double* sigma, double* gap_guess,
                            int* hold_iterations, double norm_bound);
int dftk_mi_potrf_trtri(dftk_mi_basis* basis, int n, dftk_mi_cplx* A_d, int64_t lda,
                        dftk_mi_cplx* invR_d, int64_t ldi);
int dftk_mi_potrf_trtri_real(dftk_mi_basis* basis, int n, dftk_mi_cplx* A_d, int64_t lda,
                             dftk_mi_cplx* invR_d, int64_t ldi);

int dftk_mi_lowdin_ortho(dftk_mi_basis* basis, int64_t n_rows, int n_cols, dftk_mi_cplx* Phi_d, int64_t ld,
                         double* evals_h);
int dftk_mi_pdos_accumulate(dftk_mi_basis* basis, int64_t n_rows, int n_bands, const dftk_mi_cplx* psi_d, int64_t ld_psi,
                            int n_proj, const dftk_mi_cplx* Phi_d, int64_t ld_phi, const double* eig_h, double weight,
                            int smearing_kind, double temperature, int n_eps, const double* eps_h, double* proj_d,
                            double* pdos_d);

int dftk_mi_hubbard_occupation(dftk_mi_basis* basis, int64_t n_rows, int n_bands, const dftk_mi_cplx* psi_d, int64_t ld_psi,
                               int n_proj, const dftk_mi_cplx* Phi_d, int64_t ld_phi, const double* w_h, int n_blocks,
                               const int* block_first_h, const int* block_size_h, dftk_mi_cplx* n_d);
int dftk_mi_hubbard_rotate(dftk_mi_basis* basis, int64_t n_rows, int n_blocks, const int* block_first_h,
                           const int* block_size_h, const dftk_mi_cplx* Phi_d, int64_t ld_phi, const dftk_mi_cplx* V_h,
                           dftk_mi_cplx* Out_d, int64_t ld_out);

int dftk_mi_comm_get_unique_id(char id_out[128]);
int dftk_mi_comm_init_rank(const char id[128], int n_ranks, int rank, int device,
                           dftk_mi_comm** comm_out);
typedef int (*dftk_mi_allreduce_fn)(void* user, double* buf_h, size_t n);
typedef int (*dftk_mi_alltoallv_fn)(void* user, const double* send_h, const size_t* send_counts,
                                    const size_t* send_offsets, double* recv_h, const size_t* recv_counts,
                                    const size_t* recv_offsets);
int dftk_mi_comm_create_host(int n_ranks, int rank, int device, dftk_mi_allreduce_fn allreduce,
                             dftk_mi_alltoallv_fn alltoallv, void* user, dftk_mi_comm** comm_out);
int dftk_mi_comm_destroy(dftk_mi_comm* comm);
int dftk_mi_comm_describe(const dftk_mi_comm* comm, int* backend, int* n_ranks, int* version);
int dftk_mi_comm_rank(const dftk_mi_comm* comm);
int dftk_mi_comm_size(const dftk_mi_comm* comm);
int dftk_mi_allreduce_sum_f64(dftk_mi_comm* comm, double* buf_d, size_t n, void* stream);

int dftk_mi_kblock_set_shard(dftk_mi_kblock* kb, dftk_mi_comm* comm, const int64_t* row_starts_h);

int dftk_mi_kblock_set_gamma_real(dftk_mi_kblock* kb, int on);
int dftk_mi_gamma_half_size(dftk_mi_kblock* kb, int64_t* n_half);
int dftk_mi_gamma_tables_host(int nx, int ny, int nz, int64_t n_G, const int64_t* mapping0_h, int64_t* n_half,
                              int32_t* row_h, int32_t* partner_row_h);
int dftk_mi_gamma_compress(dftk_mi_kblock* kb, int m, const dftk_mi_cplx* X_d, int64_t ldx, dftk_mi_cplx* Xh_d,
                           int64_t ldh);
int dftk_mi_gamma_compress_aligned(dftk_mi_kblock* kb, int m, const dftk_mi_cplx* X_d, int64_t ldx, dftk_mi_cplx* Xh_d,
                                   int64_t ldh);
int dftk_mi_gamma_expand(dftk_mi_kblock* kb, int m, const dftk_mi_cplx* Xh_d, int64_t ldh, dftk_mi_cplx* X_d,
                         int64_t ldx);
int dftk_mi_gamma_apply_H(dftk_mi_kblock* kb, int which, int n_bands, const dftk_mi_cplx* psih_d, int64_t ld_psi,
                          dftk_mi_cplx* Hpsih_d, int64_t ld_Hpsi);
int dftk_mi_density_accumulate_real(dftk_mi_kblock* kb, int n_bands, const dftk_mi_cplx* psi_d, int64_t ld_psi,
                                    const double* weight_h, double* rho_d);

int dftk_mi_shard_plan_host(int n_ranks, int rank, int n_bands, const int64_t* row_starts_h, int* band_starts,
                            int64_t* slab_off, int64_t* slab_cnt, int64_t* band_off, int64_t* band_cnt);

int dftk_mi_prof_enable(dftk_mi_basis* basis, int on);
int dftk_mi_prof_get(dftk_mi_basis* basis, int family, double* total_ms, double* work, int64_t* launches);
typedef struct dftk_mi_anderson dftk_mi_anderson;
int dftk_mi_anderson_create(dftk_mi_basis* basis, int64_t n, int m, double maxcond, double errorfactor,
                            dftk_mi_anderson** out);
int dftk_mi_anderson_destroy(dftk_mi_anderson* acc);
int dftk_mi_anderson_reset(dftk_mi_anderson* acc);
int dftk_mi_anderson_history(const dftk_mi_anderson* acc);
int dftk_mi_anderson_step(dftk_mi_anderson* acc, const double* x_d, double alpha, const double* Pf_d, double* x_next_d,
                          int* n_history );
int dftk_mi_chi0_mix(dftk_mi_kblock* cube_kblock, int n_comp, const double* recip_lattice_h, const double* poisson_d,
                     const double* ldos_d, double dvol, int dielectric, double kTF, double eps_r, const double* dF_d,
                     double reltol, int krylovdim, int maxiter, double* drho_d, int* n_applies, int* converged);

int dftk_mi_stiefel_project_tangent(dftk_mi_basis* basis, int64_t n, int m, const dftk_mi_cplx* X_d, int64_t ldx,
                                    dftk_mi_cplx* G_d, int64_t ldg);
typedef struct dftk_mi_lbfgs dftk_mi_lbfgs;
int dftk_mi_lbfgs_create(dftk_mi_basis* basis, int n_blocks, const int64_t* n_rows_h, const int* n_cols_h, int memory,
                         dftk_mi_lbfgs** out);
int dftk_mi_lbfgs_destroy(dftk_mi_lbfgs* acc);
int dftk_mi_lbfgs_reset(dftk_mi_lbfgs* acc);
int dftk_mi_lbfgs_history(const dftk_mi_lbfgs* acc);
int dftk_mi_lbfgs_update(dftk_mi_lbfgs* acc, const dftk_mi_cplx* const* x_d, const int64_t* ldx_h,
                         const dftk_mi_cplx* const* g_d, const int64_t* ldg_h, double* sy_h, int* kept);
int dftk_mi_lbfgs_direction(dftk_mi_lbfgs* acc, const dftk_mi_cplx* const* g_d, const int64_t* ldg_h,
                            dftk_mi_kblock* const* kblocks , const double* const* mean_kin_h ,
                            const double* scale_h , dftk_mi_cplx* const* d_d, const int64_t* ldd_h);

int dftk_mi_launch_count(int64_t* launches, int64_t* host_syncs);

int dftk_mi_device_buffers_live(int64_t* count, int64_t* bytes);

int dftk_mi_step_sums(dftk_mi_basis* basis, int64_t n, const double* a_d, const double* b_d, const double* c_d, double* out_h);

int dftk_mi_fermi_bisection(int n_k, const int* n_bands, const double* eig, const double* kweights, int smearing,
                            double temperature, double filled, double n_electrons, double lo, double hi, double* eF_out);
int dftk_mi_prof_zgemm_shapes(dftk_mi_basis* basis, int cap, int64_t* rows6, double* ms, int* count);

int dftk_mi_diag_mfma_peak(dftk_mi_basis* basis, int waves_per_simd, int iters, double* tflops);

int dftk_mi_zgemm_plan_host(char transA, int64_t m, int64_t n, int64_t k, int flags, int* out12);
int dftk_mi_zgemm_fold_host(char transA, int64_t m, int64_t n, int64_t k, int flags, int cap, int* items4, int* count);
int dftk_mi_zgemm_compact_host(int gm, int gn, int q, int nsplit, int cap, int* items3, int* count);
int dftk_mi_jacobi_schedule_host(int n, int round, int* n_blocks, int* pairs ,
                                 int* where );
int dftk_mi_fft_plan_host(int n, int* n_radices, int* radices , int* pos );
int dftk_mi_sphere_tables_host(int nx, int ny, int nz, int64_t n_G, const int64_t* mapping0_h,
                               int64_t* n_lines, int* n_zplanes, int64_t* line_id ,
                               int64_t* line_start );

#ifdef __cplusplus
}
#endif
#endif
```

Before: 6.500.

## Add tile-major layout for FFT intermediate T2 buffer and make it default

Introduces a configurable layout for the T2 intermediate between y and z FFT passes, with a new tile-major ordering (x-tile, y, z, lane) as the default instead of plane-major. All y-pass, z-pass, register z-pass and density kernels now index T2 through a stride map, and grid or column mapping is reordered so that consecutive blocks touch contiguous tiles. The aim is better locality for z-column reads and writes, which are strided by a full plane in the old layout. The trade-off is that y-pass accesses become more strided, and the planes-handover cache now also keys on layout.

```diff
diff --git a/dftk.jl_amd/_lib.py b/dftk.jl_amd/_lib.py
--- a/dftk.jl_amd/_lib.py
+++ b/dftk.jl_amd/_lib.py
@@ -35,6 +35,7 @@
     "dftk_mi_basis_destroy": (C.c_int, [C.c_void_p]),
     "dftk_mi_basis_sync": (C.c_int, [C.c_void_p]),
     "dftk_mi_basis_set_fft_batch": (C.c_int, [C.c_void_p, C.c_int]),
+    "dftk_mi_basis_set_fft_layout": (C.c_int, [C.c_void_p, C.c_int]),
     "dftk_mi_basis_stream": (C.c_void_p, [C.c_void_p]),
     "dftk_mi_kblock_create": (C.c_int, [C.c_void_p, _i64, C.c_void_p, C.c_void_p, C.POINTER(C.c_void_p)]),
     "dftk_mi_kblock_destroy": (C.c_int, [C.c_void_p]),
@@ -228,6 +229,7 @@
     "dftk_mi_jacobi_schedule_host": (C.c_int, [C.c_int, C.c_int, C.POINTER(C.c_int), C.POINTER(C.c_int),
                                                C.POINTER(C.c_int)]),
     "dftk_mi_fft_plan_host": (C.c_int, [C.c_int, C.POINTER(C.c_int), C.POINTER(C.c_int), C.POINTER(C.c_int)]),
+    "dftk_mi_fft_t2_map_host": (C.c_int, [C.c_int, C.c_int, C.c_int, C.c_int, C.c_int, C.c_void_p, C.c_void_p]),
     "dftk_mi_sphere_tables_host": (C.c_int, [C.c_int, C.c_int, C.c_int, _i64, C.c_void_p, C.POINTER(_i64),
                                              C.POINTER(C.c_int), C.c_void_p, C.c_void_p]),
 }
diff --git a/dftk.jl_amd/csrc/api.cpp b/dftk.jl_amd/csrc/api.cpp
--- a/dftk.jl_amd/csrc/api.cpp
+++ b/dftk.jl_amd/csrc/api.cpp
@@ -323,6 +323,12 @@
     b->volume = unit_cell_volume;
     b->device = device;
     b->fft_batch = 32;
+    static const int layout0 = [] {
+        const char* e = getenv("DFTK_MI_FFT_T2_LAYOUT");
+        return e && (atoi(e) == DFTK_MI_FFT_T2_PLANE_MAJOR || atoi(e) == DFTK_MI_FFT_T2_TILE_MAJOR) ? atoi(e)
+                                                                                                    : DFTK_MI_FFT_T2_DEFAULT;
+    }();
+    b->fft_layout = layout0;
     b->prof.reset(new Prof());
     const char* g = getenv("DFTK_MI_GEMM");
     b->use_mfma = (g && strcmp(g, "naive") == 0) ? 0 : 1;
@@ -374,6 +380,30 @@
 extern "C" int dftk_mi_basis_set_fft_batch(dftk_mi_basis* b, int n) {
     if (!b || n < 1 || n > 256) return DFTK_MI_EINVAL;
     b->fft_batch = n;
+    return 0;
+}
+
+extern "C" int dftk_mi_basis_set_fft_layout(dftk_mi_basis* b, int which) {
+    if (!b || (which != DFTK_MI_FFT_T2_PLANE_MAJOR && which != DFTK_MI_FFT_T2_TILE_MAJOR)) return DFTK_MI_EINVAL;
+    b->fft_layout = which;
+    return 0;
+}
+
+extern "C" int dftk_mi_fft_t2_map_host(int which, int nxp, int ny, int nzx, int nzp, int64_t* index, int64_t* strides3) {
+    if ((which != DFTK_MI_FFT_T2_PLANE_MAJOR && which != DFTK_MI_FFT_T2_TILE_MAJOR) || nxp < 8 || nxp % 8 != 0 || ny < 1 ||
+        nzx < 1 || nzp < nzx)
+        return DFTK_MI_EINVAL;
+    const T2Map tm = t2_map(which, nxp, ny, nzp);
+    if (index)
+        for (int xt = 0; xt < nxp / 8; ++xt)
+            for (int y = 0; y < ny; ++y)
+                for (int zi = 0; zi < nzx; ++zi)
+                    for (int lane = 0; lane < 8; ++lane) *index++ = t2_index(tm, xt, y, zi, lane);
+    if (strides3) {
+        strides3[0] = tm.sx;
+        strides3[1] = tm.sy;
+        strides3[2] = tm.sz;
+    }
     return 0;
 }
 
diff --git a/dftk.jl_amd/csrc/common.h b/dftk.jl_amd/csrc/common.h
--- a/dftk.jl_amd/csrc/common.h
+++ b/dftk.jl_amd/csrc/common.h
@@ -108,6 +108,18 @@
     const int* pos;
 };
 
+#define DFTK_MI_FFT_T2_DEFAULT DFTK_MI_FFT_T2_TILE_MAJOR
+struct T2Map {
+    int64_t sx, sy, sz;
+    int tile_major;
+};
+__host__ __device__ inline T2Map t2_map(int which, int nxp, int ny, int nzp) {
+    return which == 1 ? T2Map{(int64_t)ny * nzp * 8, (int64_t)nzp * 8, 8, 1} : T2Map{8, nxp, (int64_t)ny * nxp, 0};
+}
+__host__ __device__ inline int64_t t2_index(const T2Map& m, int xt, int y, int zi, int lane) {
+    return (int64_t)xt * m.sx + (int64_t)y * m.sy + (int64_t)zi * m.sz + lane;
+}
+
 int  plan_radices(int n, int* nrad, int* rad);
 void plan_positions(int n, int nrad, const int* rad, int* pos);
 
@@ -135,6 +147,7 @@
     FftAxis ax[3] = {};
     DevTable<void> d_tables[6];
     int fft_batch = 0;
+    int fft_layout = 0;
     DevBuf<cd> T1;
     DevBuf<cd> T2;
     DevBuf<void> ws;
diff --git a/dftk.jl_amd/csrc/fft_kernels.hip b/dftk.jl_amd/csrc/fft_kernels.hip
--- a/dftk.jl_amd/csrc/fft_kernels.hip
+++ b/dftk.jl_amd/csrc/fft_kernels.hip
@@ -298,6 +298,20 @@
     double w2;
 };
 
+__device__ __forceinline__ void grid_tile(const T2Map& tm, int& xt, int& other) {
+    xt = tm.tile_major ? blockIdx.y : blockIdx.x;
+    other = tm.tile_major ? blockIdx.x : blockIdx.y;
+}
+__device__ __forceinline__ void column_tile(const T2Map& tm, int grp, int nxt, int ny, int& xt, int& y) {
+    if (tm.tile_major) {
+        xt = grp / ny;
+        y = grp - xt * ny;
+    } else {
+        y = grp / nxt;
+        xt = grp - y * nxt;
+    }
+}
+
 template <bool GEN, bool PAIR = false>
 __global__ __launch_bounds__(FFT_THREADS) void k_xbwd_scatter(FftAxis ax, int nxp, int n_lines,
                                                               const int* __restrict__ line_start,
@@ -354,14 +368,16 @@
                                                       const int* __restrict__ zls,
                                                       const int* __restrict__ line_ypos,
                                                       const cd* __restrict__ T1, int64_t T1_stride,
-                                                      cd* __restrict__ T2, int64_t T2_stride,
+                                                      cd* __restrict__ T2, int64_t T2_stride, T2Map tm,
                                                       const FftJob* __restrict__ jobs) {
     constexpr int FFT_LS = FFT_LS_YZ;
     cd* buf = reinterpret_cast<cd*>(dftk_smem);
     cd* tw = buf + ay.n * FFT_LS;
     const int tid = threadIdx.x, l = tid & (FFT_L - 1), j = tid >> 3;
-    const int x = blockIdx.x * FFT_L + l;
-    const int zi = blockIdx.y, band = blockIdx.z;
+    int xt, zi;
+    grid_tile(tm, xt, zi);
+    const int x = xt * FFT_L + l;
+    const int band = blockIdx.z;
     if (jobs) {
         const FftJob jb = jobs[band];
         if (zi >= jb.nzx) return;
@@ -388,15 +404,15 @@
     }
     __syncthreads();
     fft_tile<FFT_LS, false, GEN>(buf, tw, ay, +1.0, l, j);
-    cd* t2 = T2 + (int64_t)band * T2_stride + (int64_t)zi * ny * nxp + x;
-    for (int y = j; y < ny; y += FFT_TPL) t2[(int64_t)y * nxp] = buf[y * FFT_LS + l];
+    cd* t2 = T2 + (int64_t)band * T2_stride + t2_index(tm, xt, 0, zi, l);
+    for (int y = j; y < ny; y += FFT_TPL) t2[(int64_t)y * tm.sy] = buf[y * FFT_LS + l];
 }
 
 template <int MODE, bool GEN>
 __global__ __launch_bounds__(FFT_THREADS, ZPASS_MIN_BLOCKS) void k_zpass(FftAxis az, int nx, int nxp, int ny, int nzx,
                                                        int nbands, const int* __restrict__ zpos,
                                                        const double* __restrict__ Vs,
-                                                       cd* __restrict__ T2, int64_t T2_stride,
+                                                       cd* __restrict__ T2, int64_t T2_stride, T2Map tm,
                                                        cd* __restrict__ cube, const FftJob* __restrict__ jobs = nullptr) {
     constexpr int FFT_LS = FFT_LS_YZ;
     cd* buf = reinterpret_cast<cd*>(dftk_smem);
@@ -413,17 +429,18 @@
         nzx = jb.nzx;
         Vs = jb.Vs;
     }
-    const int y = grp / nxt;
-    const int x = (grp - y * nxt) * FFT_L + l;
+    int xt, y;
+    column_tile(tm, grp, nxt, ny, xt, y);
+    const int x = xt * FFT_L + l;
     const int nz = az.n;
     const int64_t plane = (int64_t)ny * nxp;
-    cd* t2 = T2 + (int64_t)band * T2_stride + (int64_t)y * nxp + x;
+    cd* t2 = T2 + (int64_t)band * T2_stride + t2_index(tm, xt, y, 0, l);
     const bool early = MODE != 2 && nzx <= 3 * FFT_TPL;
     cd e0, e1, e2;
     if (early) {
-        if (j < nzx) e0 = t2[(int64_t)j * plane];
-        if (j + FFT_TPL < nzx) e1 = t2[(int64_t)(j + FFT_TPL) * plane];
-        if (j + 2 * FFT_TPL < nzx) e2 = t2[(int64_t)(j + 2 * FFT_TPL) * plane];
+        if (j < nzx) e0 = t2[(int64_t)j * tm.sz];
+        if (j + FFT_TPL < nzx) e1 = t2[(int64_t)(j + FFT_TPL) * tm.sz];
+        if (j + 2 * FFT_TPL < nzx) e2 = t2[(int64_t)(j + 2 * FFT_TPL) * tm.sz];
     }
     tile_prologue<FFT_LS>(buf, tw, az, MODE != 2, true);
     __syncthreads();
@@ -434,7 +451,7 @@
             if (j + FFT_TPL < nzx) buf[zpos[j + FFT_TPL] * FFT_LS + l] = e1;
             if (j + 2 * FFT_TPL < nzx) buf[zpos[j + 2 * FFT_TPL] * FFT_LS + l] = e2;
         } else {
-            for (int zi = j; zi < nzx; zi += FFT_TPL) buf[zpos[zi] * FFT_LS + l] = t2[(int64_t)zi * plane];
+            for (int zi = j; zi < nzx; zi += FFT_TPL) buf[zpos[zi] * FFT_LS + l] = t2[(int64_t)zi * tm.sz];
         }
         __syncthreads();
         fused_v = fft_tile<FFT_LS, false, GEN>(buf, tw, az, +1.0, l, j,
@@ -463,7 +480,7 @@
         __syncthreads();
     }
     fft_tile<FFT_LS, true, GEN>(buf, tw, az, -1.0, l, j, nullptr, 0, MODE == 0 && fused_v);
-    for (int zi = j; zi < nzx; zi += FFT_TPL) t2[(int64_t)zi * plane] = buf[zpos[zi] * FFT_LS + l];
+    for (int zi = j; zi < nzx; zi += FFT_TPL) t2[(int64_t)zi * tm.sz] = buf[zpos[zi] * FFT_LS + l];
 }
 
 namespace ctw {
@@ -629,7 +646,7 @@
 template <int R1A, int R1B, int R2A, int R2B>
 __global__ __launch_bounds__(FFT_L * ((R1A * R1B > R2A * R2B) ? R1A * R1B : R2A * R2B), ZREG_MIN_BLOCKS)
 void k_zpass_reg(FftAxis az, int nx, int nxp, int ny, int nzx, int z_lo, int nbands, const double* __restrict__ Vs,
-                 cd* __restrict__ T2, int64_t T2_stride, const FftJob* __restrict__ jobs) {
+                 cd* __restrict__ T2, int64_t T2_stride, T2Map tm, const FftJob* __restrict__ jobs) {
     typedef FourStep<R1A, R1B, R2A, R2B> FS;
     cd* buf = reinterpret_cast<cd*>(dftk_smem);
     const int tid = threadIdx.x, l = tid & (FFT_L - 1), j = tid >> 3;
@@ -644,12 +661,12 @@
         z_lo = jb.z_lo;
         Vs = jb.Vs;
     }
-    const int y = grp / nxt;
-    const int x = (grp - y * nxt) * FFT_L + l;
+    int xt, y;
+    column_tile(tm, grp, nxt, ny, xt, y);
     const unsigned plane = (unsigned)ny * (unsigned)nxp;
-    const int64_t col0 = (int64_t)y * nxp + (x - l);
-    cd* __restrict__ t2 = T2 + (int64_t)band * T2_stride + col0;
-    const unsigned planeB = plane * (unsigned)sizeof(cd), stepB = (unsigned)FS::R2 * planeB;
+    const int64_t col0 = (int64_t)y * nxp + xt * FFT_L;
+    cd* __restrict__ t2 = T2 + (int64_t)band * T2_stride + t2_index(tm, xt, y, 0, 0);
+    const unsigned planeB = (unsigned)tm.sz * (unsigned)sizeof(cd), stepB = (unsigned)FS::R2 * planeB;
     const unsigned off_lo = (unsigned)j * planeB + (unsigned)l * (unsigned)sizeof(cd);
     const unsigned off_hi = off_lo - (unsigned)(FS::N - nzx) * planeB;
     const int zneg0 = FS::N - (nzx - z_lo);
@@ -695,15 +712,15 @@
 template <int R1A, int R1B, int R2A, int R2B>
 __global__ __launch_bounds__(FFT_L * ((R1A * R1B > R2A * R2B) ? R1A * R1B : R2A * R2B), ZREG_MIN_BLOCKS)
 void k_zdensity_reg(FftAxis az, int nx, int nxp, int ny, int nzx, int z_lo, int nb, const double* __restrict__ w,
-                    const double* __restrict__ wim, const cd* __restrict__ T2, int64_t T2_stride,
+                    const double* __restrict__ wim, const cd* __restrict__ T2, int64_t T2_stride, T2Map tm,
                     double* __restrict__ rho, const FftJob* __restrict__ jobs, double* __restrict__ part,
                     double* __restrict__ rho2 = nullptr) {
     typedef FourStep<R1A, R1B, R2A, R2B> FS;
     cd* buf = reinterpret_cast<cd*>(dftk_smem);
     const int tid = threadIdx.x, l = tid & (FFT_L - 1), j = tid >> 3;
-    const int x = blockIdx.x * FFT_L + l;
-    const int y = blockIdx.y;
-    const unsigned plane = (unsigned)ny * (unsigned)nxp;
+    int xt, y;
+    grid_tile(tm, xt, y);
+    const int x = xt * FFT_L + l;
     double acc[FS::R2], acc2[FS::R2];
 #pragma unroll
     for (int p = 0; p < FS::R2; ++p) acc[p] = acc2[p] = 0.0;
@@ -721,8 +738,8 @@
             wi = wim ? wim[ib] : wb;
         }
         if (wb == 0.0 && wi == 0.0 && wb2 == 0.0) continue;
-        const cd* __restrict__ t2 = T2 + (int64_t)ib * T2_stride + (int64_t)y * nxp + (x - l);
-        const unsigned planeB = plane * (unsigned)sizeof(cd), stepB = (unsigned)FS::R2 * planeB;
+        const cd* __restrict__ t2 = T2 + (int64_t)ib * T2_stride + t2_index(tm, xt, y, 0, 0);
+        const unsigned planeB = (unsigned)tm.sz * (unsigned)sizeof(cd), stepB = (unsigned)FS::R2 * planeB;
         const unsigned off_lo = (unsigned)j * planeB + (unsigned)l * (unsigned)sizeof(cd);
         const unsigned off_hi = off_lo - (unsigned)(FS::N - nzx) * planeB;
         const int zneg0 = FS::N - (nzx - z_lo);
@@ -769,15 +786,17 @@
 __global__ __launch_bounds__(FFT_THREADS, YFWD_MIN_BLOCKS) void k_yfwd(FftAxis ay, int nxp, int ny,
                                                       const int* __restrict__ zls,
                                                       const int* __restrict__ line_ypos,
-                                                      const cd* __restrict__ T2, int64_t T2_stride,
+                                                      const cd* __restrict__ T2, int64_t T2_stride, T2Map tm,
                                                       cd* __restrict__ T1, int64_t T1_stride,
                                                       const FftJob* __restrict__ jobs) {
     constexpr int FFT_LS = FFT_LS_YZ;
     cd* buf = reinterpret_cast<cd*>(dftk_smem);
     cd* tw = buf + ay.n * FFT_LS;
     const int tid = threadIdx.x, l = tid & (FFT_L - 1), j = tid >> 3;
-    const int x = blockIdx.x * FFT_L + l;
-    const int zi = blockIdx.y, band = blockIdx.z;
+    int xt, zi;
+    grid_tile(tm, xt, zi);
+    const int x = xt * FFT_L + l;
+    const int band = blockIdx.z;
     if (jobs) {
         const FftJob jb = jobs[band];
         if (zi >= jb.nzx) return;
@@ -785,8 +804,8 @@
         line_ypos = jb.line_ypos;
     }
     tile_prologue<FFT_LS>(buf, tw, ay, false);
-    const cd* t2 = T2 + (int64_t)band * T2_stride + (int64_t)zi * ny * nxp + x;
-    for (int y = j; y < ny; y += FFT_TPL) buf[y * FFT_LS + l] = t2[(int64_t)y * nxp];
+    const cd* t2 = T2 + (int64_t)band * T2_stride + t2_index(tm, xt, 0, zi, l);
+    for (int y = j; y < ny; y += FFT_TPL) buf[y * FFT_LS + l] = t2[(int64_t)y * tm.sy];
     __syncthreads();
     fft_tile<FFT_LS, true, GEN>(buf, tw, ay, -1.0, l, j);
     cd* t1 = T1 + (int64_t)band * T1_stride;
@@ -856,17 +875,17 @@
                                                           const int* __restrict__ zpos, int nb,
                                                           const double* __restrict__ w,
                                                           const double* __restrict__ wim,
-                                                          const cd* __restrict__ T2, int64_t T2_stride,
+                                                          const cd* __restrict__ T2, int64_t T2_stride, T2Map tm,
                                                           double* __restrict__ rho, const FftJob* __restrict__ jobs,
                                                           double* __restrict__ part, double* __restrict__ rho2 = nullptr) {
     constexpr int FFT_LS = FFT_LS_YZ;
     cd* buf = reinterpret_cast<cd*>(dftk_smem);
     cd* tw = buf + az.n * FFT_LS;
     const int tid = threadIdx.x, l = tid & (FFT_L - 1), j = tid >> 3;
-    const int x = blockIdx.x * FFT_L + l;
-    const int y = blockIdx.y;
+    int xt, y;
+    grid_tile(tm, xt, y);
+    const int x = xt * FFT_L + l;
     const int nz = az.n;
-    const int64_t plane = (int64_t)ny * nxp;
     double acc[DENS_MAXACC], acc2[DENS_MAXACC];
 #pragma unroll
     for (int k = 0; k < DENS_MAXACC; ++k) acc[k] = acc2[k] = 0.0;
@@ -888,8 +907,8 @@
         const cd z0 = make_double2(0.0, 0.0);
         for (int t = tid; t < nz * FFT_LS; t += FFT_THREADS) buf[t] = z0;
         __syncthreads();
-        const cd* t2 = T2 + (int64_t)ib * T2_stride + (int64_t)y * nxp + x;
-        for (int zi = j; zi < nzx; zi += FFT_TPL) buf[zpos[zi] * FFT_LS + l] = t2[(int64_t)zi * plane];
+        const cd* t2 = T2 + (int64_t)ib * T2_stride + t2_index(tm, xt, y, 0, l);
+        for (int zi = j; zi < nzx; zi += FFT_TPL) buf[zpos[zi] * FFT_LS + l] = t2[(int64_t)zi * tm.sz];
         __syncthreads();
         fft_tile<FFT_LS, false, GEN>(buf, tw, az, +1.0, l, j);
 #pragma unroll
@@ -932,16 +951,16 @@
                                                                    int nzx, const int* __restrict__ zpos, int nb,
                                                                    const double* __restrict__ wo,
                                                                    const double* __restrict__ wd,
-                                                                   const cd* __restrict__ T2, int64_t T2_stride,
+                                                                   const cd* __restrict__ T2, int64_t T2_stride, T2Map tm,
                                                                    double* __restrict__ drho) {
     constexpr int FFT_LS = FFT_LS_YZ;
     cd* buf = reinterpret_cast<cd*>(dftk_smem);
     cd* tw = buf + az.n * FFT_LS;
     const int tid = threadIdx.x, l = tid & (FFT_L - 1), j = tid >> 3;
-    const int x = blockIdx.x * FFT_L + l;
-    const int y = blockIdx.y;
+    int xt, y;
+    grid_tile(tm, xt, y);
+    const int x = xt * FFT_L + l;
     const int nz = az.n;
-    const int64_t plane = (int64_t)ny * nxp;
     double acc[DENS_MAXACC];
     cd pv[DENS_MAXACC];
 #pragma unroll
@@ -953,8 +972,8 @@
         if (w2 == 0.0 && w1 == 0.0) continue;
         for (int t = tid; t < nz * FFT_LS; t += FFT_THREADS) buf[t] = z0;
         __syncthreads();
-        const cd* t2 = T2 + (int64_t)ib * T2_stride + (int64_t)y * nxp + x;
-        for (int zi = j; zi < nzx; zi += FFT_TPL) buf[zpos[zi] * FFT_LS + l] = t2[(int64_t)zi * plane];
+        const cd* t2 = T2 + (int64_t)ib * T2_stride + t2_index(tm, xt, y, 0, l);
+        for (int zi = j; zi < nzx; zi += FFT_TPL) buf[zpos[zi] * FFT_LS + l] = t2[(int64_t)zi * tm.sz];
         __syncthreads();
         fft_tile<FFT_LS, false, GEN>(buf, tw, az, +1.0, l, j);
 #pragma unroll
@@ -967,8 +986,8 @@
         if (w2 == 0.0) continue;
         for (int t = tid; t < nz * FFT_LS; t += FFT_THREADS) buf[t] = z0;
         __syncthreads();
-        const cd* d2 = T2 + (int64_t)(nb + ib) * T2_stride + (int64_t)y * nxp + x;
-        for (int zi = j; zi < nzx; zi += FFT_TPL) buf[zpos[zi] * FFT_LS + l] = d2[(int64_t)zi * plane];
+        const cd* d2 = T2 + (int64_t)(nb + ib) * T2_stride + t2_index(tm, xt, y, 0, l);
+        for (int zi = j; zi < nzx; zi += FFT_TPL) buf[zpos[zi] * FFT_LS + l] = d2[(int64_t)zi * tm.sz];
         __syncthreads();
         fft_tile<FFT_LS, false, GEN>(buf, tw, az, +1.0, l, j);
 #pragma unroll
@@ -1085,6 +1104,10 @@
     return j;
 }
 
+static dim3 tile_grid(const T2Map& tm, int nxt, int other, int nz) {
+    return tm.tile_major ? dim3(other, nxt, nz) : dim3(nxt, other, nz);
+}
+
 struct FftPipe {
     dftk_mi_basis* b;
     hipStream_t stream;
@@ -1092,6 +1115,7 @@
     cd *T1, *T2;
     int64_t s1, s2;
     int n_lines, nzx;
+    T2Map tm;
     FftJob tab;
     const FftJob* jobs;
     bool reg_z;
@@ -1102,11 +1126,13 @@
     dftk_mi_basis* b = kb->basis;
     const int64_t s1 = (int64_t)kb->n_lines * b->nxp, s2 = (int64_t)kb->nzx * b->ny * b->nxp;
     return FftPipe{b, b->stream, nb, b->T1 + t_off * s1, planes ? planes : b->T2 + t_off * s2, s1, s2, (int)kb->n_lines,
-                   kb->nzx, kblock_tables(kb), nullptr, kb->z_lo >= 0, true, kb->n_G};
+                   kb->nzx, t2_map(b->fft_layout, b->nxp, b->ny, kb->nzx), kblock_tables(kb), nullptr, kb->z_lo >= 0, true,
+                   kb->n_G};
 }
 static FftPipe jobs_pipe(dftk_mi_basis* b, hipStream_t stream, int nb, const FftJob* jobs, cd* T1, cd* T2, int64_t s1,
                          int64_t s2, int max_lines, int max_nzx, bool reg_z) {
-    return FftPipe{b, stream, nb, T1, T2, s1, s2, max_lines, max_nzx, FftJob{}, jobs, reg_z, false, 0};
+    return FftPipe{b, stream, nb, T1, T2, s1, s2, max_lines, max_nzx, t2_map(b->fft_layout, b->nxp, b->ny, max_nzx), FftJob{},
+                   jobs, reg_z, false, 0};
 }
 
 #define REG_SIZES(X)                                                                                                      \
@@ -1132,11 +1158,11 @@
     if constexpr (DENS) {
         CHK(set_lds_attr(k_zdensity_reg<A, B, C, D>, lds));
         hipLaunchKernelGGL((k_zdensity_reg<A, B, C, D>), grid, dim3(FS::THREADS), lds, p.stream, b->ax[2], b->nx, b->nxp, b->ny,
-                           p.tab.nzx, p.tab.z_lo, p.nb, w, wim, (const cd*)p.T2, p.s2, rho, p.jobs, part, rho2);
+                           p.tab.nzx, p.tab.z_lo, p.nb, w, wim, (const cd*)p.T2, p.s2, p.tm, rho, p.jobs, part, rho2);
     } else {
         CHK(set_lds_attr(k_zpass_reg<A, B, C, D>, lds));
         hipLaunchKernelGGL((k_zpass_reg<A, B, C, D>), grid, dim3(FS::THREADS), lds, p.stream, b->ax[2], b->nx, b->nxp, b->ny,
-                           p.tab.nzx, p.tab.z_lo, p.nb, p.tab.Vs, p.T2, p.s2, p.jobs);
+                           p.tab.nzx, p.tab.z_lo, p.nb, p.tab.Vs, p.T2, p.s2, p.tm, p.jobs);
     }
     return 0;
 }
@@ -1180,16 +1206,16 @@
 static int stage_B(const FftPipe& p) {
     const dftk_mi_basis* b = p.b;
     const int ps = book(p, PROF_FFT_B, (t1_bytes(p) + t2_bytes(p)) * p.nb);
-    LAUNCH_FFT((k_ybwd<GEN>), b->ax[1], dim3(b->nxp / FFT_L, p.nzx, p.nb), lds_bytes(b->ny), p.stream, b->ax[1], b->nxp,
-               b->ny, p.tab.zls, p.tab.line_ypos, (const cd*)p.T1, p.s1, p.T2, p.s2, p.jobs);
+    LAUNCH_FFT((k_ybwd<GEN>), b->ax[1], tile_grid(p.tm, b->nxp / FFT_L, p.nzx, p.nb), lds_bytes(b->ny), p.stream, b->ax[1],
+               b->nxp, b->ny, p.tab.zls, p.tab.line_ypos, (const cd*)p.T1, p.s1, p.T2, p.s2, p.tm, p.jobs);
     prof_end(p.b, ps);
     return 0;
 }
 static int stage_D(const FftPipe& p) {
     const dftk_mi_basis* b = p.b;
     const int ps = book(p, PROF_FFT_D, (t1_bytes(p) + t2_bytes(p)) * p.nb);
-    LAUNCH_FFT((k_yfwd<GEN>), b->ax[1], dim3(b->nxp / FFT_L, p.nzx, p.nb), lds_bytes(b->ny), p.stream, b->ax[1], b->nxp,
-               b->ny, p.tab.zls, p.tab.line_ypos, (const cd*)p.T2, p.s2, p.T1, p.s1, p.jobs);
+    LAUNCH_FFT((k_yfwd<GEN>), b->ax[1], tile_grid(p.tm, b->nxp / FFT_L, p.nzx, p.nb), lds_bytes(b->ny), p.stream, b->ax[1],
+               b->nxp, b->ny, p.tab.zls, p.tab.line_ypos, (const cd*)p.T2, p.s2, p.tm, p.T1, p.s1, p.jobs);
     prof_end(p.b, ps);
     return 0;
 }
@@ -1217,7 +1243,7 @@
     if (rs < 0) return rs;
     if (rs == 1)
         LAUNCH_FFT((k_zpass<0, GEN>), b->ax[2], grid, lds_bytes(b->nz), p.stream, b->ax[2], b->nx, b->nxp, b->ny, p.tab.nzx,
-                   p.nb, p.tab.zpos, p.tab.Vs, p.T2, p.s2, (cd*)nullptr, p.jobs);
+                   p.nb, p.tab.zpos, p.tab.Vs, p.T2, p.s2, p.tm, (cd*)nullptr, p.jobs);
     prof_end(p.b, ps);
     return 0;
 }
@@ -1225,7 +1251,7 @@
 static int stage_z_cube(const FftPipe& p, cd* cube) {
     const dftk_mi_basis* b = p.b;
     LAUNCH_FFT((k_zpass<MODE, GEN>), b->ax[2], zpass_grid(b, p.nb), lds_bytes(b->nz), p.stream, b->ax[2], b->nx, b->nxp,
-               b->ny, p.tab.nzx, p.nb, p.tab.zpos, (const double*)nullptr, p.T2, p.s2, cube, p.jobs);
+               b->ny, p.tab.nzx, p.nb, p.tab.zpos, (const double*)nullptr, p.T2, p.s2, p.tm, cube, p.jobs);
     return 0;
 }
 int launch_ifft_to_cube(dftk_mi_kblock* kb, const cd* c, cd* cube, int nb) {
@@ -1255,21 +1281,21 @@
 static int stage_density(const FftPipe& p, const double* w, const double* wim, double* rho, int groups = 1,
                          double* part = nullptr, double* rho2 = nullptr) {
     const dftk_mi_basis* b = p.b;
-    const dim3 grid(b->nxp / FFT_L, b->ny, groups);
+    const dim3 grid = tile_grid(p.tm, b->nxp / FFT_L, b->ny, groups);
     const int ps = book(p, PROF_DENS_Z, t2_bytes(p) * p.nb + 16.0 * (double)b->nx * b->ny * b->nz);
     const int rs = reg_launch<true>(p, grid, w, wim, rho, part, rho2);
     if (rs < 0) return rs;
     if (rs == 1)
         LAUNCH_FFT((k_zdensity<GEN>), b->ax[2], grid, lds_bytes(b->nz), p.stream, b->ax[2], b->nx, b->nxp, b->ny, p.tab.nzx,
-                   p.tab.zpos, p.nb, w, wim, (const cd*)p.T2, p.s2, rho, p.jobs, part, rho2);
+                   p.tab.zpos, p.nb, w, wim, (const cd*)p.T2, p.s2, p.tm, rho, p.jobs, part, rho2);
     prof_end(p.b, ps);
     return 0;
 }
 static int stage_density_response(const FftPipe& p, const double* wo, const double* wd, double* drho) {
     const dftk_mi_basis* b = p.b;
     const int ps = book(p, PROF_DENS_Z, 2.0 * t2_bytes(p) * p.nb + 16.0 * (double)b->nx * b->ny * b->nz);
-    LAUNCH_FFT((k_zdensity_response<GEN>), b->ax[2], dim3(b->nxp / FFT_L, b->ny), lds_bytes(b->nz), p.stream, b->ax[2], b->nx,
-               b->nxp, b->ny, p.tab.nzx, p.tab.zpos, p.nb, wo, wd, (const cd*)p.T2, p.s2, drho);
+    LAUNCH_FFT((k_zdensity_response<GEN>), b->ax[2], tile_grid(p.tm, b->nxp / FFT_L, b->ny, 1), lds_bytes(b->nz), p.stream,
+               b->ax[2], b->nx, b->nxp, b->ny, p.tab.nzx, p.tab.zpos, p.nb, wo, wd, (const cd*)p.T2, p.s2, p.tm, drho);
     prof_end(p.b, ps);
     return 0;
 }
diff --git a/dftk.jl_amd/csrc/gamma_kernels.hip b/dftk.jl_amd/csrc/gamma_kernels.hip
--- a/dftk.jl_amd/csrc/gamma_kernels.hip
+++ b/dftk.jl_amd/csrc/gamma_kernels.hip
@@ -582,7 +582,7 @@
         wre[p] = w_h[2 * p];
         wim[p] = (2 * p + 1 < nb) ? w_h[2 * p + 1] : 0.0;
     }
-    if (keep) kb->ho.planes_begin(nb, kb->basis->fft_batch);
+    if (keep) kb->ho.planes_begin(nb, kb->basis->fft_batch, kb->basis->fft_layout);
     if (pairs_in_A) return launch_density(kb, nb2, psi, ldpsi, wre.data(), rho, wim.data(), nullptr, nullptr, keep, nb);
     return launch_density(kb, nb2, kb->gr->buf, kb->n_G, wre.data(), rho, wim.data(), nullptr, nullptr, keep);
 }
diff --git a/dftk.jl_amd/csrc/handover.h b/dftk.jl_amd/csrc/handover.h
--- a/dftk.jl_amd/csrc/handover.h
+++ b/dftk.jl_amd/csrc/handover.h
@@ -18,13 +18,13 @@
 
     void promise(bool on) { promised_ = on && kept_ != nullptr; }
 
-    Taken take(int M, int64_t N, bool workspace_moves, bool planes_eligible, int fft_batch) {
+    Taken take(int M, int64_t N, bool workspace_moves, bool planes_eligible, int fft_batch, int fft_layout = 0) {
         Taken t;
         if (promised_ && kept_M_ == M && kept_N_ == N && !workspace_moves) {
             t.AX = kept_;
             t.ld = kept_ld_;
             t.planes = planes_eligible && on_ && planes != nullptr && back_M_ == M && batch_ == fft_batch &&
-                       valid_.size() == (size_t)(M + 1) / 2;
+                       layout_ == fft_layout && valid_.size() == (size_t)(M + 1) / 2;
         }
         promised_ = false;
         kept_ = nullptr;
@@ -57,9 +57,10 @@
     bool pass_keeps_planes(const cd* psi, int64_t ld, int nb) const {
         return !declined_ && back_X_ != nullptr && back_X_ == psi && back_ld_ == ld && back_M_ == nb;
     }
-    void planes_begin(int nb, int fft_batch) {
+    void planes_begin(int nb, int fft_batch, int fft_layout = 0) {
         valid_.assign((size_t)(nb + 1) / 2, 0);
         batch_ = fft_batch;
+        layout_ = fft_layout;
         on_ = true;
     }
     void planes_mark(int p0, int n) { std::fill_n(valid_.begin() + p0, n, (char)1); }
@@ -85,5 +86,6 @@
     bool on_ = false;
     bool declined_ = false;
     int batch_ = 0;
+    int layout_ = 0;
     std::vector<char> valid_;
 };
diff --git a/dftk.jl_amd/csrc/lobpcg.cpp b/dftk.jl_amd/csrc/lobpcg.cpp
--- a/dftk.jl_amd/csrc/lobpcg.cpp
+++ b/dftk.jl_amd/csrc/lobpcg.cpp
@@ -573,7 +573,7 @@
         const size_t dbl = 9 * (size_t)DS;
         const size_t need = (nbig * blk + small_elems) * sizeof(cd) + dbl * sizeof(double) + m3 * sizeof(int) + 1024;
         const bool grows = need > kb->lob_buf.bytes();
-        const LobHandover::Taken kept = kb->ho.take(M, N, grows, planes_eligible(kb), b->fft_batch);
+        const LobHandover::Taken kept = kb->ho.take(M, N, grows, planes_eligible(kb), b->fft_batch, b->fft_layout);
         kept_AX = kept.AX;
         kept_ld = kept.ld;
         kept_planes = kept.planes;
diff --git a/include/dftk_mi355x.h b/include/dftk_mi355x.h
--- a/include/dftk_mi355x.h
+++ b/include/dftk_mi355x.h
@@ -34,6 +34,9 @@
 int dftk_mi_basis_destroy(dftk_mi_basis* basis);
 int dftk_mi_basis_sync(dftk_mi_basis* basis);
 int dftk_mi_basis_set_fft_batch(dftk_mi_basis* basis, int n_bands_per_batch);
+#define DFTK_MI_FFT_T2_PLANE_MAJOR 0
+#define DFTK_MI_FFT_T2_TILE_MAJOR  1
+int dftk_mi_basis_set_fft_layout(dftk_mi_basis* basis, int which);
 void* dftk_mi_basis_stream(dftk_mi_basis* basis);
 
 int dftk_mi_kblock_create(dftk_mi_basis* basis, int64_t n_G, const int64_t* mapping0_h,
@@ -380,6 +383,8 @@
 int dftk_mi_jacobi_schedule_host(int n, int round, int* n_blocks, int* pairs ,
                                  int* where );
 int dftk_mi_fft_plan_host(int n, int* n_radices, int* radices , int* pos );
+int dftk_mi_fft_t2_map_host(int which, int nxp, int ny, int nzx, int nzp, int64_t* index ,
+                            int64_t* strides3);
 int dftk_mi_sphere_tables_host(int nx, int ny, int nz, int64_t n_G, const int64_t* mapping0_h,
                                int64_t* n_lines, int* n_zplanes, int64_t* line_id ,
                                int64_t* line_start );
```

Result: no change. 6.550 (median of 5 runs) (+0.8%).
